# vvvvvw/Sentinel

Hardware: AMD Instinct MI355X
Metric: decided entries/sec (whole node) at 1M resources; % of HBM roofline (higher is better)
Workload: dtype int64/f64

## Files before the change

### sentinel_amd/csrc/decide.hip

```cpp
#include <hip/hip_runtime.h>
#include <stdlib.h>
#include <stdint.h>

#include "authority.h"
#include "chain.h"
#include "aux.h"
#include "pmap.h"

using namespace sg;

#define WAVE 64
#define MAXR 16
#define JMAX_FLOW 4
#define JMAX_DEG 4
#define JMAX_RL 2

__device__ __forceinline__ uint32_t lane_id() { return __lane_id(); }
__device__ __forceinline__ uint64_t lanemask_lt() {
    uint32_t l = lane_id();
    return l == 0 ? 0ull : (~0ull >> (64 - l));
}

#define J8_MAX (1u << 23)
#define SEG_ITEMS 16
// ... 26 lines not shown
__device__ __forceinline__ uint32_t seg_block_excl_scan(uint32_t v, uint32_t* total) {
    __shared__ uint32_t ws[4];
    const int w = threadIdx.x >> 6, l = threadIdx.x & 63;
    uint32_t x = v;
#pragma unroll
    for (int o = 1; o < 64; o <<= 1) {
        const uint32_t y = __shfl_up(x, o, 64);
        if (l >= o) x += y;
    }
    if (l == 63) ws[w] = x;
    __syncthreads();
    uint32_t pre = 0, tot = 0;
#pragma unroll
    for (int k = 0; k < 4; ++k) { if (k < w) pre += ws[k]; tot += ws[k]; }
    *total = tot;
    return pre + x - v;
}
__global__ __launch_bounds__(256) void k_seg_count(const uint32_t* __restrict__ keys, uint64_t n, uint32_t* __restrict__ cnt,
                                                   const uint32_t* __restrict__ lo) {
    const uint64_t b = lo ? *lo : 0u;
    if ((uint64_t)(blockIdx.x + 1) * SEG_TILE <= b) {
        if (threadIdx.x == 0) cnt[blockIdx.x] = 0;
        return;
    }
    uint32_t kk[SEG_ITEMS];
    const uint64_t i0 = (uint64_t)blockIdx.x * SEG_TILE + (uint64_t)threadIdx.x * SEG_ITEMS;
    const uint32_t f = seg_flags16(keys, n, i0, kk, b);
    uint32_t tot;
    (void)seg_block_excl_scan((uint32_t)__popc(f), &tot);
    if (threadIdx.x == 0) cnt[blockIdx.x] = tot;
}
__global__ __launch_bounds__(256) void k_seg_emit(const uint32_t* __restrict__ keys, uint64_t n,
                                                  const uint32_t* __restrict__ off, Seg* __restrict__ segs,
                                                  const uint32_t* __restrict__ lo, const uint32_t* __restrict__ sbase) {
    const uint64_t b = lo ? *lo : 0u;
    if ((uint64_t)(blockIdx.x + 1) * SEG_TILE <= b) return;
    uint32_t kk[SEG_ITEMS];
    const uint64_t i0 = (uint64_t)blockIdx.x * SEG_TILE + (uint64_t)threadIdx.x * SEG_ITEMS;
    uint32_t f = seg_flags16(keys, n, i0, kk, b);
    uint32_t tot;
    uint32_t pos = (sbase ? *sbase : 0u) + off[blockIdx.x] + seg_block_excl_scan((uint32_t)__popc(f), &tot);
#pragma unroll
    for (int j = 0; j < SEG_ITEMS; ++j) {
        if ((f >> j) & 1u) {
            Seg sg;
            sg.res = kk[j];
            sg.start = (uint32_t)(i0 + j);
            sg.len = 0;
            sg.bin = 0;
            segs[pos++] = sg;
        }
    }
}
#define AUX_SHORT 256u
__device__ __forceinline__ uint32_t wave_alloc(uint32_t* ctr, uint32_t k) {
    uint32_t x = k;
#pragma unroll
    for (int o = 1; o < 64; o <<= 1) {
        const uint32_t y = __shfl_up(x, o, 64);
        if ((int)(threadIdx.x & 63) >= o) x += y;
    }
    const uint32_t tot = __shfl(x, 63, 64);
    uint32_t base = 0;
    if ((threadIdx.x & 63) == 63 && tot) base = atomicAdd(ctr, tot);
    base = __shfl(base, 63, 64);
    return base + x - k;
}
__global__ __launch_bounds__(256) void k_seg_bin(Seg* __restrict__ segs, const uint32_t* __restrict__ mp, uint64_t n,
// ... 73 lines not shown
                for (uint32_t wd = b0 >> 5; wd <= (b1 >> 5); ++wd) {
                    uint32_t m32 = 0xFFFFFFFFu;
                    if (wd == (b0 >> 5)) m32 &= 0xFFFFFFFFu << (b0 & 31);
                    if (wd == (b1 >> 5)) m32 &= 0xFFFFFFFFu >> (31 - (b1 & 31));
                    atomicOr(&need_blk[wd], m32);
                }
                tabs = true;
            }
        }
        const uint32_t rank = atomicAdd(&cnt[bin], 1u);
        sg.bin = bin | (auxp ? SEG_AUXP : 0u) | (tabs ? SEG_TABS : 0u) | (rank << SEG_RANK_SHIFT);
        segs[s] = sg;
    }
    if (aux) {
        const uint32_t o = wave_alloc(aux + 0, aux_short ? 1u : 0u);
        if (aux_short) ashort[o] = s;
        const uint32_t q = wave_alloc(aux + 1, aux_np);
        const uint32_t j = wave_alloc(aux + 3, aux_np ? 1u : 0u);
        if (aux_np) along[j] = ((uint64_t)s << 32) | q;
        const uint32_t u = wave_alloc(aux + 2, aux_np > 1 ? 1u : 0u);
        if (aux_np > 1) amulti[u] = ((uint64_t)s << 32) | q;
    }
    if (mix) {
        const uint32_t a = wave_alloc(mixc + 0, mixk == 1 ? 1u : 0u);
        if (mixk == 1) mix[a] = s;
        const uint32_t b = wave_alloc(mixc + 1, mixk == 2 ? 1u : 0u);
        if (mixk == 2) mix[mix_cap + b] = s;
    }
    __syncthreads();
    for (uint32_t b = threadIdx.x; b < N_BINS; b += blockDim.x) blkcnt[(uint64_t)b * nblk + blockIdx.x] = cnt[b];
}
__global__ __launch_bounds__(256) void k_seg_order(Seg* __restrict__ segs, const uint32_t* __restrict__ mp,
                                                   const uint32_t* __restrict__ off, uint32_t nblk,
                                                   uint32_t* __restrict__ order) {
    const uint32_t s = blockIdx.x * blockDim.x + threadIdx.x;
    if (s >= *mp) return;
    const uint32_t v = segs[s].bin, bin = v & 0x3F;
    order[off[(uint64_t)bin * nblk + blockIdx.x] + (v >> SEG_RANK_SHIFT)] = s;
    segs[s].bin = v & ((1u << SEG_RANK_SHIFT) - 1);
}
__global__ void k_bin_offsets(const uint32_t* __restrict__ off, uint32_t nblk, const uint32_t* __restrict__ mp,
                              uint32_t* __restrict__ out) {
    const uint32_t b = threadIdx.x;
    if (b < N_BINS) out[b] = off[(uint64_t)b * nblk];
    if (b == N_BINS) out[b] = *mp;
}

__global__ __launch_bounds__(256) void k_scatter_rec(const SEv* __restrict__ rec_o, uint64_t n,
                                                     const uint32_t* __restrict__ pos_of, SEv* __restrict__ recs,
                                                     uint32_t* __restrict__ prev, uint32_t* __restrict__ nprev,
                                                     Link* __restrict__ link, uint32_t* __restrict__ bst, uint32_t epoch,
                                                     uint32_t* __restrict__ bflags) {
    const uint64_t i = (uint64_t)blockIdx.x * blockDim.x + threadIdx.x;
    if (i >= n) return;
    SEv r = rec_o[i];
    const uint32_t p = pos_of[i] & 0x7FFFFFFFu;
    if (r.code == RC_BATCH) {
        const uint32_t po = pos_of[r.x];
        if (po & 0x80000000u) r.x = po & 0x7FFFFFFFu;
        else r.code = r.kind == SG_EV_EXIT ? RC_NONE : RC_NOT;
    } else if (r.code == RC_PREV) {
        prev[atomicAdd(nprev, 1u)] = p;
    }
    if (r.kind == SG_EV_ENTRY) {
        if (r.cnt == 0) atomicOr(bflags, BF_ZERO_CNT);
    } else if (r.code == RC_NONE || r.code == RC_PREV) {
        atomicOr(&bst[p >> 10], BST_STATIC);
    }
// ... 27 lines not shown
        if (in[k] && kind != SG_EV_ENTRY && code == RC_BATCH)
            xd[k] = reinterpret_cast<unsigned long long*>(kind == SG_EV_EXIT ? &link[w[k].y].exit_l : &link[w[k].y].trace_l);
    }
    auto xch = [&](int k) -> uint32_t {
        const uint64_t p = base + (uint64_t)k * 256 + threadIdx.x;
        return xd[k] ? (uint32_t)(atomicExch(xd[k], ((unsigned long long)epoch << 32) | (uint32_t)p) >> 32) : 0u;
    };
    uint32_t o0 = 0, o1 = 0, o2 = 0, o3 = 0;
    if (tables) { o0 = xch(0); o1 = xch(1); o2 = xch(2); o3 = xch(3); }
    uint32_t ka[4], kb[4];
#pragma unroll
    for (int k = 0; k < 4; ++k) {
        const uint64_t p = base + (uint64_t)k * 256 + threadIdx.x;
        ka[k] = skeys[p < n ? p : n - 1];
        kb[k] = skeys[w[k].y < n ? w[k].y : n - 1];
    }
    bool bad = false;
#pragma unroll
    for (int k = 0; k < 4; ++k)
        if (xd[k] && w[k].y >= kmin && ka[k] != kb[k]) bad = true;
    const bool multi = o0 == epoch || o1 == epoch || o2 == epoch || o3 == epoch;
    if (__ballot(multi) && (threadIdx.x & 63) == 0) atomicOr(bflags, BF_MULTI_LINK);
    if (__ballot(bad) && (threadIdx.x & 63) == 0) atomicOr(bflags, BF_BAD_REF);
    if (!tables) return;
    for (int o = 32; o > 0; o >>= 1) v += (uint32_t)__shfl_xor((int)v, o, 64);
    if ((threadIdx.x & 63) == 0) wsum[threadIdx.x >> 6] = v;
    __syncthreads();
    if (threadIdx.x == 0) {
        const uint32_t sum = wsum[0] + wsum[1] + wsum[2] + wsum[3];
        if (sum) atomicAdd(&bst[blockIdx.x], sum);
    }
}
__global__ void k_resolve(const uint32_t* __restrict__ prev, uint32_t np, const uint8_t* __restrict__ ring,
                          SEv* __restrict__ recs, const uint32_t* __restrict__ vals, const sg_event_ext* __restrict__ ext) {
    const uint32_t i = blockIdx.x * blockDim.x + threadIdx.x;
    if (i >= np) return;
    const uint32_t p = prev[i];
    SEv r = recs[p];
    const uint8_t st = ring[r.x];
    if (st == ST_NOT_ENTRY) r.code = r.kind == SG_EV_EXIT ? RC_NONE : RC_NOT;
    else r.code = (st == ST_PASS || st == ST_PASS_WAIT) ? RC_PASSED : RC_NOT;
    r.x = 0;
    if (ext) {
        const sg_event_ext x = ext[vals[p] & 0x7FFFFFFFu];
        if (!(x.origin_id >> TAG_ORIGIN_BITS)) r.x = x.origin_id | (x.context_id << TAG_ORIGIN_BITS);
    }
    recs[p] = r;
}

#define POST_ITEMS 4
__global__ __launch_bounds__(256) void k_post(const uint32_t* __restrict__ pos_of, const uint32_t* __restrict__ dec,
                                              uint64_t n, uint64_t gbase, uint8_t* __restrict__ ring, uint64_t ring_mask,
                                              uint32_t* __restrict__ out) {
    const uint64_t base = (uint64_t)blockIdx.x * (256 * POST_ITEMS) + threadIdx.x;
    uint32_t po[POST_ITEMS], d[POST_ITEMS];
#pragma unroll
    for (int k = 0; k < POST_ITEMS; ++k) {
        const uint64_t i = base + (uint64_t)k * 256;
        po[k] = i < n ? pos_of[i] : 0u;
    }
#pragma unroll
    for (int k = 0; k < POST_ITEMS; ++k)
        d[k] = (po[k] & 0x80000000u) ? dec[po[k] & 0x7FFFFFFFu] : mk_dec(ST_NOT_ENTRY, 0, 0);
#pragma unroll
    for (int k = 0; k < POST_ITEMS; ++k) {
        const uint64_t i = base + (uint64_t)k * 256;
        if (i < n) {
            out[i] = d[k];
            ring[(gbase + i) & ring_mask] = (uint8_t)(d[k] & 0xFF);
        }
    }
}
// ... 3257 lines not shown
                    if (id != NO_ID) pm_grow(S, id, adds, pool_next, pool_nb, bflags, nullptr, nullptr, 0, epoch);
                }
        }
    }
    __threadfence();
    __syncthreads();
    if (pool_nb && t == 0 && pool_next[PC_RESCUE] == epoch) atomicOr(&sflags, (uint32_t)BF_TINY_FALLBACK);
    __syncthreads();
    if (sflags & BF_TINY_FALLBACK) {
        if (t == 0) atomicOr(bflags, sflags);
        return;
    }
    if (t < m) lane_seg<16>(recs, ev, vals, sg, S, cfg, t0, dec, bflags, t);
    __threadfence();
    __syncthreads();
    if (t < n) {
        const uint32_t d = ev[t].kind == SG_EV_ENTRY ? dec[posof[t]] : (uint32_t)ST_NOT_ENTRY;
        out[t] = d;
        S.ring[(gbase + t) & ring_mask] = (uint8_t)(d & 0xFF);
    }
    if (t == 0 && sflags) atomicOr(bflags, sflags);
}

namespace sg {

hipError_t launch_seg(const uint32_t* keys, uint64_t n, uint32_t* flag, uint32_t* pos, Seg* segs, hipStream_t st,
                      hipError_t (*scan)(const uint32_t*, uint32_t*, uint64_t, uint32_t*, uint32_t*, hipStream_t),
                      uint32_t* part, uint32_t* nseg) {
    const uint32_t nt = (uint32_t)((n + SEG_TILE - 1) / SEG_TILE);
    hipLaunchKernelGGL(k_seg_count, dim3(nt), dim3(256), 0, st, keys, n, flag, (const uint32_t*)nullptr);
    hipError_t e = scan(flag, pos, nt, part, nseg, st);
    if (e != hipSuccess) return e;
    hipLaunchKernelGGL(k_seg_emit, dim3(nt), dim3(256), 0, st, keys, n, pos, segs, (const uint32_t*)nullptr,
                       (const uint32_t*)nullptr);
    return hipGetLastError();
}
__global__ void k_add2(uint32_t* __restrict__ dst, const uint32_t* __restrict__ a, const uint32_t* __restrict__ b) {
    if (threadIdx.x == 0) *dst = *a + *b;
}
hipError_t launch_seg_cold(const uint32_t* keys, uint64_t n, const uint32_t* lo, const uint32_t* sbase, uint32_t* flag,
                           uint32_t* pos, Seg* segs, hipStream_t st,
                           hipError_t (*scan)(const uint32_t*, uint32_t*, uint64_t, uint32_t*, uint32_t*, hipStream_t),
                           uint32_t* part, uint32_t* ccount, uint32_t* nseg) {
    const uint32_t nt = (uint32_t)((n + SEG_TILE - 1) / SEG_TILE);
    hipLaunchKernelGGL(k_seg_count, dim3(nt), dim3(256), 0, st, keys, n, flag, lo);
    hipError_t e = scan(flag, pos, nt, part, ccount, st);
    if (e != hipSuccess) return e;
    hipLaunchKernelGGL(k_seg_emit, dim3(nt), dim3(256), 0, st, keys, n, pos, segs, lo, sbase);
    hipLaunchKernelGGL(k_add2, dim3(1), dim3(64), 0, st, nseg, sbase, ccount);
    return hipGetLastError();
}
hipError_t launch_block_sums(const SEv* recs, uint64_t n, uint32_t* bst, Link* link, uint32_t epoch, uint32_t* bflags,
                             const uint32_t* skeys, const uint32_t* lo, const uint32_t* need_blk, hipStream_t st) {
    hipLaunchKernelGGL(k_block_sums, dim3((uint32_t)((n + 1023) / 1024)), dim3(256), 0, st, recs, skeys, n, bst, link,
                       epoch, bflags, lo, need_blk);
    return hipGetLastError();
}
hipError_t launch_seg_bin(Seg* segs, const uint32_t* mp, uint32_t mb, uint64_t n, const Prog* prog, const uint32_t* prio,
                          uint32_t lane_max, uint32_t j1_max, uint32_t j4_max, uint32_t force_lane, uint32_t* blkcnt,
                          uint32_t pq_ok, uint32_t pq_wide, uint32_t* aux, uint32_t* ashort, uint64_t* along,
                          uint64_t* amulti, uint32_t* mixc, uint32_t* mix, uint32_t mix_cap, uint32_t* mixlen,
                          uint32_t mix_wide, uint32_t head_min, const uint16_t* hot_tab, uint32_t nhot,
                          const uint32_t* nhotseg, uint32_t* need_hot, uint32_t* need_blk, const uint32_t* bmax,
                          uint32_t skip_min, uint32_t* nmark, hipStream_t st) {
    const uint32_t nblk = (mb + 255) / 256;
    if (!nblk) return hipSuccess;
    hipLaunchKernelGGL(k_seg_bin, dim3(nblk), dim3(256), 0, st, segs, mp, n, prog, prio, lane_max, j1_max, j4_max, force_lane,
                       blkcnt, nblk, pq_ok, pq_wide, aux, ashort, along, amulti, mixc, mix, mix_cap, mixlen, mix_wide,
                       head_min, hot_tab, nhot, nhotseg, need_hot, need_blk, bmax, skip_min, nmark);
    return hipGetLastError();
}
hipError_t launch_seg_order(Seg* segs, const uint32_t* mp, uint32_t mb, const uint32_t* off, uint32_t* order,
                            uint32_t* bin_off, hipStream_t st) {
    const uint32_t nblk = (mb + 255) / 256;
    if (nblk) hipLaunchKernelGGL(k_seg_order, dim3(nblk), dim3(256), 0, st, segs, mp, off, nblk, order);
    hipLaunchKernelGGL(k_bin_offsets, dim3(1), dim3(64), 0, st, off, nblk ? nblk : 1, mp, bin_off);
    return hipGetLastError();
}
hipError_t launch_gather(const SEv* rec_o, const uint32_t* vals, const uint32_t* skeys, uint64_t n,
                         const uint32_t* pos_of, SEv* recs, uint32_t* prev, uint32_t* nprev, Link* link, uint32_t* bst,
                         uint32_t epoch, uint32_t* bflags, hipStream_t st) {
    uint32_t nb = (uint32_t)((n + 255) / 256);
    hipError_t e = hipMemsetAsync(bst, 0, ((n + 1023) / 1024) * 4, st);
    if (e != hipSuccess) return e;
    hipLaunchKernelGGL(k_scatter_rec, dim3(nb), dim3(256), 0, st, rec_o, n, pos_of, recs, prev, nprev, link, bst,
                       epoch, bflags);
    hipLaunchKernelGGL(k_block_sums, dim3((uint32_t)((n + 1023) / 1024)), dim3(256), 0, st, recs, skeys, n, bst, link,
                       epoch, bflags, (const uint32_t*)nullptr, (const uint32_t*)nullptr);
    return hipGetLastError();
}
hipError_t launch_fill(const Span* spans, const uint32_t* nspan, uint32_t cap, const SEv* recs, const Prog* prog,
                       const DRule* rules, uint32_t* dec, hipStream_t st) {
    hipLaunchKernelGGL(k_fill, dim3(2048), dim3(256), 0, st, spans, nspan, cap, recs, prog, rules, dec);
    return hipGetLastError();
}
hipError_t launch_resolve(const uint32_t* prev, uint32_t np, const uint8_t* ring, SEv* recs, const uint32_t* vals,
                          const sg_event_ext* ext, hipStream_t st) {
    if (!np) return hipSuccess;
    hipLaunchKernelGGL(k_resolve, dim3((np + 255) / 256), dim3(256), 0, st, prev, np, ring, recs, vals, ext);
    return hipGetLastError();
}
hipError_t launch_post(const uint32_t* pos_of, const uint32_t* dec, uint64_t n, uint64_t gbase, uint8_t* ring,
                       uint64_t ring_mask, uint32_t* out, hipStream_t st) {
    uint32_t nb = (uint32_t)((n + 256 * POST_ITEMS - 1) / (256 * POST_ITEMS));
    hipLaunchKernelGGL(k_post, dim3(nb), dim3(256), 0, st, pos_of, dec, n, gbase, ring, ring_mask, out);
    return hipGetLastError();
}
hipError_t launch_chain(const SEv* recs, const uint32_t* vals, const Seg* segs, uint32_t m, NodeInfo* info,
                        uint32_t grant_all, uint32_t* ncand, uint64_t* cand, const sg_event* ev, const Prog* prog,
                        const sg_event_ext* ext, uint32_t max_ctx, hipStream_t st) {
    if (!m) return hipSuccess;
    hipLaunchKernelGGL(k_chain, dim3((m + 255) / 256), dim3(256), 0, st, recs, vals, segs, m, info, grant_all, ncand,
                       cand, ev, prog, ext, max_ctx);
    return hipGetLastError();
}
hipError_t launch_tiny(const sg_event* ev, uint32_t n, const DevState& S, const DevCfg& cfg, uint32_t max_res,
                       uint32_t* prio_w, const uint32_t* comp, uint64_t n_args, uint32_t grant_all,
                       unsigned long long* pool_next, uint64_t pool_nb, uint32_t epoch, SEv* recs, uint32_t* vals,
                       uint32_t* dec, Seg* segs, uint32_t* bflags, uint32_t* out, hipStream_t st) {
    if (n == 0 || n > TINY_MAX) return hipErrorInvalidValue;
    hipLaunchKernelGGL(k_tiny, dim3(1), dim3(TINY_MAX), 0, st, ev, n, S, cfg, max_res, prio_w, comp, n_args, grant_all,
                       pool_next, pool_nb, epoch, recs, vals, dec, segs, bflags, out);
    return hipGetLastError();
}
uint32_t tiny_max() { return TINY_MAX; }
hipError_t launch_head(const SEv* recs, const Seg* segs, const uint32_t* order, uint32_t m, const DevState& S,
                       const DevCfg& cfg, int64_t t0, uint32_t* dec, uint32_t* bflags, hipStream_t st);
hipError_t launch_decide_bin(int bin, const SEv* recs, const sg_event* ev, const uint32_t* vals, const Seg* segs,
                             const uint32_t* order, uint32_t m, const DevState& S, const DevCfg& cfg, int64_t t0,
                             uint32_t* dec, uint32_t* bflags, hipStream_t st) {
    if (!m) return hipSuccess;
    if ((bin == BIN_J16 || bin == BIN_J4 || bin == BIN_J1) && cfg.heads && !(cfg.dbg_flags & HEAD_OFF)) {
// ... 43 lines not shown
```

### sentinel_amd/csrc/dev_types.h

```cpp
#pragma once
#include <hip/hip_runtime.h>
#include <stdint.h>

#include "../../include/sentinel_gpu.h"

namespace sg {

struct AuthDesc;

struct Bkt {
    int64_t ws;
    int64_t pass;
    int64_t block;
    int64_t exc;
    int64_t succ;
    int64_t rt;
    int64_t occ;
    int64_t minrt;
};
static_assert(sizeof(Bkt) == 64, "Bkt must be 64 B");

#define NO_KEY 0xFFFFFFFFFFFFFFFFull

enum : uint32_t {
// ... 114 lines not shown
    int64_t stamp[PM_BKT];
};
static_assert(sizeof(PBucket) == 128, "PBucket must be one 128-byte line");
struct PData {
    int64_t v0;
    int32_t v1;
    uint32_t pad;
};
static_assert(sizeof(PData) == 16, "PData must be 16 B");
#define PM_MIN_NB 2u
enum { PC_NEXT = 0, PC_FLOOR = 1, PC_RESCUES = 2, PC_RESCUE = 3, PC_WORDS = 4 };
__host__ __device__ inline uint32_t map_buckets(uint32_t cap) { return (2u * cap + PM_BKT - 1) / PM_BKT > 2u ? (2u * cap + PM_BKT - 1) / PM_BKT : 2u; }
struct PMap {
    uint64_t base;
    uint64_t bm;
    int64_t clock;
    int64_t thr;
    uint32_t nb;
    uint32_t cap;
    uint32_t live;
    uint32_t rb_log2;
    uint32_t pad[4];
};
static_assert(sizeof(PMap) == 64, "PMap must be 64 B");
#define PM_BASE_CAP 4000u
#define PM_TOTAL_CAP 200000u
#define PQ_MAX_CAP 8176u

enum : uint8_t { ST_PASS = 0, ST_PASS_WAIT = 1, ST_BLOCK_FLOW = 2, ST_BLOCK_DEGRADE = 3, ST_BLOCK_PARAM = 4,
                 ST_NO_CHECK = 5, ST_BLOCK_UPSTREAM = 6, ST_BLOCK_AUTHORITY = 7, ST_NOT_ENTRY = 0xFF };

#define HEAD_OFF 16384u
#define TABLES_ALL 32768u
#define LITE_CHECK 65536u
struct DevCfg {
    int32_t max_rt;
    int32_t occupy_timeout;
    int32_t max_chain;
    int32_t switch_on;
    int64_t snap_hi;
    uint64_t ring_mask;
    uint32_t dbg_flags;
    uint32_t heads;
};

struct Seg {
    uint32_t res;
    uint32_t start;
    uint32_t len;
    uint32_t bin;
};
#define SEG_AUXP 0x80u
#define SEG_PV 0x40u
#define SEG_PVT 0x100u
#define SEG_TABS 0x200u
#define SEG_RANK_SHIFT 10

struct PvSeg {
    uint32_t ok;
    uint32_t n;
    uint32_t off;
    uint32_t mid;
    uint32_t rk;
    uint32_t ch0;
    uint32_t nch;
    uint32_t fbits;
// ... 166 lines not shown
enum : uint32_t { BF_PRIORITIZED = 1,
                  BF_PQ_INVARIANT = 2,
                  BF_PTAB_FULL = 4,
                  BF_BAD_RES = 8, BF_BAD_REF = 16,
                  BF_BACKWARD = 32, BF_TSPAN = 64,
                  BF_BAD_ARGS = 512,
                  BF_AUX_FULL = 1024,
                  BF_POOL_FULL = 2048,
                  BF_MULTI_LINK = 128,
                  BF_ZERO_CNT = 256,
                  BF_TINY_FALLBACK = 4096,
                  BF_TINY_REJECTED = 8192,
                  BF_LITE_STALE = 16384 };

struct SEv {
    int32_t dt;
    uint32_t x;
    uint16_t cnt;
    uint16_t rt;
    uint8_t kind;
    uint8_t flags;
    uint8_t code;
    uint8_t pad;
};
static_assert(sizeof(SEv) == 16, "SEv must be 16 B");
enum : uint8_t {
    RC_NONE = 0,
    RC_BATCH = 1,
    RC_PASSED = 2,
    RC_NOT = 3,
    RC_PREV = 4
};

enum : uint32_t {
    BIN_J16 = 0,
    BIN_J4 = 1,
    BIN_J1 = 2,
    BIN_PQ16 = 3,
    BIN_PQ4 = 4,
    BIN_J8 = 5,
    BIN_LANE = 6,
    LANE_BINS = 19,
    BIN_LANE16 = BIN_LANE + LANE_BINS,
    BIN_LITE = BIN_LANE16 + LANE_BINS,
    N_BINS = BIN_LITE + LANE_BINS
};

}
```

### sentinel_amd/csrc/engine.cpp

```cpp
#include <hip/hip_runtime.h>

#include <algorithm>
#include <array>
#include <chrono>
#include <cmath>
#include <cstdint>
#include <cstdio>
#include <cstdlib>
#include <cstring>
#include <deque>
#include <functional>
#include <map>
#include <set>
#include <string>
#include <unordered_map>
#include <vector>

#include "../../include/sentinel_gpu.h"
#include "authority.h"
#include "dev_types.h"
#include "pkeys.h"
#include "pmap.h"
#include "pvtab.h"

namespace sg {
hipError_t launch_rs_first(const sg_event* ev, uint64_t n, uint32_t max_res, uint64_t gbase, const uint8_t* ring,
                           uint64_t ring_mask, int32_t max_rt, SEv* rec_o, uint32_t* keys, uint32_t* vals,
                           uint32_t* ghist, uint32_t nblocks, uint32_t* bflags, int64_t* t0_out, uint32_t* prio,
                           uint64_t* key_ring, const uint32_t* comp, const sg_event_ext* ext, const sg_arg* args,
                           uint64_t n_args, uint32_t max_ctx, const AuthDesc* auth, const uint32_t* auth_ids,
                           hipStream_t st);
hipError_t launch_radix_hist(const uint32_t* keys, uint64_t n, int shift, uint32_t* ghist, uint32_t nblocks,
                             hipStream_t st);
hipError_t launch_radix_hist_n(const uint32_t* keys, uint64_t n, const uint32_t* ndev, int shift, uint32_t* ghist,
                               uint32_t nblocks, hipStream_t st);
hipError_t launch_radix_scatter_n(const uint32_t* kin, const uint32_t* vin, uint64_t n, const uint32_t* ndev, int shift,
                                  const uint32_t* goff, uint32_t nblocks, uint32_t* kout, uint32_t* vout, hipStream_t st);
hipError_t launch_radix_scatter_x(const uint32_t* kin, const uint32_t* vin, uint64_t n, const uint32_t* ndev,
                                  const uint32_t* tcnt, const uint32_t* dbase, int shift, const uint32_t* goff,
                                  uint32_t nblocks, uint32_t* kout, uint32_t* vout, uint32_t* pos_of, hipStream_t st);
hipError_t launch_grp_first(const sg_event* ev, uint64_t n, uint32_t max_res, uint64_t gbase, uint64_t ring_mask,
                            uint32_t* bflags, int64_t* t0_out, uint32_t* prio, uint64_t* key_ring, const uint32_t* comp,
                            const sg_event_ext* ext, const sg_arg* args, uint64_t n_args, uint32_t max_ctx,
                            const AuthDesc* auth, const uint32_t* auth_ids,
                            const uint16_t* hot_tab, uint32_t nhot, uint32_t nblocks, uint32_t* words,
                            uint32_t* hot_hist, uint32_t* ckeys, uint32_t* cvals, uint32_t* ccnt, uint32_t* chist,
                            hipStream_t st);
hipError_t launch_hot_scan(uint32_t* C, uint32_t nblocks, uint32_t nhot, uint32_t* part, uint32_t* hb, uint32_t* total,
                           hipStream_t st);
hipError_t launch_hot_bmax(const sg_event* ev, uint32_t nblocks, const uint32_t* P, uint32_t nhot, const uint32_t* hb,
                           uint32_t* edges, uint32_t* bmax, hipStream_t st);
hipError_t launch_grp_records(const sg_event* ev, uint64_t n, uint64_t gbase, uint64_t ring_mask, int32_t max_rt,
                              const uint32_t* words, const uint32_t* P, uint32_t nhot, uint32_t nblocks,
                              const uint32_t* hb, SEv* recs, uint32_t* svals, uint32_t* prev,
                              uint32_t* nprev, uint32_t* bst, uint32_t* bflags, const sg_event_ext* ext,
                              const sg_arg* args, uint32_t max_ctx, Link* link, uint32_t epoch,
                              const uint32_t* need_hot, const uint32_t* need_blk, hipStream_t st);
hipError_t launch_hot_segs(const uint32_t* hb, uint32_t nhot, const uint32_t* hot_list, Seg* segs, uint32_t* out,
                           hipStream_t st);
hipError_t launch_hot_build(const Seg* segs, const uint32_t* mp, uint32_t mb, uint32_t min_len, uint32_t max_res, uint16_t* hot_tab,
                            uint32_t* hot_list, uint32_t nhot_old, uint32_t* hot_n, hipStream_t st);
hipError_t launch_cold_n(uint64_t n, const uint32_t* hot_total, uint32_t* out, hipStream_t st);
hipError_t launch_cold_small(const uint32_t* kin, const uint32_t* vin, const uint32_t* cnt, const uint32_t* dbase,
                             uint32_t* kout, uint32_t* vout, uint32_t* words, hipStream_t st);
uint32_t hot_max();
hipError_t launch_grp_clear(uint32_t* bsmall, uint32_t nsmall, uint32_t* bst, uint32_t nbst, uint32_t* need,
                            uint32_t nneed, hipStream_t st);
hipError_t launch_seg_cold(const uint32_t* keys, uint64_t n, const uint32_t* lo, const uint32_t* sbase, uint32_t* flag,
                           uint32_t* pos, Seg* segs, hipStream_t st,
                           hipError_t (*scan)(const uint32_t*, uint32_t*, uint64_t, uint32_t*, uint32_t*, hipStream_t),
                           uint32_t* part, uint32_t* ccount, uint32_t* nseg);
hipError_t launch_block_sums(const SEv* recs, uint64_t n, uint32_t* bst, Link* link, uint32_t epoch, uint32_t* bflags,
                             const uint32_t* skeys, const uint32_t* lo, const uint32_t* need_blk, hipStream_t st);
hipError_t launch_radix_scatter(const uint32_t* kin, const uint32_t* vin, uint64_t n, int shift, const uint32_t* goff,
                                uint32_t nblocks, uint32_t* kout, uint32_t* vout, uint32_t* pos_of, hipStream_t st);
uint32_t radix_tile();
hipError_t launch_scan(const uint32_t*, uint32_t*, uint64_t, uint32_t*, uint32_t*, hipStream_t);
hipError_t launch_snapshot(Bkt*, NodeInfo*, uint32_t, int64_t, int32_t, uint32_t*, uint32_t*, uint32_t*, uint32_t*,
                           sg_metric_node*, uint64_t, hipStream_t);
hipError_t launch_init_state(Bkt* sec, Bkt* minb, NodeInfo* info, int64_t* borrow, uint32_t nres, hipStream_t st);
hipError_t launch_set_flags(NodeInfo* info, const uint64_t* upd, uint32_t n, hipStream_t st);
hipError_t launch_region_copy(const uint64_t* src, uint64_t* dst, const uint64_t* tri, uint32_t n, hipStream_t st);
hipError_t launch_seg(const uint32_t* keys, uint64_t n, uint32_t* flag, uint32_t* pos, Seg* segs, hipStream_t st,
                      hipError_t (*scan)(const uint32_t*, uint32_t*, uint64_t, uint32_t*, uint32_t*, hipStream_t),
                      uint32_t* part, uint32_t* nseg);
hipError_t launch_seg_bin(Seg* segs, const uint32_t* mp, uint32_t mb, uint64_t n, const Prog* prog, const uint32_t* prio,
                          uint32_t lane_max, uint32_t j1_max, uint32_t j4_max, uint32_t force_lane, uint32_t* blkcnt,
                          uint32_t pq_ok, uint32_t pq_wide, uint32_t* aux, uint32_t* ashort, uint64_t* along,
                          uint64_t* amulti, uint32_t* mixc, uint32_t* mix, uint32_t mix_cap, uint32_t* mixlen,
                          uint32_t mix_wide, uint32_t head_min, const uint16_t* hot_tab, uint32_t nhot,
                          const uint32_t* nhotseg, uint32_t* need_hot, uint32_t* need_blk, const uint32_t* bmax,
                          uint32_t skip_min, uint32_t* nmark, hipStream_t st);
hipError_t launch_aux(const SEv* recs, const Seg* segs, const uint32_t* aux, const uint32_t* ashort,
                      const uint64_t* along, uint64_t* apiece, const uint64_t* amulti, const DevState& S, const DevCfg& cfg,
                      int64_t t0, const uint32_t* dec, AuxAcc* pool, uint32_t pool_cap, uint32_t* pool_n, uint64_t* meta,
                      uint32_t* bflags, hipStream_t st);
hipError_t launch_aux_cold(const SEv* recs, const Seg* segs, const uint32_t* aux, const uint32_t* ashort, const DevState& S,
                           const DevCfg& cfg, int64_t t0, const uint32_t* dec, uint32_t* bflags, hipStream_t st);
hipError_t launch_pq(int wide, const SEv* recs, const sg_event* ev, const uint32_t* vals, const Seg* segs,
                     const uint32_t* order, uint32_t m, const DevState& S, const DevCfg& cfg, int64_t t0, uint32_t* dec,
                     uint32_t* bflags, hipStream_t st);
hipError_t launch_pm_grow(const Seg* segs, const uint32_t* mp, uint32_t mb, const DevState& S, unsigned long long* pool_next,
                          uint64_t pool_nb, uint32_t* bflags, uint4* mv, uint32_t* nmv, uint32_t mcap, uint32_t epoch,
                          uint32_t nm, PBucket* b2, PData* d2, uint32_t* sz, uint32_t* off, uint32_t* part,
                          hipError_t (*scan)(const uint32_t*, uint32_t*, uint64_t, uint32_t*, uint32_t*, hipStream_t),
                          hipStream_t st);
hipError_t launch_pm_compact(PMap* pm, uint32_t n, const PBucket* ob, const PData* od, PBucket* nbk, PData* nd,
                             uint32_t* sz, uint32_t* off, uint32_t* part, unsigned long long* pool_next,
                             hipError_t (*scan)(const uint32_t*, uint32_t*, uint64_t, uint32_t*, uint32_t*, hipStream_t),
                             hipStream_t st);
// ... 2 lines not shown
hipError_t launch_pv_a(SEv* recs, const uint32_t* vals, Seg* segs, const uint32_t* list, uint32_t m,
                       const DevState& S, const DevCfg& cfg, uint32_t* dec, PvSeg* pv, PvBuf B, uint32_t cap,
                       uint32_t* tot, uint32_t* hist, uint32_t* part, hipStream_t st,
                       hipError_t (*radix_hist)(const uint32_t*, uint64_t, const uint32_t*, int, uint32_t*, uint32_t, hipStream_t),
                       hipError_t (*radix_scatter)(const uint32_t*, const uint32_t*, uint64_t, const uint32_t*, int,
                                                   const uint32_t*, uint32_t, uint32_t*, uint32_t*, hipStream_t),
                       hipError_t (*scan)(const uint32_t*, uint32_t*, uint64_t, uint32_t*, uint32_t*, hipStream_t),
                       uint32_t tile, uint32_t* rest, uint32_t grant_all);
hipError_t launch_pv_b(SEv* recs, Seg* segs, const uint32_t* list, uint32_t m, const DevState& S, int64_t t0,
                       uint32_t* dec, uint32_t* bflags, PvSeg* pv, PvBuf B, uint32_t cap, uint32_t* tot, uint32_t* part,
                       uint32_t jumps, hipStream_t st,
                       hipError_t (*scan)(const uint32_t*, uint32_t*, uint64_t, uint32_t*, uint32_t*, hipStream_t),
                       uint32_t* rest);
hipError_t launch_pvt(SEv* recs, const sg_event* ev, const uint32_t* vals, Seg* segs, const uint32_t* list, uint32_t m,
                      const DevState& S, const DevCfg& cfg, uint32_t* dec, uint32_t* bflags, PvSeg* pv, PvBuf B,
                      uint32_t cap, uint32_t* tot, uint32_t* hist, uint32_t* part, hipStream_t st,
                      hipError_t (*radix_hist)(const uint32_t*, uint64_t, const uint32_t*, int, uint32_t*, uint32_t, hipStream_t),
                      hipError_t (*radix_scatter)(const uint32_t*, const uint32_t*, uint64_t, const uint32_t*, int,
                                                      const uint32_t*, uint32_t, uint32_t*, uint32_t*, hipStream_t),
                      hipError_t (*scan)(const uint32_t*, uint32_t*, uint64_t, uint32_t*, uint32_t*, hipStream_t),
                      uint32_t tile, uint32_t* rest);
hipError_t launch_pq_mix(int post, SEv* recs, const sg_event* ev, const uint32_t* vals, const Seg* segs,
                         const uint32_t* list, uint32_t n_narrow, uint64_t wide_off, uint32_t n_wide, const DevState& S,
                         const DevCfg& cfg, int64_t t0, uint32_t* dec, uint32_t* bflags, hipStream_t st,
                         const uint32_t* rest, const uint32_t* rest_n);
hipError_t launch_seg_order(Seg* segs, const uint32_t* mp, uint32_t mb, const uint32_t* off, uint32_t* order,
                            uint32_t* bin_off, hipStream_t st);
hipError_t launch_gather(const SEv* rec_o, const uint32_t* vals, const uint32_t* skeys, uint64_t n,
                         const uint32_t* pos_of, SEv* recs, uint32_t* prev, uint32_t* nprev, Link* link, uint32_t* bst,
                         uint32_t epoch, uint32_t* bflags, hipStream_t st);
hipError_t launch_fill(const Span* spans, const uint32_t* nspan, uint32_t cap, const SEv* recs, const Prog* prog,
                       const DRule* rules, uint32_t* dec, hipStream_t st);
hipError_t launch_resolve(const uint32_t* prev, uint32_t np, const uint8_t* ring, SEv* recs, const uint32_t* vals,
                          const sg_event_ext* ext, hipStream_t st);
hipError_t launch_post_w(const uint32_t* words, const uint32_t* P, uint32_t nhot, const uint32_t* dec, uint64_t n,
                         uint64_t gbase, uint8_t* ring, uint64_t ring_mask, uint32_t* out, hipStream_t st);
hipError_t launch_post(const uint32_t* pos_of, const uint32_t* dec, uint64_t n, uint64_t gbase, uint8_t* ring,
                       uint64_t ring_mask, uint32_t* out, hipStream_t st);
hipError_t launch_chain(const SEv* recs, const uint32_t* vals, const Seg* segs, uint32_t m, NodeInfo* info,
                        uint32_t grant_all, uint32_t* ncand, uint64_t* cand, const sg_event* ev, const Prog* prog,
                        const sg_event_ext* ext, uint32_t max_ctx, hipStream_t st);
hipError_t launch_tiny(const sg_event* ev, uint32_t n, const DevState& S, const DevCfg& cfg, uint32_t max_res,
                       uint32_t* prio_w, const uint32_t* comp, uint64_t n_args, uint32_t grant_all,
                       unsigned long long* pool_next, uint64_t pool_nb, uint32_t epoch, SEv* recs, uint32_t* vals,
                       uint32_t* dec, Seg* segs, uint32_t* bflags, uint32_t* out, hipStream_t st);
uint32_t tiny_max();
hipError_t launch_decide_bin(int bin, const SEv* recs, const sg_event* ev, const uint32_t* vals, const Seg* segs,
                             const uint32_t* order, uint32_t m, const DevState& S, const DevCfg& cfg, int64_t t0,
                             uint32_t* dec, uint32_t* bflags, hipStream_t st);
hipError_t launch_tok_classify(const sg_token_req* req, uint64_t n, const CSlot* tab, uint32_t mask, uint32_t* fidx,
                               sg_token_result* res, uint32_t* flags, uint32_t* nskeys, uint32_t* nsvals, uint32_t nns,
                               hipStream_t st);
hipError_t launch_tok_limiter_ns(const sg_token_req* req, uint64_t n, const uint32_t* sk, const uint32_t* sv,
                                 const uint32_t* fidx, uint32_t nflows, NsLimiter* lims, const double* limits,
                                 uint32_t nns, uint32_t* keys, uint32_t* vals, sg_token_result* res, uint32_t* bflag,
                                 uint32_t* bidx, uint32_t* bstart, uint32_t* kpass, uint32_t* part, uint32_t* small,
                                 uint32_t* nsb,
                                 hipError_t (*scan)(const uint32_t*, uint32_t*, uint64_t, uint32_t*, uint32_t*, hipStream_t),
                                 hipStream_t st);
hipError_t launch_tok_limiter_par(const sg_token_req* req, uint64_t n, const uint32_t* fidx, uint32_t nflows,
                                  NsLimiter* lim, double allowed, uint32_t* keys, uint32_t* vals, sg_token_result* res,
                                  uint32_t* bflag, uint32_t* cflag, uint32_t* bidx, uint32_t* cexcl, uint32_t* bstart,
                                  uint32_t* kpass, uint32_t* part, uint32_t* small,
                                  hipError_t (*scan)(const uint32_t*, uint32_t*, uint64_t, uint32_t*, uint32_t*, hipStream_t),
                                  hipStream_t st);
hipError_t launch_tok_limiter(const sg_token_req* req, uint64_t n, const uint32_t* fidx, uint32_t nflows,
                              NsLimiter* lim, double allowed, uint32_t* keys, uint32_t* vals, sg_token_result* res,
// ... 332 lines not shown
    PData* d_pdat = nullptr;
    uint64_t* d_pbm = nullptr;
    uint32_t* d_ppre = nullptr;
    uint32_t* d_tmid = nullptr;
    uint8_t* d_ring = nullptr;
    uint32_t rules_cap = 0, hot_cap = 0;

    struct BatchSlot {
        sg_event* d_ev = nullptr;
        uint32_t* d_out = nullptr;
        uint32_t *d_k0 = nullptr, *d_v0 = nullptr, *d_k1 = nullptr, *d_v1 = nullptr;
        uint32_t *d_hist = nullptr, *d_part = nullptr, *d_flag = nullptr, *d_pos = nullptr, *d_order = nullptr;
        uint32_t *d_posof = nullptr, *d_dec = nullptr, *d_blkcnt = nullptr, *d_prev = nullptr;
        SEv *d_recs = nullptr, *d_rec_o = nullptr;
        uint32_t* d_ccnt = nullptr;
        bool radix = false;
        uint32_t nhot = 0;
        uint32_t hot_marked = 0;
        Seg* d_segs = nullptr;
        uint64_t* d_cand = nullptr;
        uint32_t* d_bsmall = nullptr;
        sg_event_ext* d_ext = nullptr;
        sg_arg* d_args = nullptr;
        uint64_t ext_cap = 0, args_cap = 0;
        uint32_t* d_ashort = nullptr;
        uint64_t *d_apiece = nullptr, *d_amulti = nullptr, *d_along = nullptr;
        uint64_t aux_cap_n = 0;
        uint32_t* d_mix = nullptr;
        uint64_t mix_cap = 0;
        Link* d_link = nullptr;
        uint32_t *d_bst = nullptr, *d_pend = nullptr;
        Span* d_spans = nullptr;
        hipEvent_t* ev = nullptr;
        hipEvent_t last_post = nullptr;
        uint32_t* h_head = nullptr;
        struct Grouped {
            uint64_t n = 0, n_args = 0, gbase = 0, ring_mask = 0;
            const sg_event* dev_ev = nullptr;
            const sg_event_ext* dev_ext = nullptr;
            const sg_arg* dev_args = nullptr;
            uint32_t *out = nullptr, *dev_out = nullptr, *vin = nullptr;
            uint32_t epoch = 0, skip_min = 0, lane_max = 0, mb = 0;
            bool ext = false, host_out = false, force_lane = false;
            int set = 0;
        } g;
    } slot[2];
    int cur = 0;
    int last = -1;
    int grouped = -1;
    int held_rc = 0;
    std::string held_msg;
    bool handoff_late = true;
    static constexpr int N_SETS = 4;
    hipEvent_t evset[N_SETS][5] = {};
    uint32_t* h_mirror = nullptr;
    uint64_t seq = 0;
    struct InFlight { int set; uint32_t hot_marked; };
    std::deque<InFlight> inflight;
    hipStream_t gstream = nullptr;
    std::vector<std::array<double, 4>> tlog;
    std::vector<std::array<double, 2>> glog;
    std::string fatal;
    uint32_t* d_prio = nullptr;
    uint16_t* d_hot_tab = nullptr;
    uint32_t* d_hot_list = nullptr;
    uint32_t nhot = 0;
    uint32_t* d_hot_part = nullptr;
    uint32_t* d_hot_hb = nullptr;
    uint32_t* d_need = nullptr;
    uint64_t need_words = 0;
    uint32_t* d_edges = nullptr;
    uint32_t hot_marked_last = 0;
    bool radix_group = false;
    uint64_t radix_below = 1u << 18;
    uint32_t tok_light = 8192;
    uint32_t tok_wide = 1024;
    bool tiny_on = true;
    AuxNode* d_auxtab = nullptr;
    uint32_t* d_auxcnt = nullptr;
    uint64_t aux_mask = 0;
    AuxAcc* d_auxpool = nullptr;
    uint64_t* d_auxmeta = nullptr;
    uint32_t auxpool_cap = 0;
    uint64_t auxmeta_cap = 0;
    std::unordered_map<std::string, uint32_t> origin_ids, context_ids;
    std::unordered_map<std::string, int> rule_names;
    AuthTable auth;
    AuthDesc* d_auth = nullptr;
    uint32_t* d_auth_ids = nullptr;
    size_t auth_ids_cap = 0;
    bool auth_on = false, auth_loaded = false;
    std::vector<std::string> last_auth;
    uint32_t* d_comp = nullptr;
    uint32_t* d_prev = nullptr;
    uint32_t* d_bsmall = nullptr;
    Link* d_link = nullptr;
    uint32_t *d_bst = nullptr, *d_pend = nullptr;
    Span* d_spans = nullptr;
    uint32_t span_cap = 0;
    uint32_t epoch = 0;
    uint64_t spans_total = 0;
    uint64_t cap_n = 0;
    sg_event* d_ev = nullptr;
    uint32_t* d_out = nullptr;
// ... 85 lines not shown
    uint64_t pcap = 0, pvcap = 0;
    pk::Dict<pk::StdHash> pkeys;
    std::vector<uint64_t> par_pins;
    uint64_t* d_ks_key = nullptr;
    uint32_t *d_ks_idx = nullptr, *d_ks_marks = nullptr;
    uint64_t ks_cap = 0;
    hipEvent_t ks_ev[4] = {nullptr, nullptr, nullptr, nullptr};
    uint64_t ks_sweeps = 0, ks_last[4] = {0, 0, 0, 0};
    double ks_scan_ms[3] = {0, 0, 0};
    uint64_t pbm_words = 0;
    uint32_t *d_snap_cnt = nullptr, *d_snap_off = nullptr;
    sg_metric_node* d_snap_out = nullptr;
    uint64_t snap_cap = 0;
};

static int handoff(sg_engine* e);

namespace {

constexpr uint64_t SHARD_BATCH = 3ull << 21;

static void activate(sg_engine* e, int k) {
    auto& B = e->slot[k];
    e->d_ev = B.d_ev; e->d_out = B.d_out;
    e->d_k0 = B.d_k0; e->d_v0 = B.d_v0; e->d_k1 = B.d_k1; e->d_v1 = B.d_v1;
    e->d_hist = B.d_hist; e->d_part = B.d_part; e->d_flag = B.d_flag; e->d_pos = B.d_pos; e->d_order = B.d_order;
    e->d_posof = B.d_posof; e->d_dec = B.d_dec; e->d_blkcnt = B.d_blkcnt; e->d_prev = B.d_prev;
    e->d_recs = B.d_recs; e->d_rec_o = B.d_rec_o; e->d_segs = B.d_segs; e->d_cand = B.d_cand;
    e->d_bsmall = B.d_bsmall;
    e->d_link = B.d_link; e->d_bst = B.d_bst; e->d_pend = B.d_pend; e->d_spans = B.d_spans;
}
static void free_slot(sg_engine::BatchSlot& B) {
    dfree(B.d_ev); dfree(B.d_out); dfree(B.d_k0); dfree(B.d_v0); dfree(B.d_k1); dfree(B.d_v1);
    dfree(B.d_hist); dfree(B.d_part); dfree(B.d_flag); dfree(B.d_pos); dfree(B.d_order); dfree(B.d_segs);
    dfree(B.d_cand); dfree(B.d_posof); dfree(B.d_dec); dfree(B.d_recs); dfree(B.d_rec_o); dfree(B.d_blkcnt);
    dfree(B.d_prev); dfree(B.d_bsmall); dfree(B.d_ccnt);
    B.d_ccnt = nullptr;
    dfree(B.d_link); dfree(B.d_bst); dfree(B.d_pend); dfree(B.d_spans); dfree(B.d_ext); dfree(B.d_args);
    dfree(B.d_ashort); dfree(B.d_apiece); dfree(B.d_amulti); dfree(B.d_along); dfree(B.d_mix);
    B.d_mix = nullptr;
    B.ext_cap = B.args_cap = B.aux_cap_n = B.mix_cap = 0;
    B.d_link = nullptr; B.d_bst = B.d_pend = nullptr; B.d_spans = nullptr;
    B.d_ev = nullptr; B.d_out = nullptr; B.d_k0 = B.d_v0 = B.d_k1 = B.d_v1 = nullptr;
    B.d_hist = B.d_part = B.d_flag = B.d_pos = B.d_order = nullptr;
    B.d_posof = B.d_dec = B.d_blkcnt = B.d_prev = B.d_bsmall = nullptr;
    B.d_recs = B.d_rec_o = nullptr; B.d_segs = nullptr; B.d_cand = nullptr;
}
int ensure_batch(sg_engine* e, uint64_t n) {
    if (n <= e->cap_n) return SG_OK;
    uint64_t c = std::max<uint64_t>(n, 1u << 20);
    HIPCHK(hipStreamSynchronize(e->stream));
    uint64_t nblocks = (c + radix_tile() - 1) / radix_tile();
    e->cap_hist = nblocks * 256;
    for (auto& B : e->slot) {
        free_slot(B);
        HIPCHK(hipMalloc(&B.d_ev, c * sizeof(sg_event)));
        HIPCHK(hipMalloc(&B.d_out, c * 4));
        HIPCHK(hipMalloc(&B.d_k0, c * 4));
        HIPCHK(hipMalloc(&B.d_v0, c * 4));
        HIPCHK(hipMalloc(&B.d_k1, c * 4));
        HIPCHK(hipMalloc(&B.d_v1, c * 4));
        HIPCHK(hipMalloc(&B.d_hist, e->cap_hist * 4));
        HIPCHK(hipMalloc(&B.d_part, (e->cap_hist / 4096 + c / 4096 + 64) * 4));
        HIPCHK(hipMalloc(&B.d_flag, c * 4));
        HIPCHK(hipMalloc(&B.d_pos, c * 4));
        HIPCHK(hipMalloc(&B.d_order, c * 4));
        HIPCHK(hipMalloc(&B.d_segs, c * sizeof(Seg)));
        HIPCHK(hipMalloc(&B.d_cand, c * 8));
        HIPCHK(hipMalloc(&B.d_posof, c * 4));
        HIPCHK(hipMalloc(&B.d_dec, c * 4));
        HIPCHK(hipMalloc(&B.d_recs, c * sizeof(SEv)));
        const uint64_t co = (e->radix_group || c >= (1ull << 30)) ? c : std::min<uint64_t>(c, e->radix_below);
        if (co) HIPCHK(hipMalloc(&B.d_rec_o, co * sizeof(SEv)));
        HIPCHK(hipMalloc(&B.d_ccnt, 3 * (nblocks + 64) * 4));
    }
    dfree(e->d_hot_part);
    dfree(e->d_hot_hb);
    dfree(e->d_need);
    dfree(e->d_edges);
    e->need_words = hot_max() + c / 32768 + 2 + hot_max();
    HIPCHK(hipMalloc(&e->d_need, e->need_words * 4));
    HIPCHK(hipMalloc(&e->d_edges, (nblocks + 2) * 4));
    HIPCHK(hipMalloc(&e->d_hot_part, (nblocks / 16 + 2) * hot_max() * 4));
    HIPCHK(hipMalloc(&e->d_hot_hb, 2 * hot_max() * 4));
    for (auto& B : e->slot) {
        HIPCHK(hipMalloc(&B.d_blkcnt, ((c + 255) / 256 + 1) * N_BINS * 4));
        HIPCHK(hipMalloc(&B.d_prev, c * 4));
        HIPCHK(hipMalloc(&B.d_bsmall, 256 * 4));
        HIPCHK(hipMemset(B.d_bsmall, 0, 256 * 4));
        HIPCHK(hipMalloc(&B.d_link, c * sizeof(Link)));
        HIPCHK(hipMemset(B.d_link, 0, c * sizeof(Link)));
        HIPCHK(hipMalloc(&B.d_bst, ((c + 1023) / 1024 + 1) * 4));
        HIPCHK(hipMalloc(&B.d_pend, c * 4));
        HIPCHK(hipMalloc(&B.d_spans, (c / SPAN_CHUNK + 65536) * sizeof(Span)));
    }
    e->span_cap = (uint32_t)(c / SPAN_CHUNK + 65536);
    e->cap_n = c;
    activate(e, e->cur);
    return SG_OK;
}

constexpr uint32_t HEAD_WORDS = 77;
constexpr uint32_t MIRROR_WORDS = 121;

static int collect(sg_engine* e) {
    if (e->inflight.empty()) return SG_OK;
    const sg_engine::InFlight f = e->inflight.front();
    e->inflight.pop_front();
    hipEvent_t* ev = e->evset[f.set];
    HIPCHK(hipEventSynchronize(ev[4]));
    float g = 0, d = 0, p = 0;
    (void)hipEventElapsedTime(&g, ev[0], ev[1]);
    (void)hipEventElapsedTime(&d, ev[2], ev[3]);
    (void)hipEventElapsedTime(&p, ev[3], ev[4]);
    (void)hipGetLastError();
    e->last_ms[0] = g; e->last_ms[1] = d; e->last_ms[2] = p; e->last_ms[3] = (double)g + d + p;
    e->tlog.push_back({(double)g, (double)d, (double)p, (double)g + d + p});
    if (e->tlog.size() > 4096) e->tlog.erase(e->tlog.begin(), e->tlog.begin() + 2048);
    float ga = 0, gb = 0;
    const uint64_t collected = e->seq - e->inflight.size() - 1;
    if (collected > 0) {
        hipEvent_t* pv = e->evset[(f.set + sg_engine::N_SETS - 1) % sg_engine::N_SETS];
        if (hipEventElapsedTime(&ga, pv[1], ev[0]) != hipSuccess) ga = NAN;
        if (hipEventElapsedTime(&gb, pv[4], ev[2]) != hipSuccess) gb = NAN;
        (void)hipGetLastError();
    }
    e->glog.push_back({(double)ga, (double)gb});
    if (e->glog.size() > 4096) e->glog.erase(e->glog.begin(), e->glog.begin() + 2048);
    const uint32_t* mir = e->h_mirror + (size_t)f.set * MIRROR_WORDS;
    const uint32_t bflags = mir[0];
    e->spans_total += mir[120];
    e->hot_marked_last = f.hot_marked;
    if (bflags & BF_BAD_REF)
        return fail(SG_EINVAL, "an EXIT/TRACE references an event that is not an earlier ENTRY of the same resource");
    if (bflags & BF_BACKWARD)
        return fail(SG_EINVAL, "event timestamps must be non-decreasing across batches (SURVEY Q3)");
    if (bflags & BF_AUX_FULL) return fail(SG_ECAPACITY, "origin/context node pool full (raise aux_node_capacity)");
    if (bflags & BF_LITE_STALE)
        return fail(SG_ESTATE, "internal error (SG_LITE_CHECK): k_lite stored a minute bucket without a load that was not stale");
    if (bflags & BF_PQ_INVARIANT)
        e->fatal = "internal error: a k_pq tile's presorted key subset did not match its accesses";
    else if (bflags & BF_POOL_FULL)
        e->fatal = "the hot-parameter map pool is used up (raise param_table_log2)";
    else if (bflags & BF_PTAB_FULL)
        e->fatal = "a hot-parameter map table could not place a key (its map holds a ghost entry)";
    if (bflags & (BF_PQ_INVARIANT | BF_PTAB_FULL | BF_POOL_FULL)) return fail(SG_ECAPACITY, e->fatal + " -- engine unusable");
    return SG_OK;
}
static inline const AuthDesc* dev_auth(const sg_engine* e) { return e->auth_on ? e->d_auth : nullptr; }
static inline const uint32_t* dev_auth_ids(const sg_engine* e) { return e->auth_on ? e->d_auth_ids : nullptr; }

static int drain(sg_engine* e) {
    int rc = e->held_rc;
    std::string msg = e->held_msg;
    e->held_rc = 0;
    auto note = [&](int r) {
        if (r && !rc) { rc = r; msg = g_err; }
    };
    note(handoff(e));
    while (!e->inflight.empty()) note(collect(e));
    HIPCHK(hipStreamSynchronize(e->stream));
    return rc ? fail(rc, msg) : SG_OK;
}
static void drain_hold(sg_engine* e) {
    const int rc = drain(e);
    if (rc) { e->held_rc = rc; e->held_msg = g_err; }
}


static uint32_t rule_map_cap(int64_t duration_sec) {
    const int64_t c = (int64_t)PM_BASE_CAP * std::max<int64_t>(duration_sec, 1);
    return (uint32_t)std::min<int64_t>(c, PM_TOTAL_CAP);
}

int upload_rules(sg_engine* e, bool reset_flow_state, bool reset_deg_state, bool reset_par_state) {
    uint32_t R = e->cfg.max_resources;
    std::vector<Prog> prog(R);
    std::vector<DRule> rules;
    std::vector<RState> rst;
    std::vector<DHot> hot;
    std::vector<RState> old_rst;
    std::vector<Prog> old_prog;
    if ((!reset_flow_state || !reset_deg_state || !reset_par_state) && e->n_dev_rules) {
        old_rst.resize(e->n_dev_rules);
        old_prog.resize(R);
        HIPCHK(hipMemcpy(old_rst.data(), e->d_rstate, e->n_dev_rules * sizeof(RState), hipMemcpyDeviceToHost));
        HIPCHK(hipMemcpy(old_prog.data(), e->d_prog, R * sizeof(Prog), hipMemcpyDeviceToHost));
    }
    size_t nres = e->names.size();
    bool any_mix = false, any_head = false;
    std::vector<std::pair<uint32_t, uint32_t>> relate;
    for (size_t r = 0; r < nres && r < R; ++r) {
        Prog p;
        std::memset(&p, 0, sizeof(p));
// ... 329 lines not shown
}

int sg_engine_create(const sg_config* cfg_in, sg_engine** out) {
    if (!out) return fail(SG_EINVAL, "out is null");
    sg_config cfg;
    if (cfg_in) cfg = *cfg_in;
    else sg_config_default(&cfg);
    if (cfg.sample_count != 2 || cfg.interval_ms != 1000)
        return fail(SG_ENOTSUP, "the device path implements SAMPLE_COUNT=2, INTERVAL=1000 (the reference defaults)");
    if (cfg.cold_factor <= 1) return fail(SG_EINVAL, "cold factor must be > 1");
    if (cfg.max_resources == 0 || cfg.param_table_log2 < 4 || cfg.param_table_log2 > 34 || cfg.status_ring_log2 < 10 ||
        cfg.status_ring_log2 > 36)
        return fail(SG_EINVAL, "bad capacity in sg_config");
    int ndev = 0;
    if (hipGetDeviceCount(&ndev) != hipSuccess || ndev == 0) return fail(SG_EDEVICE, "no HIP device visible");
    if (cfg.device < 0 || cfg.device >= ndev) return fail(SG_EDEVICE, "device ordinal out of range");
    hipDeviceProp_t prop;
    if (hipGetDeviceProperties(&prop, cfg.device) != hipSuccess) return fail(SG_EDEVICE, "hipGetDeviceProperties failed");
    if (std::strncmp(prop.gcnArchName, "gfx950", 6) != 0)
        return fail(SG_EDEVICE, std::string("this build targets gfx950, found ") + prop.gcnArchName);
    sg_engine* e = new sg_engine();
    e->cfg = cfg;
    e->device = cfg.device;
    auto bad = [&](int rc) { sg_engine_destroy(e); return rc; };
    if (hipSetDevice(e->device) != hipSuccess) return bad(fail(SG_EDEVICE, "hipSetDevice failed"));
    int prio_lo = 0, prio_hi = 0;
    const char* sp = std::getenv("SG_STREAM_PRIO");
    if (!(sp && sp[0] == '0')) (void)hipDeviceGetStreamPriorityRange(&prio_lo, &prio_hi);
    if (!(sp && sp[0] == '1')) std::swap(prio_lo, prio_hi);
    if (hipStreamCreateWithPriority(&e->stream, hipStreamNonBlocking, prio_hi) != hipSuccess) return bad(fail(SG_EDEVICE, "stream"));
    if (hipStreamCreateWithPriority(&e->gstream, hipStreamNonBlocking, prio_lo) != hipSuccess) {
        return bad(fail(SG_EDEVICE, "stream"));
    }
    for (auto& s : e->evset)
        for (auto& v : s) if (hipEventCreate(&v) != hipSuccess) return bad(fail(SG_EDEVICE, "event"));
    for (auto& B : e->slot) {
        if (hipHostMalloc(&B.h_head, HEAD_WORDS * 4) != hipSuccess) return bad(fail(SG_ENOMEM, "pinned batch head"));
        B.ev = e->evset[0];
    }
    if (hipHostMalloc(&e->h_mirror, sg_engine::N_SETS * MIRROR_WORDS * 4) != hipSuccess)
        return bad(fail(SG_ENOMEM, "pinned batch flags"));
    std::memset(e->h_mirror, 0, sg_engine::N_SETS * MIRROR_WORDS * 4);
    uint64_t R = cfg.max_resources;
    if (hipMalloc(&e->d_sec, R * 2 * sizeof(Bkt)) != hipSuccess || hipMalloc(&e->d_minb, R * 60 * sizeof(Bkt)) != hipSuccess ||
        hipMalloc(&e->d_info, R * sizeof(NodeInfo)) != hipSuccess || hipMalloc(&e->d_prog, R * sizeof(Prog)) != hipSuccess ||
        hipMalloc(&e->d_ring, 1ull << cfg.status_ring_log2) != hipSuccess || hipMalloc(&e->d_small, 256 * 4) != hipSuccess ||
        hipMalloc(&e->d_sink, 1024 * 4) != hipSuccess || hipMalloc(&e->d_borrow, R * 4 * sizeof(int64_t)) != hipSuccess ||
        hipMalloc(&e->d_prio, R * 4) != hipSuccess || hipMalloc(&e->d_hot_tab, R * 2) != hipSuccess ||
        hipMalloc(&e->d_hot_list, hot_max() * 4) != hipSuccess)
        return bad(fail(SG_ENOMEM, "device allocation of the engine state failed"));
    {
        const uint64_t cap = std::max<uint32_t>(cfg.aux_node_capacity, 16u);
        uint64_t slots = 32;
        while (2 * slots < 3 * cap) slots <<= 1;
        e->aux_mask = slots - 1;
        e->cfg.aux_node_capacity = (uint32_t)cap;
        if (hipMalloc(&e->d_auxtab, slots * sizeof(AuxNode)) != hipSuccess || hipMalloc(&e->d_auxcnt, 4) != hipSuccess ||
            hipMemsetAsync(e->d_auxtab, 0xFF, slots * sizeof(AuxNode), e->stream) != hipSuccess ||
            hipMemsetAsync(e->d_auxcnt, 0, 4, e->stream) != hipSuccess)
            return bad(fail(SG_ENOMEM, "device allocation of the origin/context node table failed"));
    }
    if (hipMemsetAsync(e->d_prog, 0, R * sizeof(Prog), e->stream) != hipSuccess ||
        hipMemsetAsync(e->d_ring, 0xFF, 1ull << cfg.status_ring_log2, e->stream) != hipSuccess ||
        hipMemsetAsync(e->d_prio, 0, R * 4, e->stream) != hipSuccess ||
        hipMemsetAsync(e->d_hot_tab, 0xFF, R * 2, e->stream) != hipSuccess ||
        launch_init_state(e->d_sec, e->d_minb, e->d_info, e->d_borrow, (uint32_t)R, e->stream) != hipSuccess ||
        hipStreamSynchronize(e->stream) != hipSuccess)
        return bad(fail(SG_EDEVICE, "device initialisation failed"));
    for (auto& s : e->bin_stream)
        if (hipStreamCreateWithPriority(&s, hipStreamNonBlocking, prio_hi) != hipSuccess) return bad(fail(SG_EDEVICE, "stream"));
    if (hipEventCreateWithFlags(&e->fork, hipEventDisableTiming) != hipSuccess ||
        hipEventCreateWithFlags(&e->fork0, hipEventDisableTiming) != hipSuccess ||
        hipEventCreateWithFlags(&e->grown, hipEventDisableTiming) != hipSuccess)
        return bad(fail(SG_EDEVICE, "event"));
    for (auto& v : e->join)
        if (hipEventCreateWithFlags(&v, hipEventDisableTiming) != hipSuccess) return bad(fail(SG_EDEVICE, "event"));
    if (const char* d = std::getenv("SG_DEBUG")) {
        if (d[0] == '1' && hipMalloc(&e->d_dbg, 64 * 8) == hipSuccess) (void)hipMemset(e->d_dbg, 0, 64 * 8);
    }
    if (const char* f = std::getenv("SG_DEBUG_FLAGS")) e->dbg_flags = (uint32_t)std::strtoul(f, nullptr, 0);
    e->radix_group = (e->dbg_flags & 8192) != 0;
    if (const char* f = std::getenv("SG_PROF_BIN")) e->prof_bin = std::atoi(f);
    if (const char* v = std::getenv("SG_LANE_MAX")) { e->lane_max = (uint32_t)std::strtoul(v, nullptr, 0); e->bins_pinned = true; }
    if (const char* v = std::getenv("SG_J1_MAX")) { e->j1_max = (uint32_t)std::strtoul(v, nullptr, 0); e->bins_pinned = true; }
    if (const char* v = std::getenv("SG_HEAD_MIN")) e->head_min = (uint32_t)std::strtoul(v, nullptr, 0);
    if (const char* v = std::getenv("SG_J4_MAX")) { e->j4_max = (uint32_t)std::strtoul(v, nullptr, 0); e->bins_pinned = true; }
    if (const char* v = std::getenv("SG_PIPELINE")) e->pipeline = v[0] == '1';
    if (const char* v = std::getenv("SG_HANDOFF")) e->handoff_late = v[0] != '0';
    if (const char* v = std::getenv("SG_TINY")) e->tiny_on = v[0] != '0';
    if (const char* v = std::getenv("SG_LITE_CHECK")) { if (v[0] == '1') e->dbg_flags |= LITE_CHECK; }
    if (const char* v = std::getenv("SG_RADIX_BELOW")) e->radix_below = std::strtoull(v, nullptr, 0);
    if (const char* v = std::getenv("SG_TOK_WIDE")) e->tok_wide = std::atoi(v) == 512 ? 512u : 1024u;
    if (const char* v = std::getenv("SG_TOK_LIGHT")) e->tok_light = (uint32_t)std::strtoul(v, nullptr, 0);
    if (const char* v = std::getenv("SG_TOK_NS")) e->tok_ns = v[0] == '1';
    if (const char* v = std::getenv("SG_PV_LOG2")) e->pv_log2 = (uint32_t)std::min(24l, std::max(4l, std::strtol(v, nullptr, 0)));
    if (const char* v = std::getenv("SG_PV_MAX_LOG2")) e->pv_max_log2 = (uint32_t)std::min(26l, std::max(4l, std::strtol(v, nullptr, 0)));
    e->pv_max_log2 = std::max(e->pv_max_log2, e->pv_log2);
    e->ns_names.push_back("default");
    e->ns_of["default"] = 0;
    e->ns_limit.push_back((double)cfg.cluster_max_allowed_qps);
    e->ns_conn.push_back(0);
    if (const char* v = std::getenv("SG_J1_STREAM")) e->j1_stream = std::atoi(v);
    if (const char* v = std::getenv("SG_PQ")) e->pq_on = v[0] != '0';
    if (const char* v = std::getenv("SG_MIX")) e->mix_on = v[0] != '0';
    if (const char* v = std::getenv("SG_MIX_PQ")) e->mix_pq = v[0] != '0';
    if (const char* v = std::getenv("SG_PV_PQ")) e->pv_pq = v[0] != '0';
    if (const char* v = std::getenv("SG_PV")) e->pv_on = v[0] != '0';
    e->pvt_on = e->pv_on;
    if (const char* v = std::getenv("SG_PVT")) e->pvt_on = v[0] != '0';
    if (const char* v = std::getenv("SG_PQ_WIDE")) e->pq_wide = (uint32_t)std::strtoul(v, nullptr, 0);
    if (const char* v = std::getenv("SG_SKIP_MIN")) {
        e->skip_min = std::max<uint32_t>(1u, (uint32_t)std::strtoul(v, nullptr, 0));
        e->skip_pinned = true;
    }
// ... 81 lines not shown
    if (e->pvt_on && e->d_pvtseg) {
        if (hipMemcpy(v.data(), e->d_pvtseg, v.size() * sizeof(PvSeg), hipMemcpyDeviceToHost) != hipSuccess) return -1;
        for (const auto& s : v) out[3] += s.ok ? 1 : 0;
        out[4] = tot[4];
        out[5] = tot[7];
    }
    if (!e->pv_on) out[0] = out[1] = out[2] = out[6] = 0;
    return 0;
}
extern "C" int sgx_param_pool(sg_engine* e, unsigned long long* out) {
    if (!e || !out || drain(e) != SG_OK) return -1;
    unsigned long long ctl[PC_WORDS] = {0, 0, 0, 0};
    if (e->d_pool_next && hipMemcpy(ctl, e->d_pool_next, sizeof(ctl), hipMemcpyDeviceToHost) != hipSuccess) return -1;
    out[0] = e->pool_nb; out[1] = ctl[PC_NEXT]; out[2] = ctl[PC_FLOOR]; out[3] = e->n_compact; out[4] = ctl[PC_RESCUES];
    return 0;
}

static int compact_pmaps(sg_engine* e);
extern "C" int sgx_param_compact(sg_engine* e) {
    if (!e || drain(e) != SG_OK) return -1;
    if (!e->pool_nb) return 0;
    if (compact_pmaps(e) != SG_OK) return -1;
    ++e->n_compact;
    return 0;
}

static void free_pv(sg_engine* e);

int sg_engine_destroy(sg_engine* e) {
    if (!e) return SG_OK;
    (void)hipSetDevice(e->device);
    e->grouped = -1;
    if (e->stream) (void)hipStreamSynchronize(e->stream);
    if (e->gstream) (void)hipStreamSynchronize(e->gstream);
    dfree(e->d_sec); dfree(e->d_minb); dfree(e->d_info); dfree(e->d_prog); dfree(e->d_rules); dfree(e->d_rstate);
    dfree(e->d_hot); dfree(e->d_pmap); dfree(e->d_pbkt); dfree(e->d_pdat); dfree(e->d_pbm); dfree(e->d_ppre); dfree(e->d_tmid); dfree(e->d_ring); dfree(e->d_small); dfree(e->d_sink);
    dfree(e->d_pool_next); dfree(e->d_pmoves); dfree(e->d_pbkt2); dfree(e->d_pdat2); dfree(e->d_pcwork);
    if (e->h_pool_next) (void)hipHostFree(e->h_pool_next);
    free_pv(e);
    dfree(e->d_pvseg); dfree(e->d_pvtseg); dfree(e->d_pvtot); dfree(e->d_pvrest);
    if (e->gstream) (void)hipStreamSynchronize(e->gstream);
    for (auto& B : e->slot) free_slot(B);
    dfree(e->d_auth); dfree(e->d_auth_ids);
    dfree(e->d_prio); dfree(e->d_hot_tab); dfree(e->d_hot_list); dfree(e->d_hot_part); dfree(e->d_hot_hb); dfree(e->d_need); dfree(e->d_edges); dfree(e->d_comp); dfree(e->d_auxtab); dfree(e->d_auxpool); dfree(e->d_auxcnt); dfree(e->d_auxmeta);
    dfree(e->d_pflow); dfree(e->d_phot); dfree(e->d_pftab); dfree(e->d_pvtab); dfree(e->d_preq); dfree(e->d_pvals);
    dfree(e->d_cflow); dfree(e->d_cbkt); dfree(e->d_ctab); dfree(e->d_nslim); dfree(e->d_nslimit); dfree(e->d_nsb); dfree(e->d_borrow); dfree(e->d_keyring);
    dfree(e->d_treq); dfree(e->d_tres); dfree(e->d_tfidx); dfree(e->d_tbounds);
    dfree(e->d_snap_cnt); dfree(e->d_snap_off); dfree(e->d_snap_out); dfree(e->d_dbg);
    dfree(e->d_ks_key); dfree(e->d_ks_idx); dfree(e->d_ks_marks);
    for (auto& v : e->ks_ev) if (v) (void)hipEventDestroy(v);
    dfree(e->d_pvcnt); dfree(e->d_pvspare);
    for (auto& v : e->pv_ev) if (v) (void)hipEventDestroy(v);
    for (auto& s : e->evset)
        for (auto& v : s) if (v) (void)hipEventDestroy(v);
    for (auto& B : e->slot) if (B.h_head) (void)hipHostFree(B.h_head);
    if (e->h_mirror) (void)hipHostFree(e->h_mirror);
    if (e->gstream) (void)hipStreamDestroy(e->gstream);
    for (auto& v : e->join) if (v) (void)hipEventDestroy(v);
    if (e->fork) (void)hipEventDestroy(e->fork);
    if (e->fork0) (void)hipEventDestroy(e->fork0);
    if (e->grown) (void)hipEventDestroy(e->grown);
    for (auto& s : e->bin_stream) if (s) (void)hipStreamDestroy(s);
    if (e->stream) (void)hipStreamDestroy(e->stream);
    delete e;
    return SG_OK;
}

int sg_register_resources(sg_engine* e, const char* const* names, uint32_t n, uint32_t* out_ids) {
    if (!e || (n && !names)) return fail(SG_EINVAL, "null argument");
    if (int rc = drain(e)) return rc;
    for (uint32_t i = 0; i < n; ++i) {
        if (!names[i]) return fail(SG_EINVAL, "null resource name");
        auto it = e->ids.find(names[i]);
        uint32_t id;
        if (it != e->ids.end()) id = it->second;
        else {
            if (e->names.size() >= e->cfg.max_resources) return fail(SG_ECAPACITY, "max_resources reached");
// ... 858 lines not shown
    if (n > B.aux_cap_n) {
        dfree(B.d_ashort); dfree(B.d_apiece); dfree(B.d_amulti); dfree(B.d_along);
        const uint64_t c = std::max<uint64_t>(n, 1u << 16);
        HIPCHK(hipMalloc(&B.d_ashort, c * 4));
        HIPCHK(hipMalloc(&B.d_along, (c / 257 + 64) * 8));
        HIPCHK(hipMalloc(&B.d_apiece, (c / AUX_PIECE + c / 257 + 64) * 8));
        HIPCHK(hipMalloc(&B.d_amulti, (c / AUX_PIECE + 64) * 8));
        B.aux_cap_n = c;
    }
    if (!e->d_auxpool) {
        HIPCHK(hipMalloc(&e->d_auxpool, (uint64_t)AUXPOOL_CAP * sizeof(AuxAcc)));
        e->auxpool_cap = AUXPOOL_CAP;
    }
    if (npiece > e->auxmeta_cap) {
        HIPCHK(hipStreamSynchronize(e->stream));
        dfree(e->d_auxmeta);
        const uint64_t c = std::max<uint64_t>(npiece, B.aux_cap_n / AUX_PIECE + B.aux_cap_n / 257 + 64);
        HIPCHK(hipMalloc(&e->d_auxmeta, c * 8));
        e->auxmeta_cap = c;
    }
    return SG_OK;
}

static bool is_device_ptr(const void* p) {
    hipPointerAttribute_t a;
    if (hipPointerGetAttributes(&a, p) != hipSuccess) { (void)hipGetLastError(); return false; }
    return a.type == hipMemoryTypeDevice || a.type == hipMemoryTypeManaged;
}

static int decide_stage(sg_engine* e, int k);

static int group_stage(sg_engine* e, int k, const sg_event* ev, const sg_event_ext* ext, uint64_t n, const sg_arg* args,
                       uint64_t n_args, uint32_t* out, int* prev) {
    activate(e, k);
    auto& B = e->slot[k];
    B.ev = e->evset[e->seq % sg_engine::N_SETS];
    hipStream_t gs = e->gstream;
    if (B.last_post) HIPCHK(hipStreamWaitEvent(gs, B.last_post, 0));
    const sg_event* dev_ev = ev;
    bool host_in = !is_device_ptr(ev);
    bool host_out = !is_device_ptr(out);
    if (host_in) {
        HIPCHK(hipMemcpyAsync(e->d_ev, ev, n * sizeof(sg_event), hipMemcpyHostToDevice, gs));
        dev_ev = e->d_ev;
    }
    uint32_t* dev_out = host_out ? e->d_out : out;
    const sg_event_ext* dev_ext = ext;
    const sg_arg* dev_args = n_args ? args : nullptr;
    if (ext && !is_device_ptr(ext)) {
        if (n > B.ext_cap) {
            dfree(B.d_ext);
            B.ext_cap = std::max<uint64_t>(n, 1u << 16);
            HIPCHK(hipMalloc(&B.d_ext, B.ext_cap * sizeof(sg_event_ext)));
        }
        HIPCHK(hipMemcpyAsync(B.d_ext, ext, n * sizeof(sg_event_ext), hipMemcpyHostToDevice, gs));
        dev_ext = B.d_ext;
    }
    if (n_args && !is_device_ptr(args)) {
        if (n_args > B.args_cap) {
            dfree(B.d_args);
            B.args_cap = std::max<uint64_t>(n_args, 1u << 16);
            HIPCHK(hipMalloc(&B.d_args, B.args_cap * sizeof(sg_arg)));
        }
        HIPCHK(hipMemcpyAsync(B.d_args, args, n_args * sizeof(sg_arg), hipMemcpyHostToDevice, gs));
        dev_args = B.d_args;
    }
    const uint64_t ring_mask = (1ull << e->cfg.status_ring_log2) - 1;
    if (!e->pipeline && e->last >= 0 && e->slot[e->last].last_post)
        HIPCHK(hipStreamWaitEvent(gs, e->slot[e->last].last_post, 0));
    HIPCHK(hipEventRecord(B.ev[0], gs));
    uint32_t R = e->cfg.max_resources;
    int bits = 1;
    while (bits < 32 && (1ull << bits) < R) ++bits;
    const int db = 8;
    int passes = (bits + db - 1) / db;
    uint32_t nblocks = (uint32_t)((n + radix_tile() - 1) / radix_tile());
    int64_t* d_t0 = reinterpret_cast<int64_t*>(e->d_bsmall + 4);
    uint32_t *kin = e->d_k1, *vin = e->d_v1, *kout = e->d_k0, *vout = e->d_v0;
    if (++e->epoch == 0) e->epoch = 1;
    B.radix = e->radix_group || n >= (1ull << 30) || n < e->radix_below;
    HIPCHK(launch_grp_clear(e->d_bsmall, 256, e->d_bst, B.radix ? 0u : (uint32_t)((n + 1023) / 1024), e->d_need,
                            B.radix ? 0u : (uint32_t)e->need_words, gs));
    const bool force_lane = !e->cfg.switch_on || (e->dbg_flags & 2);
    const uint32_t mb = (uint32_t)std::min<uint64_t>(n, R);
    const uint32_t nblk = (mb + 255) / 256;
    uint32_t lane_max = e->lane_max, j1_max = e->j1_max, j4_max = e->j4_max;
    if (!e->bins_pinned && n < SHARD_BATCH) {
        lane_max = std::min<uint32_t>(lane_max, 128);
        j1_max = std::min<uint32_t>(j1_max, 1024);
        j4_max = std::min<uint32_t>(j4_max, 4096);
    }
    j1_max = std::min<uint32_t>(j1_max, 64u * 65000u);
    j4_max = std::min<uint32_t>(j4_max, 256u * 65000u);
    const uint32_t skip_min = (!e->skip_pinned && n < SHARD_BATCH) ? std::min<uint32_t>(e->skip_min, 8192) : e->skip_min;
    auto bins = [&](uint32_t* need_hot, uint32_t* need_blk, const uint32_t* bmax) -> int {
        if (ext) {
            if (int arc = ensure_aux(e, B, n)) return arc;
        }
        if (e->has_mix) {
            if (int mrc = ensure_mix(B, mb)) return mrc;
        }
        HIPCHK(launch_seg_bin(e->d_segs, e->d_bsmall + 1, mb, n, e->d_prog, e->d_prio, lane_max, j1_max, j4_max,
                              force_lane ? 1 : 0, e->d_blkcnt, e->pq_on ? 1u : 0u, e->pq_wide, ext ? e->d_bsmall + 130 : nullptr,
                              B.d_ashort, B.d_along, B.d_amulti, e->d_bsmall + 6, e->has_mix ? B.d_mix : nullptr,
                              (uint32_t)B.mix_cap, e->d_bsmall + 72, (e->pv_on || e->pvt_on) ? 0u : e->pq_wide,
                              (e->dbg_flags & HEAD_OFF) ? 0u : e->head_min, e->d_hot_tab, e->nhot, e->d_bsmall + 80, need_hot,
                              need_blk, bmax, skip_min, e->d_bsmall + 73, gs));
        HIPCHK(launch_scan(e->d_blkcnt, e->d_blkcnt, (uint64_t)nblk * N_BINS, e->d_part, nullptr, gs));
        HIPCHK(launch_seg_order(e->d_segs, e->d_bsmall + 1, mb, e->d_blkcnt, e->d_order, e->d_bsmall + 8, gs));
        return SG_OK;
    };
    auto decide_prev = [&]() -> int {
        if (*prev < 0) return SG_OK;
        const int pk = *prev;
        *prev = -1;
        const int drc = decide_stage(e, pk);
        activate(e, k);
        return drc;
    };
    if (B.radix) {
        HIPCHK(launch_rs_first(dev_ev, n, R, e->gbase, e->d_ring, ring_mask, e->cfg.statistic_max_rt, e->d_rec_o,
                               e->d_k1, e->d_v1, e->d_hist, nblocks, e->d_bsmall + 0, d_t0, e->d_prio, e->d_keyring,
                               e->d_comp, dev_ext, dev_args, n_args, SG_MAX_CONTEXTS, dev_auth(e), dev_auth_ids(e), gs));
        if (int drc = decide_prev()) return drc;
        for (int p = 0; p < passes; ++p) {
            if (p > 0) HIPCHK(launch_radix_hist(kin, n, p * db, e->d_hist, nblocks, gs));
            HIPCHK(launch_scan(e->d_hist, e->d_hist, (uint64_t)nblocks << db, e->d_part, nullptr, gs));
            HIPCHK(launch_radix_scatter(kin, vin, n, p * db, e->d_hist, nblocks, kout, vout,
                                        p == passes - 1 ? e->d_posof : nullptr, gs));
            std::swap(kin, kout);
            std::swap(vin, vout);
        }
        HIPCHK(launch_seg(kin, n, e->d_flag, e->d_pos, e->d_segs, gs, launch_scan, e->d_part, e->d_bsmall + 1));
        HIPCHK(launch_gather(e->d_rec_o, vin, kin, n, e->d_posof, e->d_recs, e->d_prev, e->d_bsmall + 3, e->d_link,
                             e->d_bst, e->epoch, e->d_bsmall + 0, gs));
        if (int brc = bins(nullptr, nullptr, nullptr)) return brc;
    } else {
        const uint32_t nhot = e->nhot;
        B.nhot = nhot;
        uint32_t* words = e->d_flag;
        uint32_t* hot_off = e->d_pos;
        uint32_t* ccnt = B.d_ccnt;
        HIPCHK(launch_grp_first(dev_ev, n, R, e->gbase, ring_mask, e->d_bsmall + 0, d_t0, e->d_prio, e->d_keyring,
                                e->d_comp, dev_ext, dev_args, n_args, SG_MAX_CONTEXTS, dev_auth(e), dev_auth_ids(e),
                                e->d_hot_tab, nhot, nblocks,
                                words, hot_off, e->d_k1, e->d_v1, ccnt, e->d_hist, gs));
        if (int drc = decide_prev()) return drc;
        HIPCHK(launch_hot_scan(hot_off, nblocks, nhot, e->d_hot_part, e->d_hot_hb, e->d_bsmall + 77, gs));
        HIPCHK(launch_cold_n(n, e->d_bsmall + 77, e->d_bsmall + 78, gs));
        if (nblocks == 1) {
            HIPCHK(launch_cold_small(kin, vin, ccnt, e->d_bsmall + 77, kout, vout, words, gs));
            std::swap(kin, kout);
            std::swap(vin, vout);
        }
        for (int p = 0; p < passes && nblocks > 1; ++p) {
            if (p > 0) HIPCHK(launch_radix_hist_n(kin, n, e->d_bsmall + 78, p * db, e->d_hist, nblocks, gs));
            HIPCHK(launch_scan(e->d_hist, e->d_hist, (uint64_t)nblocks << db, e->d_part, nullptr, gs));
            const bool last = p == passes - 1;
            HIPCHK(launch_radix_scatter_x(kin, vin, n, p ? e->d_bsmall + 78 : nullptr, p ? nullptr : ccnt,
                                          last ? e->d_bsmall + 77 : nullptr, p * db, e->d_hist, nblocks, kout, vout,
                                          last ? words : nullptr, gs));
            std::swap(kin, kout);
            std::swap(vin, vout);
        }
        HIPCHK(launch_hot_segs(e->d_hot_hb, nhot, e->d_hot_list, e->d_segs, e->d_bsmall + 80, gs));
        const uint64_t sc = nblocks + 64;
        HIPCHK(launch_seg_cold(kin, n, e->d_bsmall + 77, e->d_bsmall + 80, ccnt + sc, ccnt + 2 * sc, e->d_segs, gs,
                               launch_scan, e->d_part, e->d_bsmall + 82, e->d_bsmall + 1));
        uint32_t *need_hot = nullptr, *need_blk = nullptr, *bmax = nullptr;
        if (!(e->dbg_flags & TABLES_ALL)) {
            need_hot = e->d_need;
            need_blk = e->d_need + hot_max();
            bmax = e->d_need + e->need_words - hot_max();
            HIPCHK(launch_hot_bmax(dev_ev, nblocks, hot_off, nhot, e->d_hot_hb, e->d_edges, bmax, gs));
        }
        if (int brc = bins(need_hot, need_blk, bmax)) return brc;
        HIPCHK(launch_grp_records(dev_ev, n, e->gbase, ring_mask, e->cfg.statistic_max_rt, words, hot_off, nhot, nblocks,
                                  e->d_hot_hb, e->d_recs, vin, e->d_prev, e->d_bsmall + 3, e->d_bst,
                                  e->d_bsmall + 0, dev_ext, dev_args, SG_MAX_CONTEXTS, e->d_link, e->epoch, need_hot,
                                  need_blk, gs));
        HIPCHK(launch_block_sums(e->d_recs, n, e->d_bst, e->d_link, e->epoch, e->d_bsmall + 0, kin, e->d_bsmall + 77,
                                 need_blk, gs));
    }
    const uint32_t hot_min = (uint32_t)std::max<uint64_t>(64, n / 8192);
    if (!B.radix)
        HIPCHK(launch_hot_build(e->d_segs, e->d_bsmall + 1, mb, hot_min, R, e->d_hot_tab, e->d_hot_list, e->nhot,
                                e->d_bsmall + 76, gs));
    static_assert(8 + N_BINS + 1 <= 72 && HEAD_WORDS == 77, "head layout");
    HIPCHK(hipMemcpyAsync(B.h_head, e->d_bsmall, HEAD_WORDS * 4, hipMemcpyDeviceToHost, gs));
    HIPCHK(hipEventRecord(B.ev[1], gs));
    auto& G = B.g;
    G.n = n; G.n_args = n_args; G.gbase = e->gbase; G.ring_mask = ring_mask;
    G.dev_ev = dev_ev; G.dev_ext = dev_ext; G.dev_args = dev_args;
    G.out = out; G.dev_out = dev_out; G.vin = vin;
    G.epoch = e->epoch; G.skip_min = skip_min; G.lane_max = lane_max; G.mb = mb;
    G.ext = ext != nullptr; G.host_out = host_out; G.force_lane = force_lane;
    G.set = (int)(e->seq % sg_engine::N_SETS);
    e->grouped = k;
    return SG_OK;
}

static int accept_grouped(sg_engine* e, bool drop = false) {
    const int k = e->grouped;
    auto& B = e->slot[k];
    e->grouped = -1;
    HIPCHK(hipEventSynchronize(B.ev[1]));
    const uint32_t* head = B.h_head;
    if (!B.radix) e->nhot = std::min<uint32_t>(head[76], hot_max());
    if (drop) return SG_OK;
    B.hot_marked = head[73];
    const uint32_t bflags = head[0];
    if (bflags & BF_BAD_RES) return fail(SG_EINVAL, "event res_id >= max_resources");
    if (bflags & BF_BAD_REF)
        return fail(SG_EINVAL, "an EXIT/TRACE references an event that is not an earlier ENTRY of the same resource");
    if (bflags & BF_TSPAN) return fail(SG_EINVAL, "a batch must span less than 2^31 ms");
    if (bflags & BF_BACKWARD) return fail(SG_EINVAL, "event timestamps must be non-decreasing (SURVEY Q3)");
    if (bflags & BF_BAD_ARGS)
        return fail(SG_EINVAL, "an sg_event_ext names args outside the table (or more than SG_MAX_ARGS, or a bad kind)");
    if (e->has_mix && head[7] && (e->pv_on || e->pvt_on) && head[72]) {
        if (int prc = ensure_pv(e, head[72], head[7])) return prc;
    }
    e->inflight.push_back({B.g.set, B.hot_marked});
    ++e->seq;
    e->last = k;
    e->cur = k ^ 1;
    e->gbase += B.g.n;
    return SG_OK;
}

static int handoff(sg_engine* e) {
    if (e->grouped < 0) return SG_OK;
    const int k = e->grouped;
    if (int rc = accept_grouped(e)) return rc;
    return decide_stage(e, k);
}

static int decide_enqueue(sg_engine* e, int k);

static int decide_stage(sg_engine* e, int k) {
    const int rc = decide_enqueue(e, k);
    if (rc) {
        const std::string why = g_err;
        if (!e->inflight.empty()) e->inflight.pop_back();
        if (e->fatal.empty()) e->fatal = "the decide stage of an accepted batch could not be enqueued (" + why + ")";
        return fail(rc, why);
    }
    return rc;
}

static int decide_enqueue(sg_engine* e, int k) {
    activate(e, k);
    auto& B = e->slot[k];
    const auto& G = B.g;
    hipStream_t st = e->stream;
    const uint64_t n = G.n, n_args = G.n_args, ring_mask = G.ring_mask;
    const sg_event* dev_ev = G.dev_ev;
    const sg_event_ext* dev_ext = G.dev_ext;
    const sg_arg* dev_args = G.dev_args;
    uint32_t *out = G.out, *dev_out = G.dev_out, *vin = G.vin;
    const uint32_t skip_min = G.skip_min, lane_max = G.lane_max, mb = G.mb;
    const bool ext = G.ext, host_out = G.host_out, force_lane = G.force_lane;
    (void)n_args;
    const uint32_t* head = B.h_head;
    const uint32_t m = head[1];
    const uint32_t nprev = head[3];
    int64_t t0 = 0;
    std::memcpy(&t0, head + 4, 8);
    const uint32_t bflags = head[0];
    const uint32_t* off = head + 8;
    uint32_t bin_n[N_BINS];
    for (int b = 0; b < N_BINS; ++b) bin_n[b] = off[b + 1] - off[b];
    DevCfg dc;
    std::memset(&dc, 0, sizeof(dc));
    dc.max_rt = e->cfg.statistic_max_rt;
    dc.occupy_timeout = e->cfg.occupy_timeout_ms;
// ... 26 lines not shown
    S.gbase = G.gbase;
    S.link = e->d_link;
    S.bst = e->d_bst;
    S.pend = e->d_pend;
    S.spans = e->d_spans;
    S.nspan = e->d_bsmall + 120;
    S.span_cap = e->span_cap;
    S.epoch = G.epoch;
    S.skip_ok = !(bflags & (BF_MULTI_LINK | BF_ZERO_CNT)) && !(e->dbg_flags & 4) ? 1u : 0u;
    S.skip_min = skip_min;
    S.ext = dev_ext;
    S.args = dev_args;
    S.aux_tab = e->d_auxtab;
    S.aux_count = e->d_auxcnt;
    S.aux_cap = e->cfg.aux_node_capacity;
    S.aux_mask = e->aux_mask;
    S.max_ctx = SG_MAX_CONTEXTS;
    S.auth = dev_auth(e);
    S.auth_ids = dev_auth_ids(e);
    HIPCHK(hipStreamWaitEvent(st, B.ev[1], 0));
    const uint32_t n_mix = e->has_mix ? head[6] : 0u, n_mixw = e->has_mix ? head[7] : 0u;
    const bool serial_bins = (e->dbg_flags & 8) != 0;
    const bool pre_split = (n_mix || n_mixw) && !serial_bins;
    hipStream_t ps = pre_split ? e->bin_stream[1] : st;
    const uint32_t grant_all = (e->cfg.switch_on && e->cfg.max_slot_chain_size <= 0) ? 1u : 0u;
    if (n_mixw && (e->pv_on || e->pvt_on) && head[72]) {
        if (int prc = ensure_pv(e, head[72], n_mixw)) return prc;
        e->pv_last_m = n_mixw;
    }
    const bool pv_ran = n_mixw && e->pv_on && head[72];
    const bool pv_early = pv_ran && pre_split && grant_all && !e->has_multi;
    if (pv_early) {
        HIPCHK(hipStreamWaitEvent(ps, B.ev[1], 0));
        HIPCHK(launch_pv_a(e->d_recs, vin, e->d_segs, B.d_mix + B.mix_cap, n_mixw, S, dc, e->d_dec, e->d_pvseg, e->pvb,
                           head[72], e->d_pvtot, e->d_pvhist, e->d_pvpart, ps, launch_radix_hist_n,
                           launch_radix_scatter_n, launch_scan, radix_tile(), e->d_pvrest, grant_all));
    }
    HIPCHK(launch_resolve(e->d_prev, nprev, e->d_ring, e->d_recs, vin, dev_ext, st));
    if (e->cfg.switch_on && (e->cfg.max_slot_chain_size <= 0 || e->n_chains < (uint32_t)e->cfg.max_slot_chain_size)) {
        const bool grant_all = e->cfg.max_slot_chain_size <= 0;
        HIPCHK(launch_chain(e->d_recs, vin, e->d_segs, m, e->d_info, grant_all ? 1 : 0, e->d_bsmall + 2, e->d_cand,
                            dev_ev, e->d_prog, dev_ext, SG_MAX_CONTEXTS, st));
        if (!grant_all) {
            uint32_t ncand = 0;
            HIPCHK(hipMemcpyAsync(&ncand, e->d_bsmall + 2, 4, hipMemcpyDeviceToHost, st));
            HIPCHK(hipStreamSynchronize(st));
            if (ncand) {
                std::vector<uint64_t> cand(ncand);
                HIPCHK(hipMemcpy(cand.data(), e->d_cand, ncand * 8ull, hipMemcpyDeviceToHost));
                std::sort(cand.begin(), cand.end());
                std::vector<uint64_t> upd;
                std::unordered_map<uint32_t, int> seen;
                for (uint32_t i = 0; i < ncand; ++i) {
                    uint32_t res = (uint32_t)cand[i];
                    if (!seen.emplace(res, 1).second) continue;
                    bool grant = e->n_chains < (uint32_t)e->cfg.max_slot_chain_size;
                    if (grant) e->n_chains++;
                    upd.push_back(((uint64_t)(grant ? NI_CHAIN : NI_REJECTED) << 32) | res | (1ull << 63));
                }
                ncand = (uint32_t)upd.size();
                HIPCHK(hipMemcpyAsync(e->d_cand, upd.data(), ncand * 8ull, hipMemcpyHostToDevice, st));
                HIPCHK(launch_set_flags(e->d_info, e->d_cand, ncand, st));
                HIPCHK(hipStreamSynchronize(st));
            }
        }
    }
    if (pre_split) {
        HIPCHK(hipEventRecord(e->fork0, st));
        HIPCHK(hipStreamWaitEvent(ps, e->fork0, 0));
    }
    if (pv_ran && !pv_early)
// ... 99 lines not shown
            HIPCHK(launch_decide_bin(BIN_J1, e->d_recs, dev_ev, vin, e->d_segs, e->d_order + off[BIN_J1] + (c ? h : 0),
                                     c ? bin_n[BIN_J1] - h : h, Sj, dc, t0, e->d_dec, e->d_bsmall + 0, bs));
            HIPCHK(hipEventRecord(e->join[c], bs));
        }
    } else if (bin_n[BIN_J1]) {
        DevState Sj = S;
        Sj.dbg = (e->prof_bin == 2 && e->d_dbg) ? e->d_dbg : nullptr;
        hipStream_t bs = j1_b0 ? e->bin_stream[0] : st;
        if (j1_b0 && !(bin_n[BIN_J16] || bin_n[BIN_J8] || bin_n[BIN_PQ16])) HIPCHK(hipStreamWaitEvent(bs, e->fork, 0));
        HIPCHK(launch_decide_bin(BIN_J1, e->d_recs, dev_ev, vin, e->d_segs, e->d_order + off[BIN_J1], bin_n[BIN_J1], Sj, dc,
                                 t0, e->d_dec, e->d_bsmall + 0, bs));
        if (j1_b0) HIPCHK(hipEventRecord(e->join[0], bs));
    }
    for (int c = 0; c < 2; ++c)
        if (bin_n[coop[c]] || bin_n[c == 0 ? BIN_PQ16 : BIN_PQ4] || (c == 0 && (j8_own || j1_b0)) || j1_split)
            HIPCHK(hipStreamWaitEvent(st, e->join[c], 0));
    if (S.skip_ok && (bin_n[BIN_J16] || bin_n[BIN_J8] || bin_n[BIN_J4]))
        HIPCHK(launch_fill(e->d_spans, S.nspan, e->span_cap, e->d_recs, e->d_prog, e->d_rules, e->d_dec, st));
    if (n_mixw && e->pvt_on && head[72])
        HIPCHK(launch_pvt(e->d_recs, dev_ev, vin, e->d_segs, B.d_mix + B.mix_cap, n_mixw, S, dc, e->d_dec,
                          e->d_bsmall + 0, e->d_pvtseg, e->pvbt, head[72], e->d_pvtot + 4, e->d_pvthist, e->d_pvtpart, st,
                          launch_radix_hist_n, launch_radix_scatter_n, launch_scan, radix_tile(),
                          e->d_pvrest + e->pvseg_cap + 1));
    const bool pvt_ran = n_mixw && e->pvt_on && head[72];
    uint32_t* prest = e->d_pvrest + e->pvseg_cap + 1;
    if (n_mix || n_mixw)
        HIPCHK(launch_pq_mix(1, e->d_recs, dev_ev, vin, e->d_segs, B.d_mix, n_mix, B.mix_cap, n_mixw, S, dc, t0,
                             e->d_dec, e->d_bsmall + 0, st, pvt_ran ? prest + 1 : nullptr, prest));
    if (ext)
        HIPCHK(launch_aux(e->d_recs, e->d_segs, e->d_bsmall + 130, aux_early ? nullptr : B.d_ashort, B.d_along, B.d_apiece,
                          B.d_amulti, S, dc, t0, e->d_dec, e->d_auxpool, e->auxpool_cap, e->d_bsmall + 134, e->d_auxmeta,
                          e->d_bsmall + 0, st));
    HIPCHK(hipEventRecord(B.ev[3], st));
    if (B.radix) HIPCHK(launch_post(e->d_posof, e->d_dec, n, G.gbase, e->d_ring, ring_mask, dev_out, st));
    else HIPCHK(launch_post_w(e->d_flag, e->d_pos, B.nhot, e->d_dec, n, G.gbase, e->d_ring, ring_mask, dev_out, st));
    if (host_out) HIPCHK(hipMemcpyAsync(out, dev_out, n * 4, hipMemcpyDeviceToHost, st));
    HIPCHK(hipMemcpyAsync(e->h_mirror + (size_t)G.set * MIRROR_WORDS, e->d_bsmall, MIRROR_WORDS * 4, hipMemcpyDeviceToHost,
                          st));
    HIPCHK(hipEventRecord(B.ev[4], st));
    B.last_post = B.ev[4];
    return SG_OK;
}

static int submit_impl(sg_engine* e, const sg_event* ev, const sg_event_ext* ext, uint64_t n, const sg_arg* args,
                       uint64_t n_args, uint32_t* out) {
    if (!e || (n && (!ev || !out))) return fail(SG_EINVAL, "null argument");
    if (n_args && !args) return fail(SG_EINVAL, "null args table");
    if (!e->fatal.empty()) return fail(SG_ESTATE, e->fatal + " -- engine unusable, recreate it");
    if (n == 0) return SG_OK;
    if (n > e->cfg.max_batch_events || n >= (1ull << 31)) return fail(SG_EINVAL, "batch larger than max_batch_events");
    HIPCHK(hipSetDevice(e->device));
    if (e->held_rc) return drain(e);
    const bool late = e->handoff_late && e->pipeline && e->cfg.max_slot_chain_size <= 0;
    int rc;
    if (n > e->cap_n && (rc = drain(e))) return rc;
    if ((rc = ensure_batch(e, n))) return rc;
    if ((rc = ensure_pool2(e))) return rc;
    int prev = e->grouped;
    if (prev >= 0 && (rc = accept_grouped(e))) return rc;
    auto give_up = [&](int why) -> int {
        if (prev >= 0) {
            const std::string msg = g_err;
            const int pk = prev;
            prev = -1;
            if (decide_stage(e, pk) == SG_OK) g_err = msg;
        }
        return why;
    };
    const unsigned long long pfloor = e->h_pool_next ? e->h_pool_next[PC_FLOOR] : 0;
    const bool compact = e->pool_nb && e->h_pool_next[PC_NEXT] > pfloor + (e->pool_nb - pfloor) / 2;
    if (!late || compact) {
        if (prev >= 0) {
            const int pk = prev;
// ... 702 lines not shown
```

### sentinel_amd/csrc/kernels.hip

```cpp
#include <hip/hip_runtime.h>
#include <stdint.h>
#include <stdlib.h>

#include "../../include/sentinel_gpu.h"
#include "authority.h"
#include "dev_types.h"

using namespace sg;

#define WAVE 64

#define RS_THREADS 256
#ifndef RS_ITEMS
#define RS_ITEMS 16
#endif
#define RS_TILE (RS_THREADS * RS_ITEMS)
#define RS_BINS 256

template <int DB>
__device__ __forceinline__ void hist_add(uint32_t* h, uint32_t d, bool valid) {
    uint64_t peers = __ballot(valid);
#pragma unroll
    for (int b = 0; b < DB; ++b) {
        const uint64_t bb = __ballot((d >> b) & 1);
        peers &= ((d >> b) & 1) ? bb : ~bb;
    }
    const int l = threadIdx.x & 63;
    const uint64_t lt = (l == 0) ? 0ull : (~0ull >> (64 - l));
    if (valid && (peers & lt) == 0) atomicAdd(&h[d], (uint32_t)__popcll(peers));
}

template <int DB>
__global__ __launch_bounds__(RS_THREADS) void k_rs_first(const sg_event* __restrict__ ev, uint64_t n, uint32_t max_res,
                                                      uint64_t gbase, const uint8_t* __restrict__ ring,
                                                      uint64_t ring_mask, int32_t max_rt, SEv* __restrict__ rec_o,
                                                      uint32_t* __restrict__ keys, uint32_t* __restrict__ vals,
                                                      uint32_t* __restrict__ ghist, uint32_t nblocks,
                                                      uint32_t* __restrict__ bflags, int64_t* __restrict__ t0_out,
                                                      uint32_t* __restrict__ prio, uint64_t* __restrict__ key_ring,
                                                      const uint32_t* __restrict__ comp,
                                                      const sg_event_ext* __restrict__ ext,
                                                      const sg_arg* __restrict__ args, uint64_t n_args,
                                                      uint32_t max_ctx, const AuthDesc* __restrict__ auth,
                                                      const uint32_t* __restrict__ auth_ids) {
    constexpr int NB = 1 << DB;
    __shared__ uint32_t h[NB];
    for (int i = threadIdx.x; i < NB; i += RS_THREADS) h[i] = 0;
    __syncthreads();
    const int64_t t0 = ev[0].ts;
// ... 68 lines not shown
            if (e.kind == SG_EV_EXIT) {
                const int64_t raw = (int64_t)(e.aux >> 48);
                r.rt = (uint16_t)(raw > max_rt ? max_rt : raw);
                if (own_args && key_ring) key_ring[(gbase + i) & ring_mask] = key0;
            }
            const uint64_t ref = e.aux & SG_REF_NONE;
            if (ref != SG_REF_NONE) {
                if (ref >= gbase) {
                    if (ref - gbase >= i) fl |= BF_BAD_REF;
                    else { r.code = RC_BATCH; r.x = (uint32_t)(ref - gbase); }
                } else {
                    r.code = RC_PREV;
                    r.x = (uint32_t)(ref & ring_mask);
                }
            }
        }
        if (mark && e.res_id < max_res && (prio[e.res_id] & mark) != mark) atomicOr(&prio[e.res_id], mark);
        rec_o[i] = r;
        const uint32_t key = (comp && e.res_id < max_res) ? comp[e.res_id] : e.res_id;
        keys[i] = key;
        vals[i] = (uint32_t)i | (e.kind == SG_EV_ENTRY ? 0x80000000u : 0u);
        hkey[it] = key;
    }
#pragma unroll
    for (int it = 0; it < RS_ITEMS; ++it) {
        const uint64_t i = base + (uint64_t)it * RS_THREADS + threadIdx.x;
        hist_add<DB>(h, hkey[it] & (NB - 1), i < n);
    }
    if (fl) atomicOr(bflags, fl);
    __syncthreads();
    for (int b = threadIdx.x; b < NB; b += RS_THREADS) ghist[(uint64_t)b * nblocks + blockIdx.x] = h[b];
}

#define HOT_MAX 1024u
#define HOT_NONE 0xFFFFu
#define W_HOT 0x80000000u
#define W_ENT 0x40000000u
#define W_POS 0x3FFFFFFFu

template <int DB>
__global__ __launch_bounds__(RS_THREADS) void k_grp_first(const sg_event* __restrict__ ev, uint64_t n, uint32_t max_res,
                                                       uint64_t gbase, uint64_t ring_mask, uint32_t* __restrict__ bflags,
                                                       int64_t* __restrict__ t0_out, uint32_t* __restrict__ prio,
                                                       uint64_t* __restrict__ key_ring, const uint32_t* __restrict__ comp,
                                                       const sg_event_ext* __restrict__ ext, const sg_arg* __restrict__ args,
                                                       uint64_t n_args, uint32_t max_ctx,
                                                       const AuthDesc* __restrict__ auth,
                                                       const uint32_t* __restrict__ auth_ids,
                                                       const uint16_t* __restrict__ hot_tab, uint32_t nhot,
                                                       uint32_t nblocks, uint32_t* __restrict__ words,
                                                       uint32_t* __restrict__ hot_hist, uint32_t* __restrict__ ckeys,
                                                       uint32_t* __restrict__ cvals, uint32_t* __restrict__ ccnt,
                                                       uint32_t* __restrict__ chist) {
    constexpr int NB = 1 << DB;
    __shared__ uint32_t wcnt[4][HOT_MAX];
    __shared__ uint32_t h[NB];
    __shared__ uint32_t cw[4];
    const int w = threadIdx.x >> 6, l = threadIdx.x & 63;
    for (int i = threadIdx.x; i < NB; i += RS_THREADS) h[i] = 0;
    for (uint32_t i = threadIdx.x; i < 4 * HOT_MAX; i += RS_THREADS) (&wcnt[0][0])[i] = 0;
    __syncthreads();
    const int64_t t0 = ev[0].ts;
    if (blockIdx.x == 0 && threadIdx.x == 0) *t0_out = t0;
    const uint64_t base = (uint64_t)blockIdx.x * RS_TILE;
    const uint64_t wbase = base + (uint64_t)w * (RS_TILE / 4);
    const uint64_t lt = (l == 0) ? 0ull : (~0ull >> (64 - l));
    uint32_t fl = 0;
    uint32_t kk[RS_ITEMS], rk[RS_ITEMS];
    uint32_t hotm = 0, entm = 0;
    uint32_t ccount = 0;
#pragma unroll
    for (int it = 0; it < RS_ITEMS; ++it) {
        const uint64_t i = wbase + (uint64_t)it * WAVE + l;
        const bool valid = i < n;
        uint32_t key = 0, hid = HOT_NONE;
        if (valid) {
            const sg_event e = ev[i];
            if (e.res_id >= max_res) fl |= BF_BAD_RES;
            const int64_t dt = e.ts - t0;
            if (dt < 0 || dt > 0x7FFFFFFFLL) fl |= (dt < 0 ? BF_BACKWARD : BF_TSPAN);
            if (i > 0 && ev[i - 1].ts > e.ts) fl |= BF_BACKWARD;
            uint32_t mark = 0;
            uint64_t key0 = (e.flags & SG_F_HAS_ARG) ? e.aux : NO_KEY;
            bool own_args = false;
            if (ext) {
                const sg_event_ext x = ext[i];
                if (x.n_args > SG_MAX_ARGS || (uint64_t)x.arg_off + x.n_args > n_args) fl |= BF_BAD_ARGS;
                else if (x.n_args) {
                    for (uint32_t k = 0; k < x.n_args; ++k) {
                        const sg_arg a = args[x.arg_off + k];
                        if (a.kind > SG_ARG_LIST || (a.kind == SG_ARG_LIST && (a.key > n_args || a.len > n_args - a.key)))
                            fl |= BF_BAD_ARGS;
                        else if (a.kind == SG_ARG_LIST) {
                            mark |= PM_ARGL;
                            for (uint32_t q = 0; q < a.len; ++q)
                                if (args[a.key + q].kind > SG_ARG_SCALAR) fl |= BF_BAD_ARGS;
                        }
// ... 62 lines not shown
    uint32_t coff = 0;
    for (int ww = 0; ww < w; ++ww) coff += cw[ww];
    if (threadIdx.x == 0) ccnt[blockIdx.x] = cw[0] + cw[1] + cw[2] + cw[3];
    for (int b = threadIdx.x; b < NB; b += RS_THREADS) chist[(uint64_t)b * nblocks + blockIdx.x] = h[b];
    __syncthreads();
#pragma unroll
    for (int it = 0; it < RS_ITEMS; ++it) {
        const uint64_t i = wbase + (uint64_t)it * WAVE + l;
        if (i >= n) continue;
        const uint32_t ent = ((entm >> it) & 1) ? W_ENT : 0u;
        if ((hotm >> it) & 1) {
            const uint32_t hid = rk[it] >> 16;
            words[i] = W_HOT | ent | (hid << 12) | (wcnt[w][hid] + (rk[it] & 0xFFFFu));
        } else {
            words[i] = ent;
            const uint64_t o = base + coff + rk[it];
            ckeys[o] = kk[it];
            cvals[o] = (uint32_t)i | (((entm >> it) & 1) ? 0x80000000u : 0u);
        }
    }
}

#define HS_TC 16u
__global__ __launch_bounds__(256) void k_hot_scan_a(const uint32_t* __restrict__ C, uint32_t nblocks, uint32_t nhot,
                                                    uint32_t* __restrict__ part) {
    const uint32_t c = blockIdx.x, t0 = c * HS_TC, t1 = min(nblocks, t0 + HS_TC);
    for (uint32_t h = threadIdx.x; h < nhot; h += 256) {
        uint32_t a = 0;
        for (uint32_t t = t0; t < t1; ++t) a += C[(uint64_t)t * nhot + h];
        part[(uint64_t)c * nhot + h] = a;
    }
}
__global__ __launch_bounds__(HOT_MAX) void k_hot_scan_b(uint32_t* __restrict__ part, uint32_t nch, uint32_t nhot,
                                                        uint32_t* __restrict__ hb, uint32_t* __restrict__ out) {
    __shared__ uint32_t ws[HOT_MAX / 64];
    const uint32_t h = threadIdx.x, l = h & 63, wv = h >> 6;
    uint32_t tot = 0;
    if (h < nhot) {
        constexpr uint32_t U = 16;
        uint32_t c = 0;
        for (; c + U <= nch; c += U) {
            uint32_t v[U];
#pragma unroll
            for (uint32_t k = 0; k < U; ++k) v[k] = part[(uint64_t)(c + k) * nhot + h];
#pragma unroll
            for (uint32_t k = 0; k < U; ++k) {
                part[(uint64_t)(c + k) * nhot + h] = tot;
                tot += v[k];
            }
        }
        for (; c < nch; ++c) {
            const uint32_t v = part[(uint64_t)c * nhot + h];
            part[(uint64_t)c * nhot + h] = tot;
            tot += v;
        }
    }
    uint32_t x = tot;
#pragma unroll
    for (int o = 1; o < 64; o <<= 1) {
        const uint32_t y = __shfl_up(x, o, 64);
        if ((int)l >= o) x += y;
    }
    if (l == 63) ws[wv] = x;
    __syncthreads();
    uint32_t pre = 0, all = 0;
    for (uint32_t k = 0; k < HOT_MAX / 64; ++k) { if (k < wv) pre += ws[k]; all += ws[k]; }
    if (h < nhot) { hb[h] = pre + x - tot; hb[HOT_MAX + h] = tot; }
    if (h == 0) *out = all;
}
__global__ __launch_bounds__(256) void k_hot_scan_c(uint32_t* __restrict__ C, uint32_t nblocks, uint32_t nhot,
                                                    const uint32_t* __restrict__ part, const uint32_t* __restrict__ hb) {
    const uint32_t c = blockIdx.x, t0 = c * HS_TC, t1 = min(nblocks, t0 + HS_TC);
    for (uint32_t h = threadIdx.x; h < nhot; h += 256) {
        uint32_t run = hb[h] + part[(uint64_t)c * nhot + h];
        for (uint32_t t = t0; t < t1; ++t) {
            const uint32_t v = C[(uint64_t)t * nhot + h];
            C[(uint64_t)t * nhot + h] = run;
            run += v;
        }
    }
}

#define BE_THREADS 1024
#define BE_ITEMS 8
__global__ __launch_bounds__(BE_THREADS) void k_bkt_edges(const sg_event* __restrict__ ev, uint32_t nblocks,
                                                          uint32_t* __restrict__ edges) {
    __shared__ uint32_t ws[BE_THREADS / 64];
    const uint32_t t = threadIdx.x, l = t & 63, wv = t >> 6;
    uint32_t run = 0;
    for (uint32_t c0 = 0; c0 < nblocks; c0 += BE_THREADS * BE_ITEMS) {
        const uint32_t t0 = c0 + t * BE_ITEMS;
        int64_t ts[BE_ITEMS + 1];
#pragma unroll
        for (int k = 0; k <= BE_ITEMS; ++k) {
            uint32_t tl = (t0 + k) ? t0 + k - 1 : 0u;
            if (tl >= nblocks) tl = nblocks - 1;
            ts[k] = ev[(uint64_t)tl * RS_TILE].ts;
        }
        uint32_t f = 0;
#pragma unroll
        for (int k = 0; k < BE_ITEMS; ++k)
            if (t0 + k < nblocks && (t0 + k == 0 || ts[k + 1] / 500 != ts[k] / 500)) f |= 1u << k;
        const uint32_t c = (uint32_t)__popc(f);
        uint32_t x = c;
#pragma unroll
        for (int o = 1; o < 64; o <<= 1) {
            const uint32_t y = __shfl_up(x, o, 64);
            if ((int)l >= o) x += y;
        }
        if (l == 63) ws[wv] = x;
        __syncthreads();
        uint32_t pre = 0, all = 0;
        for (uint32_t k = 0; k < BE_THREADS / 64; ++k) { if (k < wv) pre += ws[k]; all += ws[k]; }
        uint32_t o = 1 + run + pre + x - c;
#pragma unroll
        for (int k = 0; k < BE_ITEMS; ++k)
            if ((f >> k) & 1u) edges[o++] = t0 + k;
        run += all;
        __syncthreads();
    }
    if (t == 0) edges[0] = run;
}
#define BM_EDGES 32u
__global__ __launch_bounds__(256) void k_hot_bmax(const uint32_t* __restrict__ P, uint32_t nblocks, uint32_t nhot,
                                                  const uint32_t* __restrict__ hb, const uint32_t* __restrict__ edges,
                                                  uint32_t* __restrict__ bmax) {
    const uint32_t ne = edges[0], j0 = blockIdx.y * BM_EDGES, j1 = min(ne, j0 + BM_EDGES);
    const uint32_t h = blockIdx.x * 256 + threadIdx.x;
    if (j0 >= ne || h >= nhot) return;
    const uint32_t end = hb[h] + hb[HOT_MAX + h];
    uint32_t m = 0;
    for (uint32_t j = j0; j < j1; ++j) {
        const uint32_t a = edges[1 + j], b = j + 1 < ne ? edges[2 + j] : nblocks;
        const uint32_t lo = P[(uint64_t)(a ? a - 1 : 0u) * nhot + h];
        const uint32_t hi = b < nblocks ? P[(uint64_t)b * nhot + h] : end;
        m = max(m, hi - lo);
    }
    if (m) atomicMax(&bmax[h], m);
}

__device__ __forceinline__ uint32_t grp_pos(uint64_t j, uint32_t wd, const uint32_t* __restrict__ P, uint32_t nhot) {
    if (wd & W_HOT) return P[(j / RS_TILE) * nhot + ((wd >> 12) & (HOT_MAX - 1))] + (wd & 0xFFFu);
    return wd & W_POS;
}

#define GR_THREADS 256
#define GR_EVENTS (RS_TILE / 4)
#define GR_ITEMS (GR_EVENTS / GR_THREADS)
__global__ __launch_bounds__(GR_THREADS) void k_grp_records(const sg_event* __restrict__ ev, uint64_t n,
                                                            uint64_t gbase, uint64_t ring_mask, int32_t max_rt,
                                                            const uint32_t* __restrict__ words,
                                                            const uint32_t* __restrict__ P, uint32_t nhot,
                                                            uint32_t nblocks, const uint32_t* __restrict__ hb,
                                                            SEv* __restrict__ recs,
                                                            uint32_t* __restrict__ svals, uint32_t* __restrict__ prev,
                                                            uint32_t* __restrict__ nprev, uint32_t* __restrict__ bst,
                                                            uint32_t* __restrict__ bflags,
                                                            const sg_event_ext* __restrict__ ext,
                                                            const sg_arg* __restrict__ args, uint32_t max_ctx,
                                                            Link* __restrict__ link, uint32_t epoch,
                                                            const uint32_t* __restrict__ need_hot,
                                                            const uint32_t* __restrict__ need_blk) {
    __shared__ uint4 srec[GR_EVENTS];
    __shared__ uint32_t spos[GR_EVENTS], sval[GR_EVENTS];
    __shared__ uint32_t lo[HOT_MAX];
    __shared__ uint32_t r0[HOT_MAX];
    __shared__ uint32_t prow[HOT_MAX];
    __shared__ uint8_t hneed[HOT_MAX];
    __shared__ uint32_t ws[GR_THREADS / 64];
    __shared__ uint32_t nh_q;
    const uint32_t t = threadIdx.x, l = t & 63, wv = t >> 6;
    const uint32_t tile = blockIdx.x >> 2;
    const uint64_t base = (uint64_t)tile * RS_TILE + (uint64_t)(blockIdx.x & 3) * GR_EVENTS;
    sg_event e[GR_ITEMS];
    uint32_t wd[GR_ITEMS];
#pragma unroll
// ... 222 lines not shown
__global__ __launch_bounds__(256) void k_post_w(const uint32_t* __restrict__ words, const uint32_t* __restrict__ P,
                                                uint32_t nhot, const uint32_t* __restrict__ dec, uint64_t n,
                                                uint64_t gbase, uint8_t* __restrict__ ring, uint64_t ring_mask,
                                                uint32_t* __restrict__ out) {
    const uint64_t base = (uint64_t)blockIdx.x * (256 * POSTW_ITEMS) + threadIdx.x;
    uint32_t w[POSTW_ITEMS], d[POSTW_ITEMS];
#pragma unroll
    for (int k = 0; k < POSTW_ITEMS; ++k) {
        const uint64_t i = base + (uint64_t)k * 256;
        w[k] = i < n ? words[i] : 0u;
    }
    uint32_t pr[POSTW_ITEMS];
#pragma unroll
    for (int k = 0; k < POSTW_ITEMS; ++k) {
        const uint64_t i = base + (uint64_t)k * 256;
        pr[k] = P[(w[k] & W_HOT) ? (i / RS_TILE) * nhot + ((w[k] >> 12) & (HOT_MAX - 1)) : 0];
    }
#pragma unroll
    for (int k = 0; k < POSTW_ITEMS; ++k) {
        const uint32_t q = (w[k] & W_HOT) ? pr[k] + (w[k] & 0xFFFu) : (w[k] & W_POS);
        const uint32_t x = dec[(w[k] & W_ENT) ? q : 0u];
        d[k] = (w[k] & W_ENT) ? x : (uint32_t)ST_NOT_ENTRY;
    }
#pragma unroll
    for (int k = 0; k < POSTW_ITEMS; ++k) {
        const uint64_t i = base + (uint64_t)k * 256;
        if (i < n) {
            out[i] = d[k];
            ring[(gbase + i) & ring_mask] = (uint8_t)(d[k] & 0xFF);
        }
    }
}

__global__ __launch_bounds__(HOT_MAX) void k_hot_segs(const uint32_t* __restrict__ hb, uint32_t nhot,
                                                      const uint32_t* __restrict__ hot_list, Seg* __restrict__ segs,
                                                      uint32_t* __restrict__ out) {
    __shared__ uint32_t ws[HOT_MAX / 64];
    const uint32_t t = threadIdx.x, l = t & 63, wv = t >> 6;
    const uint32_t len = t < nhot ? hb[HOT_MAX + t] : 0u;
    const uint32_t f = len ? 1u : 0u;
    uint32_t x = f;
#pragma unroll
    for (int o = 1; o < 64; o <<= 1) {
        const uint32_t y = __shfl_up(x, o, 64);
        if ((int)l >= o) x += y;
    }
    if (l == 63) ws[wv] = x;
    __syncthreads();
    uint32_t pre = 0, all = 0;
    for (uint32_t k = 0; k < HOT_MAX / 64; ++k) { if (k < wv) pre += ws[k]; all += ws[k]; }
    if (f) {
        Seg sg;
        sg.res = hot_list[t];
        sg.start = hb[t];
        sg.len = 0;
        sg.bin = 0;
        segs[pre + x - f] = sg;
    }
    if (t == 0) out[0] = all;
}

__global__ void k_hot_clear(uint16_t* __restrict__ hot_tab, const uint32_t* __restrict__ hot_list, uint32_t nhot) {
    const uint32_t t = blockIdx.x * blockDim.x + threadIdx.x;
    if (t < nhot) hot_tab[hot_list[t]] = (uint16_t)HOT_NONE;
}
__global__ __launch_bounds__(256) void k_hot_build(const Seg* __restrict__ segs, const uint32_t* __restrict__ mp,
                                                   uint32_t min_len, uint32_t max_res, uint16_t* __restrict__ hot_tab,
                                                   uint32_t* __restrict__ hot_list, uint32_t* __restrict__ hot_n) {
    const uint32_t s = blockIdx.x * blockDim.x + threadIdx.x;
    if (s >= *mp || segs[s].len < min_len || segs[s].res >= max_res) return;
    const uint32_t k = atomicAdd(hot_n, 1u);
    if (k >= HOT_MAX) return;
    const uint32_t r = segs[s].res;
    hot_tab[r] = (uint16_t)k;
    hot_list[k] = r;
}

template <int DB>
__global__ __launch_bounds__(RS_THREADS) void k_radix_hist(const uint32_t* __restrict__ keys, uint64_t n, int shift,
                                                        uint32_t* __restrict__ ghist, uint32_t nblocks,
                                                        const uint32_t* __restrict__ ndev) {
    constexpr int NB = 1 << DB;
    if (ndev && *ndev < n) n = *ndev;
    __shared__ uint32_t h[NB];
    for (int i = threadIdx.x; i < NB; i += RS_THREADS) h[i] = 0;
    __syncthreads();
    const uint64_t base = (uint64_t)blockIdx.x * RS_TILE;
#pragma unroll
    for (int it = 0; it < RS_ITEMS; ++it) {
        const uint64_t i = base + (uint64_t)it * RS_THREADS + threadIdx.x;
        hist_add<DB>(h, i < n ? (keys[i] >> shift) & (NB - 1) : 0u, i < n);
    }
    __syncthreads();
    for (int b = threadIdx.x; b < NB; b += RS_THREADS) ghist[(uint64_t)b * nblocks + blockIdx.x] = h[b];
// ... 121 lines not shown

__global__ __launch_bounds__(SC_THREADS) void k_scan_reduce(const uint32_t* __restrict__ in, uint64_t n, uint32_t* __restrict__ part,
                                                         const uint32_t* __restrict__ ndev) {
    if (ndev && *ndev < n) n = *ndev;
    uint64_t base = (uint64_t)blockIdx.x * SC_TILE;
    if (base >= n) {
        if (threadIdx.x == 0) part[blockIdx.x] = 0;
        return;
    }
    uint32_t s = 0;
    for (int it = 0; it < SC_ITEMS; ++it) {
        uint64_t i = base + (uint64_t)it * SC_THREADS + threadIdx.x;
        if (i < n) s += in[i];
    }
    uint32_t tot;
    block_excl_scan(s, &tot);
    if (threadIdx.x == 0) part[blockIdx.x] = tot;
}

__global__ __launch_bounds__(SC_THREADS) void k_scan_top(uint32_t* __restrict__ part, uint32_t nparts, uint32_t* __restrict__ total_out) {
    uint32_t carry = 0;
    for (uint32_t base = 0; base < nparts; base += SC_THREADS) {
        uint32_t i = base + threadIdx.x;
        uint32_t v = i < nparts ? part[i] : 0;
        uint32_t tot;
        uint32_t ex = block_excl_scan(v, &tot);
        if (i < nparts) part[i] = carry + ex;
        carry += tot;
        __syncthreads();
    }
    if (threadIdx.x == 0 && total_out) *total_out = carry;
}

__global__ __launch_bounds__(SC_THREADS) void k_scan_down(const uint32_t* __restrict__ in, uint64_t n, const uint32_t* __restrict__ part,
                                                       uint32_t* __restrict__ out, const uint32_t* __restrict__ ndev) {
    if (ndev && *ndev < n) n = *ndev;
    if ((uint64_t)blockIdx.x * SC_TILE >= n) return;
    uint64_t base = (uint64_t)blockIdx.x * SC_TILE + (uint64_t)threadIdx.x * SC_ITEMS;
    uint32_t loc[SC_ITEMS];
    uint32_t s = 0;
    #pragma unroll
    for (int k = 0; k < SC_ITEMS; ++k) {
        uint64_t i = base + k;
        loc[k] = i < n ? in[i] : 0;
        s += loc[k];
    }
    uint32_t ex = block_excl_scan(s, nullptr) + part[blockIdx.x];
    #pragma unroll
    for (int k = 0; k < SC_ITEMS; ++k) {
        uint64_t i = base + k;
        if (i < n) out[i] = ex;
        ex += loc[k];
    }
}

__device__ __forceinline__ bool snap_valid(const Bkt& b, int64_t now, int64_t cur, int64_t last) {
    if (b.ws < 0 || now - b.ws > 60000) return false;
    int64_t rt = b.succ != 0 ? b.rt / b.succ : b.rt;
    bool in_time = b.ws > last && b.ws < cur;
    bool nz = b.pass > 0 || b.block > 0 || b.succ > 0 || b.exc > 0 || rt > 0 || b.occ > 0;
    return in_time && nz;
}

__global__ void k_snap_count(Bkt* __restrict__ minb, const NodeInfo* __restrict__ info, uint32_t nres, int64_t now,
                             int32_t max_rt, uint32_t* __restrict__ cnt) {
    uint32_t r = blockIdx.x * blockDim.x + threadIdx.x;
    if (r >= nres) return;
    if (!(info[r].flags & NI_CHAIN)) { cnt[r] = 0; return; }
    int64_t cur = now - now % 1000;
    int slot = (int)((now / 1000) % 60);
    Bkt& c = minb[(uint64_t)r * 60 + slot];
    if (c.ws < cur) {
        c.ws = cur; c.pass = 0; c.block = 0; c.exc = 0; c.succ = 0; c.rt = 0; c.occ = 0; c.minrt = max_rt;
    }
    int64_t last = info[r].last_fetch;
    uint32_t k = 0;
    for (int s = 0; s < 60; ++s) if (snap_valid(minb[(uint64_t)r * 60 + s], now, cur, last)) ++k;
    cnt[r] = k;
}

// ... 77 lines not shown
                       (const uint32_t*)nullptr);
    return hipGetLastError();
}
hipError_t launch_radix_hist_n(const uint32_t* keys, uint64_t n, const uint32_t* ndev, int shift, uint32_t* ghist,
                               uint32_t nblocks, hipStream_t st) {
    hipLaunchKernelGGL(k_radix_hist<8>, dim3(nblocks), dim3(RS_THREADS), 0, st, keys, n, shift, ghist, nblocks, ndev);
    return hipGetLastError();
}
hipError_t launch_radix_scatter_n(const uint32_t* kin, const uint32_t* vin, uint64_t n, const uint32_t* ndev, int shift,
                                  const uint32_t* goff, uint32_t nblocks, uint32_t* kout, uint32_t* vout, hipStream_t st) {
    hipLaunchKernelGGL(k_radix_scatter<8>, dim3(nblocks), dim3(RS_THREADS), 0, st, kin, vin, n, shift, goff, nblocks,
                       kout, vout, (uint32_t*)nullptr, ndev, (const uint32_t*)nullptr, (const uint32_t*)nullptr, 0u);
    return hipGetLastError();
}
hipError_t launch_radix_scatter(const uint32_t* kin, const uint32_t* vin, uint64_t n, int shift, const uint32_t* goff,
                                uint32_t nblocks, uint32_t* kout, uint32_t* vout, uint32_t* pos_of, hipStream_t st) {
    hipLaunchKernelGGL(k_radix_scatter<8>, dim3(nblocks), dim3(RS_THREADS), 0, st, kin, vin, n, shift, goff, nblocks,
                       kout, vout, pos_of, (const uint32_t*)nullptr, (const uint32_t*)nullptr, (const uint32_t*)nullptr, 0u);
    return hipGetLastError();
}
hipError_t launch_radix_scatter_x(const uint32_t* kin, const uint32_t* vin, uint64_t n, const uint32_t* ndev,
                                  const uint32_t* tcnt, const uint32_t* dbase, int shift, const uint32_t* goff,
                                  uint32_t nblocks, uint32_t* kout, uint32_t* vout, uint32_t* pos_of, hipStream_t st) {
    hipLaunchKernelGGL(k_radix_scatter<8>, dim3(nblocks), dim3(RS_THREADS), 0, st, kin, vin, n, shift, goff, nblocks,
                       kout, vout, pos_of, ndev, tcnt, dbase, 1u);
    return hipGetLastError();
}
hipError_t launch_grp_first(const sg_event* ev, uint64_t n, uint32_t max_res, uint64_t gbase, uint64_t ring_mask,
                            uint32_t* bflags, int64_t* t0_out, uint32_t* prio, uint64_t* key_ring, const uint32_t* comp,
                            const sg_event_ext* ext, const sg_arg* args, uint64_t n_args, uint32_t max_ctx,
                            const AuthDesc* auth, const uint32_t* auth_ids,
                            const uint16_t* hot_tab, uint32_t nhot, uint32_t nblocks, uint32_t* words,
                            uint32_t* hot_hist, uint32_t* ckeys, uint32_t* cvals, uint32_t* ccnt, uint32_t* chist,
                            hipStream_t st) {
    hipLaunchKernelGGL(k_grp_first<8>, dim3(nblocks), dim3(RS_THREADS), 0, st, ev, n, max_res, gbase, ring_mask, bflags,
                       t0_out, prio, key_ring, comp, ext, args, n_args, max_ctx, auth, auth_ids, hot_tab, nhot, nblocks, words,
                       hot_hist, ckeys, cvals, ccnt, chist);
    return hipGetLastError();
}
hipError_t launch_hot_scan(uint32_t* C, uint32_t nblocks, uint32_t nhot, uint32_t* part, uint32_t* hb, uint32_t* total,
                           hipStream_t st) {
    if (!nhot) return hipMemsetAsync(total, 0, 4, st);
    const uint32_t nch = (nblocks + HS_TC - 1) / HS_TC;
    hipLaunchKernelGGL(k_hot_scan_a, dim3(nch), dim3(256), 0, st, C, nblocks, nhot, part);
    hipLaunchKernelGGL(k_hot_scan_b, dim3(1), dim3(HOT_MAX), 0, st, part, nch, nhot, hb, total);
    hipLaunchKernelGGL(k_hot_scan_c, dim3(nch), dim3(256), 0, st, C, nblocks, nhot, part, hb);
    return hipGetLastError();
}
hipError_t launch_hot_bmax(const sg_event* ev, uint32_t nblocks, const uint32_t* P, uint32_t nhot, const uint32_t* hb,
                           uint32_t* edges, uint32_t* bmax, hipStream_t st) {
    if (!nhot || !nblocks) return hipSuccess;
    hipLaunchKernelGGL(k_bkt_edges, dim3(1), dim3(BE_THREADS), 0, st, ev, nblocks, edges);
    hipLaunchKernelGGL(k_hot_bmax, dim3((nhot + 255) / 256, (nblocks + BM_EDGES - 1) / BM_EDGES), dim3(256), 0, st, P,
                       nblocks, nhot, hb, edges, bmax);
    return hipGetLastError();
}
hipError_t launch_grp_records(const sg_event* ev, uint64_t n, uint64_t gbase, uint64_t ring_mask, int32_t max_rt,
                              const uint32_t* words, const uint32_t* P, uint32_t nhot, uint32_t nblocks,
                              const uint32_t* hb, SEv* recs, uint32_t* svals, uint32_t* prev,
                              uint32_t* nprev, uint32_t* bst, uint32_t* bflags, const sg_event_ext* ext,
                              const sg_arg* args, uint32_t max_ctx, Link* link, uint32_t epoch,
                              const uint32_t* need_hot, const uint32_t* need_blk, hipStream_t st) {
    hipLaunchKernelGGL(k_grp_records, dim3(nblocks * 4), dim3(GR_THREADS), 0, st, ev, n, gbase, ring_mask, max_rt, words, P,
                       nhot, nblocks, hb, recs, svals, prev, nprev, bst, bflags, ext, args, max_ctx, link, epoch, need_hot,
                       need_blk);
    return hipGetLastError();
}
hipError_t launch_hot_segs(const uint32_t* hb, uint32_t nhot, const uint32_t* hot_list, Seg* segs, uint32_t* out,
                           hipStream_t st) {
    hipLaunchKernelGGL(k_hot_segs, dim3(1), dim3(HOT_MAX), 0, st, hb, nhot, hot_list, segs, out);
    return hipGetLastError();
}
hipError_t launch_hot_build(const Seg* segs, const uint32_t* mp, uint32_t mb, uint32_t min_len, uint32_t max_res, uint16_t* hot_tab,
                            uint32_t* hot_list, uint32_t nhot_old, uint32_t* hot_n, hipStream_t st) {
    if (nhot_old) hipLaunchKernelGGL(k_hot_clear, dim3((nhot_old + 255) / 256), dim3(256), 0, st, hot_tab, hot_list, nhot_old);
    if (mb) hipLaunchKernelGGL(k_hot_build, dim3((mb + 255) / 256), dim3(256), 0, st, segs, mp, min_len, max_res, hot_tab,
                               hot_list, hot_n);
    return hipGetLastError();
}
__global__ void k_cold_n(uint64_t n, const uint32_t* __restrict__ hot_total, uint32_t* __restrict__ out) {
    if (threadIdx.x == 0) *out = (uint32_t)(n - *hot_total);
}
hipError_t launch_cold_n(uint64_t n, const uint32_t* hot_total, uint32_t* out, hipStream_t st) {
    hipLaunchKernelGGL(k_cold_n, dim3(1), dim3(64), 0, st, n, hot_total, out);
    return hipGetLastError();
}
uint32_t hot_max() { return HOT_MAX; }

__global__ void k_grp_clear(uint32_t* __restrict__ bsmall, uint32_t nsmall, uint32_t* __restrict__ bst, uint32_t nbst,
                            uint32_t* __restrict__ need, uint32_t nneed) {
    const uint32_t i = blockIdx.x * blockDim.x + threadIdx.x;
    if (i < nsmall) bsmall[i] = 0;
    if (i < nbst) bst[i] = 0;
    if (i < nneed) need[i] = 0;
}
hipError_t launch_grp_clear(uint32_t* bsmall, uint32_t nsmall, uint32_t* bst, uint32_t nbst, uint32_t* need,
                            uint32_t nneed, hipStream_t st) {
    uint32_t m = nsmall > nbst ? nsmall : nbst;
    if (nneed > m) m = nneed;
    hipLaunchKernelGGL(k_grp_clear, dim3((m + 255) / 256), dim3(256), 0, st, bsmall, nsmall, bst, nbst, need, nneed);
    return hipGetLastError();
}

__global__ __launch_bounds__(1024) void k_cold_small(const uint32_t* __restrict__ kin, const uint32_t* __restrict__ vin,
                                                     const uint32_t* __restrict__ cnt_p, const uint32_t* __restrict__ dbase,
                                                     uint32_t* __restrict__ kout, uint32_t* __restrict__ vout,
                                                     uint32_t* __restrict__ words) {
    __shared__ unsigned long long s[RS_TILE];
    const uint32_t cnt = *cnt_p, ob = *dbase, t = threadIdx.x;
    uint32_t n2 = 1;
    while (n2 < cnt) n2 <<= 1;
    for (uint32_t i = t; i < n2; i += blockDim.x)
        s[i] = i < cnt ? (((unsigned long long)kin[i] << 32) | i) : ~0ull;
    __syncthreads();
    for (uint32_t k = 2; k <= n2; k <<= 1)
        for (uint32_t j = k >> 1; j > 0; j >>= 1) {
            for (uint32_t i = t; i < n2; i += blockDim.x) {
// ... 34 lines not shown
hipError_t launch_set_flags(NodeInfo* info, const uint64_t* upd, uint32_t n, hipStream_t st) {
    if (!n) return hipSuccess;
    hipLaunchKernelGGL(k_set_flags, dim3((n + 255) / 256), dim3(256), 0, st, info, upd, n);
    return hipGetLastError();
}

hipError_t launch_region_copy(const uint64_t* src, uint64_t* dst, const uint64_t* tri, uint32_t n, hipStream_t st) {
    if (!n) return hipSuccess;
    hipLaunchKernelGGL(k_region_copy, dim3(n), dim3(256), 0, st, src, dst, tri);
    return hipGetLastError();
}

__global__ __launch_bounds__(SC_THREADS) void k_scan_one(const uint32_t* __restrict__ in, uint64_t n,
                                                      uint32_t* __restrict__ out, uint32_t* __restrict__ total) {
    const uint64_t base = (uint64_t)threadIdx.x * SC_ITEMS;
    uint32_t loc[SC_ITEMS];
    uint32_t s = 0;
#pragma unroll
    for (int k = 0; k < SC_ITEMS; ++k) {
        const uint64_t i = base + k;
        loc[k] = i < n ? in[i] : 0;
        s += loc[k];
    }
    uint32_t tot;
    uint32_t ex = block_excl_scan(s, &tot);
#pragma unroll
    for (int k = 0; k < SC_ITEMS; ++k) {
        const uint64_t i = base + k;
        if (i < n) out[i] = ex;
        ex += loc[k];
    }
    if (threadIdx.x == 0 && total) *total = tot;
}
hipError_t launch_scan(const uint32_t* in, uint32_t* out, uint64_t n, uint32_t* part, uint32_t* total,
                       hipStream_t st) {
    if (n <= SC_TILE) {
        hipLaunchKernelGGL(k_scan_one, dim3(1), dim3(SC_THREADS), 0, st, in, n, out, total);
        return hipGetLastError();
    }
    uint32_t nb = (uint32_t)((n + SC_TILE - 1) / SC_TILE);
    if (nb == 0) nb = 1;
    hipLaunchKernelGGL(k_scan_reduce, dim3(nb), dim3(SC_THREADS), 0, st, in, n, part, (const uint32_t*)nullptr);
    hipLaunchKernelGGL(k_scan_top, dim3(1), dim3(SC_THREADS), 0, st, part, nb, total);
    hipLaunchKernelGGL(k_scan_down, dim3(nb), dim3(SC_THREADS), 0, st, in, n, part, out, (const uint32_t*)nullptr);
    return hipGetLastError();
}
hipError_t launch_scan_n(const uint32_t* in, uint32_t* out, uint64_t n, const uint32_t* ndev, uint32_t* part,
                         uint32_t* total, hipStream_t st) {
    uint32_t nb = (uint32_t)((n + SC_TILE - 1) / SC_TILE);
    if (nb == 0) nb = 1;
    hipLaunchKernelGGL(k_scan_reduce, dim3(nb), dim3(SC_THREADS), 0, st, in, n, part, ndev);
    hipLaunchKernelGGL(k_scan_top, dim3(1), dim3(SC_THREADS), 0, st, part, nb, total);
    hipLaunchKernelGGL(k_scan_down, dim3(nb), dim3(SC_THREADS), 0, st, in, n, part, out, ndev);
    return hipGetLastError();
}

hipError_t launch_snapshot(Bkt* minb, NodeInfo* info, uint32_t nres, int64_t now, int32_t max_rt, uint32_t* cnt,
                           uint32_t* off, uint32_t* part, uint32_t* total, sg_metric_node* outp, uint64_t cap,
                           hipStream_t st) {
    uint32_t nb = (nres + 255) / 256;
    hipLaunchKernelGGL(k_snap_count, dim3(nb), dim3(256), 0, st, minb, info, nres, now, max_rt, cnt);
    hipError_t e = launch_scan(cnt, off, nres, part, total, st);
    if (e != hipSuccess) return e;
    hipLaunchKernelGGL(k_snap_emit, dim3(nb), dim3(256), 0, st, minb, info, nres, now, off, outp, cap);
    return hipGetLastError();
}

}
```

Baseline: 4.730 billion.

## Fold small helper kernels into neighbours and overlap post stage across batches

Several tiny single-thread kernels (add2, bin_offsets, cold_n, hot_segs, scan_top) are folded into adjacent kernels, and the three-pass scan becomes two passes when the tile count is small. Resolve now reads the previous batch's decision directly instead of waiting for its ring write. Scratch buffers rotate across batches, and a separate post stream with early slot release is added. The aim is to cut launch count and inter-batch serialization, at the cost of more host-side bookkeeping and cross-batch state that could go stale.

```diff
diff --git a/sentinel_amd/csrc/decide.hip b/sentinel_amd/csrc/decide.hip
--- a/sentinel_amd/csrc/decide.hip
+++ b/sentinel_amd/csrc/decide.hip
@@ -82,8 +82,10 @@
 }
 __global__ __launch_bounds__(256) void k_seg_emit(const uint32_t* __restrict__ keys, uint64_t n,
                                                   const uint32_t* __restrict__ off, Seg* __restrict__ segs,
-                                                  const uint32_t* __restrict__ lo, const uint32_t* __restrict__ sbase) {
+                                                  const uint32_t* __restrict__ lo, const uint32_t* __restrict__ sbase,
+                                                  const uint32_t* __restrict__ ccount, uint32_t* __restrict__ nseg) {
     const uint64_t b = lo ? *lo : 0u;
+    if (nseg && blockIdx.x == 0 && threadIdx.x == 0) *nseg = *sbase + *ccount;
     if ((uint64_t)(blockIdx.x + 1) * SEG_TILE <= b) return;
     uint32_t kk[SEG_ITEMS];
     const uint64_t i0 = (uint64_t)blockIdx.x * SEG_TILE + (uint64_t)threadIdx.x * SEG_ITEMS;
@@ -223,8 +225,9 @@
 }
 __global__ __launch_bounds__(256) void k_seg_order(Seg* __restrict__ segs, const uint32_t* __restrict__ mp,
                                                    const uint32_t* __restrict__ off, uint32_t nblk,
-                                                   uint32_t* __restrict__ order) {
+                                                   uint32_t* __restrict__ order, uint32_t* __restrict__ bin_off) {
     const uint32_t s = blockIdx.x * blockDim.x + threadIdx.x;
+    if (blockIdx.x == 0 && threadIdx.x <= N_BINS) bin_off[threadIdx.x] = threadIdx.x < N_BINS ? off[(uint64_t)threadIdx.x * nblk] : *mp;
     if (s >= *mp) return;
     const uint32_t v = segs[s].bin, bin = v & 0x3F;
     order[off[(uint64_t)bin * nblk + blockIdx.x] + (v >> SEG_RANK_SHIFT)] = s;
@@ -318,12 +321,27 @@
     }
 }
 __global__ void k_resolve(const uint32_t* __restrict__ prev, uint32_t np, const uint8_t* __restrict__ ring,
-                          SEv* __restrict__ recs, const uint32_t* __restrict__ vals, const sg_event_ext* __restrict__ ext) {
+                          SEv* __restrict__ recs, const uint32_t* __restrict__ vals, const sg_event_ext* __restrict__ ext,
+                          uint32_t pbase, uint32_t pmask, uint32_t pn, const uint32_t* __restrict__ pdec,
+                          const uint32_t* __restrict__ pwords, const uint32_t* __restrict__ pP, uint32_t pnhot,
+                          const uint32_t* __restrict__ ppos_of) {
     const uint32_t i = blockIdx.x * blockDim.x + threadIdx.x;
     if (i >= np) return;
     const uint32_t p = prev[i];
     SEv r = recs[p];
-    const uint8_t st = ring[r.x];
+    const uint32_t j = (r.x - pbase) & pmask;
+    uint8_t st;
+    if (j < pn) {
+        if (ppos_of) {
+            const uint32_t po = ppos_of[j];
+            st = (po & 0x80000000u) ? (uint8_t)(pdec[po & 0x7FFFFFFFu] & 0xFF) : (uint8_t)ST_NOT_ENTRY;
+        } else {
+            const uint32_t wd = pwords[j];
+            st = (wd & W_ENT) ? (uint8_t)(pdec[grp_pos(j, wd, pP, pnhot)] & 0xFF) : (uint8_t)ST_NOT_ENTRY;
+        }
+    } else {
+        st = ring[r.x];
+    }
     if (st == ST_NOT_ENTRY) r.code = r.kind == SG_EV_EXIT ? RC_NONE : RC_NOT;
     else r.code = (st == ST_PASS || st == ST_PASS_WAIT) ? RC_PASSED : RC_NOT;
     r.x = 0;
@@ -3647,11 +3665,8 @@
     hipError_t e = scan(flag, pos, nt, part, nseg, st);
     if (e != hipSuccess) return e;
     hipLaunchKernelGGL(k_seg_emit, dim3(nt), dim3(256), 0, st, keys, n, pos, segs, (const uint32_t*)nullptr,
-                       (const uint32_t*)nullptr);
+                       (const uint32_t*)nullptr, (const uint32_t*)nullptr, (uint32_t*)nullptr);
     return hipGetLastError();
-}
-__global__ void k_add2(uint32_t* __restrict__ dst, const uint32_t* __restrict__ a, const uint32_t* __restrict__ b) {
-    if (threadIdx.x == 0) *dst = *a + *b;
 }
 hipError_t launch_seg_cold(const uint32_t* keys, uint64_t n, const uint32_t* lo, const uint32_t* sbase, uint32_t* flag,
                            uint32_t* pos, Seg* segs, hipStream_t st,
@@ -3661,8 +3676,7 @@
     hipLaunchKernelGGL(k_seg_count, dim3(nt), dim3(256), 0, st, keys, n, flag, lo);
     hipError_t e = scan(flag, pos, nt, part, ccount, st);
     if (e != hipSuccess) return e;
-    hipLaunchKernelGGL(k_seg_emit, dim3(nt), dim3(256), 0, st, keys, n, pos, segs, lo, sbase);
-    hipLaunchKernelGGL(k_add2, dim3(1), dim3(64), 0, st, nseg, sbase, ccount);
+    hipLaunchKernelGGL(k_seg_emit, dim3(nt), dim3(256), 0, st, keys, n, pos, segs, lo, sbase, (const uint32_t*)ccount, nseg);
     return hipGetLastError();
 }
 hipError_t launch_block_sums(const SEv* recs, uint64_t n, uint32_t* bst, Link* link, uint32_t epoch, uint32_t* bflags,
@@ -3688,8 +3702,8 @@
 hipError_t launch_seg_order(Seg* segs, const uint32_t* mp, uint32_t mb, const uint32_t* off, uint32_t* order,
                             uint32_t* bin_off, hipStream_t st) {
     const uint32_t nblk = (mb + 255) / 256;
-    if (nblk) hipLaunchKernelGGL(k_seg_order, dim3(nblk), dim3(256), 0, st, segs, mp, off, nblk, order);
-    hipLaunchKernelGGL(k_bin_offsets, dim3(1), dim3(64), 0, st, off, nblk ? nblk : 1, mp, bin_off);
+    if (nblk) hipLaunchKernelGGL(k_seg_order, dim3(nblk), dim3(256), 0, st, segs, mp, off, nblk, order, bin_off);
+    else hipLaunchKernelGGL(k_bin_offsets, dim3(1), dim3(64), 0, st, off, 1u, mp, bin_off);
     return hipGetLastError();
 }
 hipError_t launch_gather(const SEv* rec_o, const uint32_t* vals, const uint32_t* skeys, uint64_t n,
@@ -3710,9 +3724,12 @@
     return hipGetLastError();
 }
 hipError_t launch_resolve(const uint32_t* prev, uint32_t np, const uint8_t* ring, SEv* recs, const uint32_t* vals,
-                          const sg_event_ext* ext, hipStream_t st) {
+                          const sg_event_ext* ext, uint32_t pbase, uint32_t pmask, uint32_t pn, const uint32_t* pdec,
+                          const uint32_t* pwords, const uint32_t* pP, uint32_t pnhot, const uint32_t* ppos_of,
+                          hipStream_t st) {
     if (!np) return hipSuccess;
-    hipLaunchKernelGGL(k_resolve, dim3((np + 255) / 256), dim3(256), 0, st, prev, np, ring, recs, vals, ext);
+    hipLaunchKernelGGL(k_resolve, dim3((np + 255) / 256), dim3(256), 0, st, prev, np, ring, recs, vals, ext, pbase, pmask,
+                       pn, pdec, pwords, pP, pnhot, ppos_of);
     return hipGetLastError();
 }
 hipError_t launch_post(const uint32_t* pos_of, const uint32_t* dec, uint64_t n, uint64_t gbase, uint8_t* ring,
diff --git a/sentinel_amd/csrc/dev_types.h b/sentinel_amd/csrc/dev_types.h
--- a/sentinel_amd/csrc/dev_types.h
+++ b/sentinel_amd/csrc/dev_types.h
@@ -170,6 +170,7 @@
 
 #define HEAD_OFF 16384u
 #define TABLES_ALL 32768u
+#define SCAN_THREE 131072u
 #define LITE_CHECK 65536u
 struct DevCfg {
     int32_t max_rt;
@@ -402,6 +403,20 @@
     RC_PREV = 4
 };
 
+#define RS_THREADS 256
+#ifndef RS_ITEMS
+#define RS_ITEMS 16
+#endif
+#define RS_TILE (RS_THREADS * RS_ITEMS)
+#define HOT_MAX 1024u
+#define W_HOT 0x80000000u
+#define W_ENT 0x40000000u
+#define W_POS 0x3FFFFFFFu
+__device__ __forceinline__ uint32_t grp_pos(uint64_t j, uint32_t wd, const uint32_t* __restrict__ P, uint32_t nhot) {
+    if (wd & W_HOT) return P[(j / RS_TILE) * nhot + ((wd >> 12) & (HOT_MAX - 1))] + (wd & 0xFFFu);
+    return wd & W_POS;
+}
+
 enum : uint32_t {
     BIN_J16 = 0,
     BIN_J4 = 1,
diff --git a/sentinel_amd/csrc/engine.cpp b/sentinel_amd/csrc/engine.cpp
--- a/sentinel_amd/csrc/engine.cpp
+++ b/sentinel_amd/csrc/engine.cpp
@@ -45,22 +45,20 @@
                             const AuthDesc* auth, const uint32_t* auth_ids,
                             const uint16_t* hot_tab, uint32_t nhot, uint32_t nblocks, uint32_t* words,
                             uint32_t* hot_hist, uint32_t* ckeys, uint32_t* cvals, uint32_t* ccnt, uint32_t* chist,
-                            hipStream_t st);
+                            int64_t* tfirst, hipStream_t st);
 hipError_t launch_hot_scan(uint32_t* C, uint32_t nblocks, uint32_t nhot, uint32_t* part, uint32_t* hb, uint32_t* total,
+                           uint64_t n, uint32_t* cold, const uint32_t* hot_list, Seg* segs, uint32_t* nseg,
                            hipStream_t st);
-hipError_t launch_hot_bmax(const sg_event* ev, uint32_t nblocks, const uint32_t* P, uint32_t nhot, const uint32_t* hb,
-                           uint32_t* edges, uint32_t* bmax, hipStream_t st);
+hipError_t launch_hot_bmax(const int64_t* tfirst, uint32_t nblocks, const uint32_t* P, uint32_t nhot, const uint32_t* hb,
+                           uint32_t* bmax, hipStream_t st);
 hipError_t launch_grp_records(const sg_event* ev, uint64_t n, uint64_t gbase, uint64_t ring_mask, int32_t max_rt,
                               const uint32_t* words, const uint32_t* P, uint32_t nhot, uint32_t nblocks,
                               const uint32_t* hb, SEv* recs, uint32_t* svals, uint32_t* prev,
                               uint32_t* nprev, uint32_t* bst, uint32_t* bflags, const sg_event_ext* ext,
                               const sg_arg* args, uint32_t max_ctx, Link* link, uint32_t epoch,
                               const uint32_t* need_hot, const uint32_t* need_blk, hipStream_t st);
-hipError_t launch_hot_segs(const uint32_t* hb, uint32_t nhot, const uint32_t* hot_list, Seg* segs, uint32_t* out,
-                           hipStream_t st);
 hipError_t launch_hot_build(const Seg* segs, const uint32_t* mp, uint32_t mb, uint32_t min_len, uint32_t max_res, uint16_t* hot_tab,
                             uint32_t* hot_list, uint32_t nhot_old, uint32_t* hot_n, hipStream_t st);
-hipError_t launch_cold_n(uint64_t n, const uint32_t* hot_total, uint32_t* out, hipStream_t st);
 hipError_t launch_cold_small(const uint32_t* kin, const uint32_t* vin, const uint32_t* cnt, const uint32_t* dbase,
                              uint32_t* kout, uint32_t* vout, uint32_t* words, hipStream_t st);
 uint32_t hot_max();
@@ -76,6 +74,7 @@
                                 uint32_t nblocks, uint32_t* kout, uint32_t* vout, uint32_t* pos_of, hipStream_t st);
 uint32_t radix_tile();
 hipError_t launch_scan(const uint32_t*, uint32_t*, uint64_t, uint32_t*, uint32_t*, hipStream_t);
+void scan_force_three(bool on);
 hipError_t launch_snapshot(Bkt*, NodeInfo*, uint32_t, int64_t, int32_t, uint32_t*, uint32_t*, uint32_t*, uint32_t*,
                            sg_metric_node*, uint64_t, hipStream_t);
 hipError_t launch_init_state(Bkt* sec, Bkt* minb, NodeInfo* info, int64_t* borrow, uint32_t nres, hipStream_t st);
@@ -144,7 +143,9 @@
 hipError_t launch_fill(const Span* spans, const uint32_t* nspan, uint32_t cap, const SEv* recs, const Prog* prog,
                        const DRule* rules, uint32_t* dec, hipStream_t st);
 hipError_t launch_resolve(const uint32_t* prev, uint32_t np, const uint8_t* ring, SEv* recs, const uint32_t* vals,
-                          const sg_event_ext* ext, hipStream_t st);
+                          const sg_event_ext* ext, uint32_t pbase, uint32_t pmask, uint32_t pn, const uint32_t* pdec,
+                          const uint32_t* pwords, const uint32_t* pP, uint32_t pnhot, const uint32_t* ppos_of,
+                          hipStream_t st);
 hipError_t launch_post_w(const uint32_t* words, const uint32_t* P, uint32_t nhot, const uint32_t* dec, uint64_t n,
                          uint64_t gbase, uint8_t* ring, uint64_t ring_mask, uint32_t* out, hipStream_t st);
 hipError_t launch_post(const uint32_t* pos_of, const uint32_t* dec, uint64_t n, uint64_t gbase, uint8_t* ring,
@@ -543,6 +544,7 @@
         uint32_t *d_bst = nullptr, *d_pend = nullptr;
         Span* d_spans = nullptr;
         hipEvent_t* ev = nullptr;
+        hipEvent_t last_mirror = nullptr;
         hipEvent_t last_post = nullptr;
         uint32_t* h_head = nullptr;
         struct Grouped {
@@ -563,12 +565,25 @@
     std::string held_msg;
     bool handoff_late = true;
     static constexpr int N_SETS = 4;
-    hipEvent_t evset[N_SETS][5] = {};
+    hipEvent_t evset[N_SETS][6] = {};
     uint32_t* h_mirror = nullptr;
     uint64_t seq = 0;
     struct InFlight { int set; uint32_t hot_marked; };
     std::deque<InFlight> inflight;
     hipStream_t gstream = nullptr;
+    bool post_stream = true;
+    bool slot_early = true;
+    int post_bin = -1;
+    hipEvent_t post_tail = nullptr;
+    static constexpr int N_ROT = 3;
+    uint32_t *r_flag[N_ROT] = {}, *r_pos[N_ROT] = {}, *r_posof[N_ROT] = {};
+    struct PrevLoc {
+        bool valid = false;
+        bool radix = false;
+        uint64_t gbase = 0, n = 0;
+        uint32_t nhot = 0;
+        const uint32_t *dec = nullptr, *words = nullptr, *P = nullptr, *posof = nullptr;
+    } prevloc;
     std::vector<std::array<double, 4>> tlog;
     std::vector<std::array<double, 2>> glog;
     std::string fatal;
@@ -580,7 +595,7 @@
     uint32_t* d_hot_hb = nullptr;
     uint32_t* d_need = nullptr;
     uint64_t need_words = 0;
-    uint32_t* d_edges = nullptr;
+    int64_t* d_tfirst = nullptr;
     uint32_t hot_marked_last = 0;
     bool radix_group = false;
     uint64_t radix_below = 1u << 18;
@@ -732,8 +747,8 @@
 }
 static void free_slot(sg_engine::BatchSlot& B) {
     dfree(B.d_ev); dfree(B.d_out); dfree(B.d_k0); dfree(B.d_v0); dfree(B.d_k1); dfree(B.d_v1);
-    dfree(B.d_hist); dfree(B.d_part); dfree(B.d_flag); dfree(B.d_pos); dfree(B.d_order); dfree(B.d_segs);
-    dfree(B.d_cand); dfree(B.d_posof); dfree(B.d_dec); dfree(B.d_recs); dfree(B.d_rec_o); dfree(B.d_blkcnt);
+    dfree(B.d_hist); dfree(B.d_part); dfree(B.d_order); dfree(B.d_segs);
+    dfree(B.d_cand); dfree(B.d_dec); dfree(B.d_recs); dfree(B.d_rec_o); dfree(B.d_blkcnt);
     dfree(B.d_prev); dfree(B.d_bsmall); dfree(B.d_ccnt);
     B.d_ccnt = nullptr;
     dfree(B.d_link); dfree(B.d_bst); dfree(B.d_pend); dfree(B.d_spans); dfree(B.d_ext); dfree(B.d_args);
@@ -750,6 +765,8 @@
     if (n <= e->cap_n) return SG_OK;
     uint64_t c = std::max<uint64_t>(n, 1u << 20);
     HIPCHK(hipStreamSynchronize(e->stream));
+    for (auto s : e->bin_stream)
+        if (s) HIPCHK(hipStreamSynchronize(s));
     uint64_t nblocks = (c + radix_tile() - 1) / radix_tile();
     e->cap_hist = nblocks * 256;
     for (auto& B : e->slot) {
@@ -762,25 +779,33 @@
         HIPCHK(hipMalloc(&B.d_v1, c * 4));
         HIPCHK(hipMalloc(&B.d_hist, e->cap_hist * 4));
         HIPCHK(hipMalloc(&B.d_part, (e->cap_hist / 4096 + c / 4096 + 64) * 4));
-        HIPCHK(hipMalloc(&B.d_flag, c * 4));
-        HIPCHK(hipMalloc(&B.d_pos, c * 4));
         HIPCHK(hipMalloc(&B.d_order, c * 4));
         HIPCHK(hipMalloc(&B.d_segs, c * sizeof(Seg)));
         HIPCHK(hipMalloc(&B.d_cand, c * 8));
-        HIPCHK(hipMalloc(&B.d_posof, c * 4));
         HIPCHK(hipMalloc(&B.d_dec, c * 4));
         HIPCHK(hipMalloc(&B.d_recs, c * sizeof(SEv)));
         const uint64_t co = (e->radix_group || c >= (1ull << 30)) ? c : std::min<uint64_t>(c, e->radix_below);
         if (co) HIPCHK(hipMalloc(&B.d_rec_o, co * sizeof(SEv)));
         HIPCHK(hipMalloc(&B.d_ccnt, 3 * (nblocks + 64) * 4));
     }
+    for (int r = 0; r < sg_engine::N_ROT; ++r) {
+        dfree(e->r_flag[r]); dfree(e->r_pos[r]); dfree(e->r_posof[r]);
+        e->r_flag[r] = e->r_pos[r] = e->r_posof[r] = nullptr;
+        HIPCHK(hipMalloc(&e->r_flag[r], c * 4));
+        HIPCHK(hipMalloc(&e->r_pos[r], c * 4));
+        HIPCHK(hipMalloc(&e->r_posof[r], c * 4));
+    }
+    for (int k = 0; k < 2; ++k) {
+        e->slot[k].d_flag = e->r_flag[k]; e->slot[k].d_pos = e->r_pos[k]; e->slot[k].d_posof = e->r_posof[k];
+    }
+    e->prevloc.valid = false;
     dfree(e->d_hot_part);
     dfree(e->d_hot_hb);
     dfree(e->d_need);
-    dfree(e->d_edges);
+    dfree(e->d_tfirst);
     e->need_words = hot_max() + c / 32768 + 2 + hot_max();
     HIPCHK(hipMalloc(&e->d_need, e->need_words * 4));
-    HIPCHK(hipMalloc(&e->d_edges, (nblocks + 2) * 4));
+    HIPCHK(hipMalloc(&e->d_tfirst, (nblocks + 2) * 8));
     HIPCHK(hipMalloc(&e->d_hot_part, (nblocks / 16 + 2) * hot_max() * 4));
     HIPCHK(hipMalloc(&e->d_hot_hb, 2 * hot_max() * 4));
     for (auto& B : e->slot) {
@@ -822,7 +847,7 @@
     if (collected > 0) {
         hipEvent_t* pv = e->evset[(f.set + sg_engine::N_SETS - 1) % sg_engine::N_SETS];
         if (hipEventElapsedTime(&ga, pv[1], ev[0]) != hipSuccess) ga = NAN;
-        if (hipEventElapsedTime(&gb, pv[4], ev[2]) != hipSuccess) gb = NAN;
+        if (hipEventElapsedTime(&gb, pv[3], ev[2]) != hipSuccess) gb = NAN;
         (void)hipGetLastError();
     }
     e->glog.push_back({(double)ga, (double)gb});
@@ -860,6 +885,10 @@
     note(handoff(e));
     while (!e->inflight.empty()) note(collect(e));
     HIPCHK(hipStreamSynchronize(e->stream));
+    for (auto s : e->bin_stream)
+        if (s) HIPCHK(hipStreamSynchronize(s));
+    e->prevloc.valid = false;
+    e->post_tail = nullptr;
     return rc ? fail(rc, msg) : SG_OK;
 }
 static void drain_hold(sg_engine* e) {
@@ -1255,6 +1284,9 @@
     if (hipStreamCreateWithPriority(&e->gstream, hipStreamNonBlocking, prio_lo) != hipSuccess) {
         return bad(fail(SG_EDEVICE, "stream"));
     }
+    if (const char* v = std::getenv("SG_POST_STREAM")) e->post_stream = v[0] != '0';
+    if (const char* v = std::getenv("SG_SLOT_EARLY")) e->slot_early = v[0] != '0';
+    if (const char* v = std::getenv("SG_POST_BIN")) e->post_bin = std::atoi(v);
     for (auto& s : e->evset)
         for (auto& v : s) if (hipEventCreate(&v) != hipSuccess) return bad(fail(SG_EDEVICE, "event"));
     for (auto& B : e->slot) {
@@ -1303,6 +1335,7 @@
     }
     if (const char* f = std::getenv("SG_DEBUG_FLAGS")) e->dbg_flags = (uint32_t)std::strtoul(f, nullptr, 0);
     e->radix_group = (e->dbg_flags & 8192) != 0;
+    scan_force_three((e->dbg_flags & SCAN_THREE) != 0);
     if (const char* f = std::getenv("SG_PROF_BIN")) e->prof_bin = std::atoi(f);
     if (const char* v = std::getenv("SG_LANE_MAX")) { e->lane_max = (uint32_t)std::strtoul(v, nullptr, 0); e->bins_pinned = true; }
     if (const char* v = std::getenv("SG_J1_MAX")) { e->j1_max = (uint32_t)std::strtoul(v, nullptr, 0); e->bins_pinned = true; }
@@ -1450,6 +1483,8 @@
     (void)hipSetDevice(e->device);
     e->grouped = -1;
     if (e->stream) (void)hipStreamSynchronize(e->stream);
+    for (auto s : e->bin_stream)
+        if (s) (void)hipStreamSynchronize(s);
     if (e->gstream) (void)hipStreamSynchronize(e->gstream);
     dfree(e->d_sec); dfree(e->d_minb); dfree(e->d_info); dfree(e->d_prog); dfree(e->d_rules); dfree(e->d_rstate);
     dfree(e->d_hot); dfree(e->d_pmap); dfree(e->d_pbkt); dfree(e->d_pdat); dfree(e->d_pbm); dfree(e->d_ppre); dfree(e->d_tmid); dfree(e->d_ring); dfree(e->d_small); dfree(e->d_sink);
@@ -1459,8 +1494,9 @@
     dfree(e->d_pvseg); dfree(e->d_pvtseg); dfree(e->d_pvtot); dfree(e->d_pvrest);
     if (e->gstream) (void)hipStreamSynchronize(e->gstream);
     for (auto& B : e->slot) free_slot(B);
+    for (int r = 0; r < sg_engine::N_ROT; ++r) { dfree(e->r_flag[r]); dfree(e->r_pos[r]); dfree(e->r_posof[r]); }
     dfree(e->d_auth); dfree(e->d_auth_ids);
-    dfree(e->d_prio); dfree(e->d_hot_tab); dfree(e->d_hot_list); dfree(e->d_hot_part); dfree(e->d_hot_hb); dfree(e->d_need); dfree(e->d_edges); dfree(e->d_comp); dfree(e->d_auxtab); dfree(e->d_auxpool); dfree(e->d_auxcnt); dfree(e->d_auxmeta);
+    dfree(e->d_prio); dfree(e->d_hot_tab); dfree(e->d_hot_list); dfree(e->d_hot_part); dfree(e->d_hot_hb); dfree(e->d_need); dfree(e->d_tfirst); dfree(e->d_comp); dfree(e->d_auxtab); dfree(e->d_auxpool); dfree(e->d_auxcnt); dfree(e->d_auxmeta);
     dfree(e->d_pflow); dfree(e->d_phot); dfree(e->d_pftab); dfree(e->d_pvtab); dfree(e->d_preq); dfree(e->d_pvals);
     dfree(e->d_cflow); dfree(e->d_cbkt); dfree(e->d_ctab); dfree(e->d_nslim); dfree(e->d_nslimit); dfree(e->d_nsb); dfree(e->d_borrow); dfree(e->d_keyring);
     dfree(e->d_treq); dfree(e->d_tres); dfree(e->d_tfidx); dfree(e->d_tbounds);
@@ -2385,11 +2421,21 @@
 
 static int group_stage(sg_engine* e, int k, const sg_event* ev, const sg_event_ext* ext, uint64_t n, const sg_arg* args,
                        uint64_t n_args, uint32_t* out, int* prev) {
+    auto& B = e->slot[k];
+    {
+        const int r = (int)(e->seq % sg_engine::N_ROT);
+        B.d_flag = e->r_flag[r]; B.d_pos = e->r_pos[r]; B.d_posof = e->r_posof[r];
+    }
     activate(e, k);
-    auto& B = e->slot[k];
     B.ev = e->evset[e->seq % sg_engine::N_SETS];
     hipStream_t gs = e->gstream;
-    if (B.last_post) HIPCHK(hipStreamWaitEvent(gs, B.last_post, 0));
+    const bool radix_next = e->radix_group || n >= (1ull << 30) || n < e->radix_below;
+    if (B.last_mirror && !radix_next && e->slot_early) {
+        HIPCHK(hipStreamWaitEvent(gs, B.last_mirror, 0));
+        if (e->seq >= 3) HIPCHK(hipStreamWaitEvent(gs, e->evset[(e->seq + 1) % sg_engine::N_SETS][4], 0));
+    } else if (B.last_post) {
+        HIPCHK(hipStreamWaitEvent(gs, B.last_post, 0));
+    }
     const sg_event* dev_ev = ev;
     bool host_in = !is_device_ptr(ev);
     bool host_out = !is_device_ptr(out);
@@ -2431,7 +2477,7 @@
     int64_t* d_t0 = reinterpret_cast<int64_t*>(e->d_bsmall + 4);
     uint32_t *kin = e->d_k1, *vin = e->d_v1, *kout = e->d_k0, *vout = e->d_v0;
     if (++e->epoch == 0) e->epoch = 1;
-    B.radix = e->radix_group || n >= (1ull << 30) || n < e->radix_below;
+    B.radix = radix_next;
     HIPCHK(launch_grp_clear(e->d_bsmall, 256, e->d_bst, B.radix ? 0u : (uint32_t)((n + 1023) / 1024), e->d_need,
                             B.radix ? 0u : (uint32_t)e->need_words, gs));
     const bool force_lane = !e->cfg.switch_on || (e->dbg_flags & 2);
@@ -2497,10 +2543,10 @@
         HIPCHK(launch_grp_first(dev_ev, n, R, e->gbase, ring_mask, e->d_bsmall + 0, d_t0, e->d_prio, e->d_keyring,
                                 e->d_comp, dev_ext, dev_args, n_args, SG_MAX_CONTEXTS, dev_auth(e), dev_auth_ids(e),
                                 e->d_hot_tab, nhot, nblocks,
-                                words, hot_off, e->d_k1, e->d_v1, ccnt, e->d_hist, gs));
+                                words, hot_off, e->d_k1, e->d_v1, ccnt, e->d_hist, e->d_tfirst, gs));
         if (int drc = decide_prev()) return drc;
-        HIPCHK(launch_hot_scan(hot_off, nblocks, nhot, e->d_hot_part, e->d_hot_hb, e->d_bsmall + 77, gs));
-        HIPCHK(launch_cold_n(n, e->d_bsmall + 77, e->d_bsmall + 78, gs));
+        HIPCHK(launch_hot_scan(hot_off, nblocks, nhot, e->d_hot_part, e->d_hot_hb, e->d_bsmall + 77, n, e->d_bsmall + 78,
+                               e->d_hot_list, e->d_segs, e->d_bsmall + 80, gs));
         if (nblocks == 1) {
             HIPCHK(launch_cold_small(kin, vin, ccnt, e->d_bsmall + 77, kout, vout, words, gs));
             std::swap(kin, kout);
@@ -2516,7 +2562,6 @@
             std::swap(kin, kout);
             std::swap(vin, vout);
         }
-        HIPCHK(launch_hot_segs(e->d_hot_hb, nhot, e->d_hot_list, e->d_segs, e->d_bsmall + 80, gs));
         const uint64_t sc = nblocks + 64;
         HIPCHK(launch_seg_cold(kin, n, e->d_bsmall + 77, e->d_bsmall + 80, ccnt + sc, ccnt + 2 * sc, e->d_segs, gs,
                                launch_scan, e->d_part, e->d_bsmall + 82, e->d_bsmall + 1));
@@ -2525,7 +2570,7 @@
             need_hot = e->d_need;
             need_blk = e->d_need + hot_max();
             bmax = e->d_need + e->need_words - hot_max();
-            HIPCHK(launch_hot_bmax(dev_ev, nblocks, hot_off, nhot, e->d_hot_hb, e->d_edges, bmax, gs));
+            HIPCHK(launch_hot_bmax(e->d_tfirst, nblocks, hot_off, nhot, e->d_hot_hb, bmax, gs));
         }
         if (int brc = bins(need_hot, need_blk, bmax)) return brc;
         HIPCHK(launch_grp_records(dev_ev, n, e->gbase, ring_mask, e->cfg.statistic_max_rt, words, hot_off, nhot, nblocks,
@@ -2557,6 +2602,8 @@
     const int k = e->grouped;
     auto& B = e->slot[k];
     e->grouped = -1;
+    const bool chained = e->prevloc.valid;
+    e->prevloc.valid = false;
     HIPCHK(hipEventSynchronize(B.ev[1]));
     const uint32_t* head = B.h_head;
     if (!B.radix) e->nhot = std::min<uint32_t>(head[76], hot_max());
@@ -2573,6 +2620,7 @@
     if (e->has_mix && head[7] && (e->pv_on || e->pvt_on) && head[72]) {
         if (int prc = ensure_pv(e, head[72], head[7])) return prc;
     }
+    e->prevloc.valid = chained;
     e->inflight.push_back({B.g.set, B.hot_marked});
     ++e->seq;
     e->last = k;
@@ -2594,6 +2642,7 @@
     const int rc = decide_enqueue(e, k);
     if (rc) {
         const std::string why = g_err;
+        e->prevloc.valid = false;
         if (!e->inflight.empty()) e->inflight.pop_back();
         if (e->fatal.empty()) e->fatal = "the decide stage of an accepted batch could not be enqueued (" + why + ")";
         return fail(rc, why);
@@ -2686,11 +2735,24 @@
     const bool pv_early = pv_ran && pre_split && grant_all && !e->has_multi;
     if (pv_early) {
         HIPCHK(hipStreamWaitEvent(ps, B.ev[1], 0));
+        if (e->post_stream && B.last_post) HIPCHK(hipStreamWaitEvent(ps, B.last_post, 0));
         HIPCHK(launch_pv_a(e->d_recs, vin, e->d_segs, B.d_mix + B.mix_cap, n_mixw, S, dc, e->d_dec, e->d_pvseg, e->pvb,
                            head[72], e->d_pvtot, e->d_pvhist, e->d_pvpart, ps, launch_radix_hist_n,
                            launch_radix_scatter_n, launch_scan, radix_tile(), e->d_pvrest, grant_all));
     }
-    HIPCHK(launch_resolve(e->d_prev, nprev, e->d_ring, e->d_recs, vin, dev_ext, st));
+    const auto& PL = e->prevloc;
+    const bool direct = e->post_stream && PL.valid && e->pipeline && e->cfg.max_slot_chain_size <= 0 &&
+                        PL.n <= ring_mask + 1 && ring_mask <= 0xFFFFFFFFull && PL.gbase + PL.n == G.gbase;
+    if (e->post_stream) {
+        if (direct) {
+            if (B.last_post) HIPCHK(hipStreamWaitEvent(st, B.last_post, 0));
+        } else if (e->post_tail) {
+            HIPCHK(hipStreamWaitEvent(st, e->post_tail, 0));
+        }
+    }
+    HIPCHK(launch_resolve(e->d_prev, nprev, e->d_ring, e->d_recs, vin, dev_ext, (uint32_t)(PL.gbase & ring_mask),
+                          (uint32_t)ring_mask, direct ? (uint32_t)PL.n : 0u, PL.dec, PL.radix ? nullptr : PL.words, PL.P,
+                          PL.nhot, PL.radix ? PL.posof : nullptr, st));
     if (e->cfg.switch_on && (e->cfg.max_slot_chain_size <= 0 || e->n_chains < (uint32_t)e->cfg.max_slot_chain_size)) {
         const bool grant_all = e->cfg.max_slot_chain_size <= 0;
         HIPCHK(launch_chain(e->d_recs, vin, e->d_segs, m, e->d_info, grant_all ? 1 : 0, e->d_bsmall + 2, e->d_cand,
@@ -2856,13 +2918,28 @@
                           B.d_amulti, S, dc, t0, e->d_dec, e->d_auxpool, e->auxpool_cap, e->d_bsmall + 134, e->d_auxmeta,
                           e->d_bsmall + 0, st));
     HIPCHK(hipEventRecord(B.ev[3], st));
-    if (B.radix) HIPCHK(launch_post(e->d_posof, e->d_dec, n, G.gbase, e->d_ring, ring_mask, dev_out, st));
-    else HIPCHK(launch_post_w(e->d_flag, e->d_pos, B.nhot, e->d_dec, n, G.gbase, e->d_ring, ring_mask, dev_out, st));
-    if (host_out) HIPCHK(hipMemcpyAsync(out, dev_out, n * 4, hipMemcpyDeviceToHost, st));
+    const int post_bin = (e->post_bin == 0 || e->post_bin == 1) ? e->post_bin : (pre_split ? 0 : 1);
+    hipStream_t pst = (e->post_stream && !serial_bins) ? e->bin_stream[post_bin] : st;
+    if (pst != st) {
+        HIPCHK(hipStreamWaitEvent(pst, B.ev[3], 0));
+        if (e->post_tail) HIPCHK(hipStreamWaitEvent(pst, e->post_tail, 0));
+    }
     HIPCHK(hipMemcpyAsync(e->h_mirror + (size_t)G.set * MIRROR_WORDS, e->d_bsmall, MIRROR_WORDS * 4, hipMemcpyDeviceToHost,
-                          st));
-    HIPCHK(hipEventRecord(B.ev[4], st));
+                          pst));
+    B.last_mirror = nullptr;
+    if (pst != st && !B.radix) {
+        HIPCHK(hipEventRecord(B.ev[5], pst));
+        B.last_mirror = B.ev[5];
+    }
+    if (B.radix) HIPCHK(launch_post(e->d_posof, e->d_dec, n, G.gbase, e->d_ring, ring_mask, dev_out, pst));
+    else HIPCHK(launch_post_w(e->d_flag, e->d_pos, B.nhot, e->d_dec, n, G.gbase, e->d_ring, ring_mask, dev_out, pst));
+    if (host_out) HIPCHK(hipMemcpyAsync(out, dev_out, n * 4, hipMemcpyDeviceToHost, pst));
+    HIPCHK(hipEventRecord(B.ev[4], pst));
     B.last_post = B.ev[4];
+    e->post_tail = B.ev[4];
+    auto& NL = e->prevloc;
+    NL.valid = true; NL.radix = B.radix; NL.gbase = G.gbase; NL.n = n; NL.nhot = B.nhot;
+    NL.dec = e->d_dec; NL.words = e->d_flag; NL.P = e->d_pos; NL.posof = e->d_posof;
     return SG_OK;
 }
 
diff --git a/sentinel_amd/csrc/kernels.hip b/sentinel_amd/csrc/kernels.hip
--- a/sentinel_amd/csrc/kernels.hip
+++ b/sentinel_amd/csrc/kernels.hip
@@ -10,11 +10,6 @@
 
 #define WAVE 64
 
-#define RS_THREADS 256
-#ifndef RS_ITEMS
-#define RS_ITEMS 16
-#endif
-#define RS_TILE (RS_THREADS * RS_ITEMS)
 #define RS_BINS 256
 
 template <int DB>
@@ -149,11 +144,7 @@
     for (int b = threadIdx.x; b < NB; b += RS_THREADS) ghist[(uint64_t)b * nblocks + blockIdx.x] = h[b];
 }
 
-#define HOT_MAX 1024u
 #define HOT_NONE 0xFFFFu
-#define W_HOT 0x80000000u
-#define W_ENT 0x40000000u
-#define W_POS 0x3FFFFFFFu
 
 template <int DB>
 __global__ __launch_bounds__(RS_THREADS) void k_grp_first(const sg_event* __restrict__ ev, uint64_t n, uint32_t max_res,
@@ -168,7 +159,7 @@
                                                        uint32_t nblocks, uint32_t* __restrict__ words,
                                                        uint32_t* __restrict__ hot_hist, uint32_t* __restrict__ ckeys,
                                                        uint32_t* __restrict__ cvals, uint32_t* __restrict__ ccnt,
-                                                       uint32_t* __restrict__ chist) {
+                                                       uint32_t* __restrict__ chist, int64_t* __restrict__ tfirst) {
     constexpr int NB = 1 << DB;
     __shared__ uint32_t wcnt[4][HOT_MAX];
     __shared__ uint32_t h[NB];
@@ -180,6 +171,7 @@
     const int64_t t0 = ev[0].ts;
     if (blockIdx.x == 0 && threadIdx.x == 0) *t0_out = t0;
     const uint64_t base = (uint64_t)blockIdx.x * RS_TILE;
+    if (threadIdx.x == 0) tfirst[blockIdx.x] = ev[base].ts;
     const uint64_t wbase = base + (uint64_t)w * (RS_TILE / 4);
     const uint64_t lt = (l == 0) ? 0ull : (~0ull >> (64 - l));
     uint32_t fl = 0;
@@ -308,7 +300,10 @@
     }
 }
 __global__ __launch_bounds__(HOT_MAX) void k_hot_scan_b(uint32_t* __restrict__ part, uint32_t nch, uint32_t nhot,
-                                                        uint32_t* __restrict__ hb, uint32_t* __restrict__ out) {
+                                                        uint32_t* __restrict__ hb, uint32_t* __restrict__ out, uint64_t n,
+                                                        uint32_t* __restrict__ cold_out,
+                                                        const uint32_t* __restrict__ hot_list, Seg* __restrict__ segs,
+                                                        uint32_t* __restrict__ nseg_out) {
     __shared__ uint32_t ws[HOT_MAX / 64];
     const uint32_t h = threadIdx.x, l = h & 63, wv = h >> 6;
     uint32_t tot = 0;
@@ -341,8 +336,30 @@
     __syncthreads();
     uint32_t pre = 0, all = 0;
     for (uint32_t k = 0; k < HOT_MAX / 64; ++k) { if (k < wv) pre += ws[k]; all += ws[k]; }
-    if (h < nhot) { hb[h] = pre + x - tot; hb[HOT_MAX + h] = tot; }
-    if (h == 0) *out = all;
+    const uint32_t first = pre + x - tot;
+    if (h < nhot) { hb[h] = first; hb[HOT_MAX + h] = tot; }
+    if (h == 0) { *out = all; *cold_out = (uint32_t)(n - all); }
+    __syncthreads();
+    const uint32_t f = (h < nhot && tot) ? 1u : 0u;
+    uint32_t y = f;
+#pragma unroll
+    for (int o = 1; o < 64; o <<= 1) {
+        const uint32_t z = __shfl_up(y, o, 64);
+        if ((int)l >= o) y += z;
+    }
+    if (l == 63) ws[wv] = y;
+    __syncthreads();
+    uint32_t spre = 0, sall = 0;
+    for (uint32_t k = 0; k < HOT_MAX / 64; ++k) { if (k < wv) spre += ws[k]; sall += ws[k]; }
+    if (f) {
+        Seg sg;
+        sg.res = hot_list[h];
+        sg.start = first;
+        sg.len = 0;
+        sg.bin = 0;
+        segs[spre + y - f] = sg;
+    }
+    if (h == 0) nseg_out[0] = sall;
 }
 __global__ __launch_bounds__(256) void k_hot_scan_c(uint32_t* __restrict__ C, uint32_t nblocks, uint32_t nhot,
                                                     const uint32_t* __restrict__ part, const uint32_t* __restrict__ hb) {
@@ -357,67 +374,46 @@
     }
 }
 
-#define BE_THREADS 1024
-#define BE_ITEMS 8
-__global__ __launch_bounds__(BE_THREADS) void k_bkt_edges(const sg_event* __restrict__ ev, uint32_t nblocks,
-                                                          uint32_t* __restrict__ edges) {
-    __shared__ uint32_t ws[BE_THREADS / 64];
+#define BM_TILES 256u
+__global__ __launch_bounds__(BM_TILES) void k_hot_bmax(const int64_t* __restrict__ tfirst, const uint32_t* __restrict__ P,
+                                                       uint32_t nblocks, uint32_t nhot, const uint32_t* __restrict__ hb,
+                                                       uint32_t* __restrict__ bmax) {
+    __shared__ uint32_t opens[BM_TILES];
+    __shared__ uint32_t nopen, next;
+    __shared__ uint64_t wm[BM_TILES / 64];
     const uint32_t t = threadIdx.x, l = t & 63, wv = t >> 6;
-    uint32_t run = 0;
-    for (uint32_t c0 = 0; c0 < nblocks; c0 += BE_THREADS * BE_ITEMS) {
-        const uint32_t t0 = c0 + t * BE_ITEMS;
-        int64_t ts[BE_ITEMS + 1];
-#pragma unroll
-        for (int k = 0; k <= BE_ITEMS; ++k) {
-            uint32_t tl = (t0 + k) ? t0 + k - 1 : 0u;
-            if (tl >= nblocks) tl = nblocks - 1;
-            ts[k] = ev[(uint64_t)tl * RS_TILE].ts;
-        }
-        uint32_t f = 0;
-#pragma unroll
-        for (int k = 0; k < BE_ITEMS; ++k)
-            if (t0 + k < nblocks && (t0 + k == 0 || ts[k + 1] / 500 != ts[k] / 500)) f |= 1u << k;
-        const uint32_t c = (uint32_t)__popc(f);
-        uint32_t x = c;
-#pragma unroll
-        for (int o = 1; o < 64; o <<= 1) {
-            const uint32_t y = __shfl_up(x, o, 64);
-            if ((int)l >= o) x += y;
-        }
-        if (l == 63) ws[wv] = x;
+    const uint32_t t0 = blockIdx.y * BM_TILES, a = t0 + t;
+    bool op = false;
+    if (a < nblocks) op = a == 0 || tfirst[a] / 500 != tfirst[a - 1] / 500;
+    const uint64_t bal = __ballot(op);
+    if (l == 0) wm[wv] = bal;
+    if (t == 0) next = nblocks;
+    __syncthreads();
+    uint32_t pre = 0, all = 0;
+    for (uint32_t k = 0; k < BM_TILES / 64; ++k) { const uint32_t c = (uint32_t)__popcll(wm[k]); if (k < wv) pre += c; all += c; }
+    if (op) opens[pre + (uint32_t)__popcll(bal & ((1ull << l) - 1ull))] = a;
+    if (t == 0) nopen = all;
+    if (all == 0) return;
+    for (uint32_t c0 = t0 + BM_TILES; c0 < nblocks; c0 += BM_TILES) {
+        const uint32_t b = c0 + t;
+        const bool ob = b < nblocks && tfirst[b] / 500 != tfirst[b - 1] / 500;
+        if (ob) atomicMin(&next, b);
         __syncthreads();
-        uint32_t pre = 0, all = 0;
-        for (uint32_t k = 0; k < BE_THREADS / 64; ++k) { if (k < wv) pre += ws[k]; all += ws[k]; }
-        uint32_t o = 1 + run + pre + x - c;
-#pragma unroll
-        for (int k = 0; k < BE_ITEMS; ++k)
-            if ((f >> k) & 1u) edges[o++] = t0 + k;
-        run += all;
+        if (next < nblocks) break;
         __syncthreads();
     }
-    if (t == 0) edges[0] = run;
-}
-#define BM_EDGES 32u
-__global__ __launch_bounds__(256) void k_hot_bmax(const uint32_t* __restrict__ P, uint32_t nblocks, uint32_t nhot,
-                                                  const uint32_t* __restrict__ hb, const uint32_t* __restrict__ edges,
-                                                  uint32_t* __restrict__ bmax) {
-    const uint32_t ne = edges[0], j0 = blockIdx.y * BM_EDGES, j1 = min(ne, j0 + BM_EDGES);
-    const uint32_t h = blockIdx.x * 256 + threadIdx.x;
-    if (j0 >= ne || h >= nhot) return;
+    __syncthreads();
+    const uint32_t h = blockIdx.x * BM_TILES + t;
+    if (h >= nhot) return;
     const uint32_t end = hb[h] + hb[HOT_MAX + h];
     uint32_t m = 0;
-    for (uint32_t j = j0; j < j1; ++j) {
-        const uint32_t a = edges[1 + j], b = j + 1 < ne ? edges[2 + j] : nblocks;
-        const uint32_t lo = P[(uint64_t)(a ? a - 1 : 0u) * nhot + h];
-        const uint32_t hi = b < nblocks ? P[(uint64_t)b * nhot + h] : end;
+    for (uint32_t j = 0; j < nopen; ++j) {
+        const uint32_t ea = opens[j], eb = j + 1 < nopen ? opens[j + 1] : next;
+        const uint32_t lo = P[(uint64_t)(ea ? ea - 1 : 0u) * nhot + h];
+        const uint32_t hi = eb < nblocks ? P[(uint64_t)eb * nhot + h] : end;
         m = max(m, hi - lo);
     }
     if (m) atomicMax(&bmax[h], m);
-}
-
-__device__ __forceinline__ uint32_t grp_pos(uint64_t j, uint32_t wd, const uint32_t* __restrict__ P, uint32_t nhot) {
-    if (wd & W_HOT) return P[(j / RS_TILE) * nhot + ((wd >> 12) & (HOT_MAX - 1))] + (wd & 0xFFFu);
-    return wd & W_POS;
 }
 
 #define GR_THREADS 256
@@ -706,34 +702,6 @@
     }
 }
 
-__global__ __launch_bounds__(HOT_MAX) void k_hot_segs(const uint32_t* __restrict__ hb, uint32_t nhot,
-                                                      const uint32_t* __restrict__ hot_list, Seg* __restrict__ segs,
-                                                      uint32_t* __restrict__ out) {
-    __shared__ uint32_t ws[HOT_MAX / 64];
-    const uint32_t t = threadIdx.x, l = t & 63, wv = t >> 6;
-    const uint32_t len = t < nhot ? hb[HOT_MAX + t] : 0u;
-    const uint32_t f = len ? 1u : 0u;
-    uint32_t x = f;
-#pragma unroll
-    for (int o = 1; o < 64; o <<= 1) {
-        const uint32_t y = __shfl_up(x, o, 64);
-        if ((int)l >= o) x += y;
-    }
-    if (l == 63) ws[wv] = x;
-    __syncthreads();
-    uint32_t pre = 0, all = 0;
-    for (uint32_t k = 0; k < HOT_MAX / 64; ++k) { if (k < wv) pre += ws[k]; all += ws[k]; }
-    if (f) {
-        Seg sg;
-        sg.res = hot_list[t];
-        sg.start = hb[t];
-        sg.len = 0;
-        sg.bin = 0;
-        segs[pre + x - f] = sg;
-    }
-    if (t == 0) out[0] = all;
-}
-
 __global__ void k_hot_clear(uint16_t* __restrict__ hot_tab, const uint32_t* __restrict__ hot_list, uint32_t nhot) {
     const uint32_t t = blockIdx.x * blockDim.x + threadIdx.x;
     if (t < nhot) hot_tab[hot_list[t]] = (uint16_t)HOT_NONE;
@@ -921,9 +889,22 @@
     if (threadIdx.x == 0 && total_out) *total_out = carry;
 }
 
+template <bool SELF>
 __global__ __launch_bounds__(SC_THREADS) void k_scan_down(const uint32_t* __restrict__ in, uint64_t n, const uint32_t* __restrict__ part,
-                                                       uint32_t* __restrict__ out, const uint32_t* __restrict__ ndev) {
+                                                       uint32_t* __restrict__ out, const uint32_t* __restrict__ ndev,
+                                                       uint32_t* __restrict__ total_out) {
     if (ndev && *ndev < n) n = *ndev;
+    uint32_t pbase = 0;
+    if (SELF) {
+        const bool last = blockIdx.x == gridDim.x - 1;
+        if ((uint64_t)blockIdx.x * SC_TILE >= n && !(last && total_out)) return;
+        uint32_t s = 0;
+        for (uint32_t i = threadIdx.x; i < blockIdx.x; i += SC_THREADS) s += part[i];
+        (void)block_excl_scan(s, &pbase);
+        if (last && total_out && threadIdx.x == 0) *total_out = pbase + part[blockIdx.x];
+    } else {
+        pbase = part[blockIdx.x];
+    }
     if ((uint64_t)blockIdx.x * SC_TILE >= n) return;
     uint64_t base = (uint64_t)blockIdx.x * SC_TILE + (uint64_t)threadIdx.x * SC_ITEMS;
     uint32_t loc[SC_ITEMS];
@@ -934,7 +915,7 @@
         loc[k] = i < n ? in[i] : 0;
         s += loc[k];
     }
-    uint32_t ex = block_excl_scan(s, nullptr) + part[blockIdx.x];
+    uint32_t ex = block_excl_scan(s, nullptr) + pbase;
     #pragma unroll
     for (int k = 0; k < SC_ITEMS; ++k) {
         uint64_t i = base + k;
@@ -1078,27 +1059,27 @@
                             const AuthDesc* auth, const uint32_t* auth_ids,
                             const uint16_t* hot_tab, uint32_t nhot, uint32_t nblocks, uint32_t* words,
                             uint32_t* hot_hist, uint32_t* ckeys, uint32_t* cvals, uint32_t* ccnt, uint32_t* chist,
-                            hipStream_t st) {
+                            int64_t* tfirst, hipStream_t st) {
     hipLaunchKernelGGL(k_grp_first<8>, dim3(nblocks), dim3(RS_THREADS), 0, st, ev, n, max_res, gbase, ring_mask, bflags,
                        t0_out, prio, key_ring, comp, ext, args, n_args, max_ctx, auth, auth_ids, hot_tab, nhot, nblocks, words,
-                       hot_hist, ckeys, cvals, ccnt, chist);
+                       hot_hist, ckeys, cvals, ccnt, chist, tfirst);
     return hipGetLastError();
 }
 hipError_t launch_hot_scan(uint32_t* C, uint32_t nblocks, uint32_t nhot, uint32_t* part, uint32_t* hb, uint32_t* total,
+                           uint64_t n, uint32_t* cold, const uint32_t* hot_list, Seg* segs, uint32_t* nseg,
                            hipStream_t st) {
-    if (!nhot) return hipMemsetAsync(total, 0, 4, st);
-    const uint32_t nch = (nblocks + HS_TC - 1) / HS_TC;
-    hipLaunchKernelGGL(k_hot_scan_a, dim3(nch), dim3(256), 0, st, C, nblocks, nhot, part);
-    hipLaunchKernelGGL(k_hot_scan_b, dim3(1), dim3(HOT_MAX), 0, st, part, nch, nhot, hb, total);
-    hipLaunchKernelGGL(k_hot_scan_c, dim3(nch), dim3(256), 0, st, C, nblocks, nhot, part, hb);
-    return hipGetLastError();
-}
-hipError_t launch_hot_bmax(const sg_event* ev, uint32_t nblocks, const uint32_t* P, uint32_t nhot, const uint32_t* hb,
-                           uint32_t* edges, uint32_t* bmax, hipStream_t st) {
+    const uint32_t nch = nhot ? (nblocks + HS_TC - 1) / HS_TC : 0u;
+    if (nhot) hipLaunchKernelGGL(k_hot_scan_a, dim3(nch), dim3(256), 0, st, C, nblocks, nhot, part);
+    hipLaunchKernelGGL(k_hot_scan_b, dim3(1), dim3(HOT_MAX), 0, st, part, nch, nhot, hb, total, n, cold, hot_list, segs,
+                       nseg);
+    if (nhot) hipLaunchKernelGGL(k_hot_scan_c, dim3(nch), dim3(256), 0, st, C, nblocks, nhot, part, hb);
+    return hipGetLastError();
+}
+hipError_t launch_hot_bmax(const int64_t* tfirst, uint32_t nblocks, const uint32_t* P, uint32_t nhot, const uint32_t* hb,
+                           uint32_t* bmax, hipStream_t st) {
     if (!nhot || !nblocks) return hipSuccess;
-    hipLaunchKernelGGL(k_bkt_edges, dim3(1), dim3(BE_THREADS), 0, st, ev, nblocks, edges);
-    hipLaunchKernelGGL(k_hot_bmax, dim3((nhot + 255) / 256, (nblocks + BM_EDGES - 1) / BM_EDGES), dim3(256), 0, st, P,
-                       nblocks, nhot, hb, edges, bmax);
+    hipLaunchKernelGGL(k_hot_bmax, dim3((nhot + BM_TILES - 1) / BM_TILES, (nblocks + BM_TILES - 1) / BM_TILES),
+                       dim3(BM_TILES), 0, st, tfirst, P, nblocks, nhot, hb, bmax);
     return hipGetLastError();
 }
 hipError_t launch_grp_records(const sg_event* ev, uint64_t n, uint64_t gbase, uint64_t ring_mask, int32_t max_rt,
@@ -1112,23 +1093,11 @@
                        need_blk);
     return hipGetLastError();
 }
-hipError_t launch_hot_segs(const uint32_t* hb, uint32_t nhot, const uint32_t* hot_list, Seg* segs, uint32_t* out,
-                           hipStream_t st) {
-    hipLaunchKernelGGL(k_hot_segs, dim3(1), dim3(HOT_MAX), 0, st, hb, nhot, hot_list, segs, out);
-    return hipGetLastError();
-}
 hipError_t launch_hot_build(const Seg* segs, const uint32_t* mp, uint32_t mb, uint32_t min_len, uint32_t max_res, uint16_t* hot_tab,
                             uint32_t* hot_list, uint32_t nhot_old, uint32_t* hot_n, hipStream_t st) {
     if (nhot_old) hipLaunchKernelGGL(k_hot_clear, dim3((nhot_old + 255) / 256), dim3(256), 0, st, hot_tab, hot_list, nhot_old);
     if (mb) hipLaunchKernelGGL(k_hot_build, dim3((mb + 255) / 256), dim3(256), 0, st, segs, mp, min_len, max_res, hot_tab,
                                hot_list, hot_n);
-    return hipGetLastError();
-}
-__global__ void k_cold_n(uint64_t n, const uint32_t* __restrict__ hot_total, uint32_t* __restrict__ out) {
-    if (threadIdx.x == 0) *out = (uint32_t)(n - *hot_total);
-}
-hipError_t launch_cold_n(uint64_t n, const uint32_t* hot_total, uint32_t* out, hipStream_t st) {
-    hipLaunchKernelGGL(k_cold_n, dim3(1), dim3(64), 0, st, n, hot_total, out);
     return hipGetLastError();
 }
 uint32_t hot_max() { return HOT_MAX; }
@@ -1229,6 +1198,19 @@
     }
     if (threadIdx.x == 0 && total) *total = tot;
 }
+#define SC_SELF_MAX 1024u
+static bool g_scan_three = false;
+void scan_force_three(bool on) { g_scan_three = on; }
+static void scan_tiles(const uint32_t* in, uint32_t* out, uint64_t n, const uint32_t* ndev, uint32_t* part,
+                       uint32_t* total, uint32_t nb, hipStream_t st) {
+    hipLaunchKernelGGL(k_scan_reduce, dim3(nb), dim3(SC_THREADS), 0, st, in, n, part, ndev);
+    if (nb <= SC_SELF_MAX && !g_scan_three) {
+        hipLaunchKernelGGL(k_scan_down<true>, dim3(nb), dim3(SC_THREADS), 0, st, in, n, part, out, ndev, total);
+        return;
+    }
+    hipLaunchKernelGGL(k_scan_top, dim3(1), dim3(SC_THREADS), 0, st, part, nb, total);
+    hipLaunchKernelGGL(k_scan_down<false>, dim3(nb), dim3(SC_THREADS), 0, st, in, n, part, out, ndev, (uint32_t*)nullptr);
+}
 hipError_t launch_scan(const uint32_t* in, uint32_t* out, uint64_t n, uint32_t* part, uint32_t* total,
                        hipStream_t st) {
     if (n <= SC_TILE) {
@@ -1237,18 +1219,14 @@
     }
     uint32_t nb = (uint32_t)((n + SC_TILE - 1) / SC_TILE);
     if (nb == 0) nb = 1;
-    hipLaunchKernelGGL(k_scan_reduce, dim3(nb), dim3(SC_THREADS), 0, st, in, n, part, (const uint32_t*)nullptr);
-    hipLaunchKernelGGL(k_scan_top, dim3(1), dim3(SC_THREADS), 0, st, part, nb, total);
-    hipLaunchKernelGGL(k_scan_down, dim3(nb), dim3(SC_THREADS), 0, st, in, n, part, out, (const uint32_t*)nullptr);
+    scan_tiles(in, out, n, nullptr, part, total, nb, st);
     return hipGetLastError();
 }
 hipError_t launch_scan_n(const uint32_t* in, uint32_t* out, uint64_t n, const uint32_t* ndev, uint32_t* part,
                          uint32_t* total, hipStream_t st) {
     uint32_t nb = (uint32_t)((n + SC_TILE - 1) / SC_TILE);
     if (nb == 0) nb = 1;
-    hipLaunchKernelGGL(k_scan_reduce, dim3(nb), dim3(SC_THREADS), 0, st, in, n, part, ndev);
-    hipLaunchKernelGGL(k_scan_top, dim3(1), dim3(SC_THREADS), 0, st, part, nb, total);
-    hipLaunchKernelGGL(k_scan_down, dim3(nb), dim3(SC_THREADS), 0, st, in, n, part, out, ndev);
+    scan_tiles(in, out, n, ndev, part, total, nb, st);
     return hipGetLastError();
 }
 
```

Measured after the change: 4.756 billion, median of 6. About the same (+0.5%).
